# yzGuu830/efficient-speech-codec

Measured on AMD Instinct MI355X. Metric: audio-seconds/sec encode+decode, ESC-Base 9kbps 3s@16kHz, higher is better.
Workload: dtype f32 (fp32 storage and accumulation everywhere; the K = C contractions of the MLPs, of the attention's Q / K / V projections, of PatchMerge / PatchSplit and of the de-embedding run on the fp16 matrix cores with every fp32 operand split into two fp16 terms under power-of-two scales (range-safe by cons

## Files before the change

### efficient-speech-codec_amd/build.py

```python
import os
import subprocess
import sys
from concurrent.futures import ThreadPoolExecutor

HERE = os.path.dirname(os.path.abspath(__file__))
CSRC = os.path.join(HERE, "csrc")
OUT_DIR = os.path.join(HERE, "esc", "lib")
TAG = os.environ.get("ESCX_BUILD_TAG", "")
OBJ_DIR = os.path.join(HERE, "build" + ("_" + TAG if TAG else ""))
LIB = os.path.join(OUT_DIR, "libescx" + ("_" + TAG if TAG else "") + ".so")
SOURCES = ["escx_api.cpp", "escx_params.cpp", "escx_profile.cpp", "collective.cpp", "train.hip", "disc.hip", "dac.hip", "dac_loss.hip", "gemm_swin.hip", "gemm_misc.hip", "kernels_misc.hip", "len_kernels.hip", "fused_swin.hip"]
HEADERS = ["launch_prof.h", "split_terms.h", "fused_pvq.h", "fused_prvq.h", "train_prvq.h", "fused_mlp_x3.h", "train_kernels.h", "train_mlp_fused.h", "disc_kernels.h", "disc_msd_kernels.h", "dac_kernels.h", "dac_x3.h", "dac_grad_kernels.h", "dac_param_grad_kernels.h", "dac_loss_kernels.h", "gemm_bf16.h", "conv32_halo.h", "gemm_engine.h", "kernels.h", "len_kernels.h", "launchers.h", "escx_internal.h", "fused_mlp.h", "fused_attn.h", "fused_rowgemm.h", "fused_deembed.h", os.path.join("..", "..", "include", "escx.h")]
HIPCC = os.environ.get("HIPCC", "/opt/rocm/bin/hipcc")
FLAGS = ["--offload-arch=gfx950", "-O3", "-std=c++17", "-fPIC", "-Wno-unused-result"] + os.environ.get("ESCX_EXTRA_CXXFLAGS", "").split()


def _newest(paths):
    return max(os.path.getmtime(p) for p in paths)


def build(force: bool = False, verbose: bool = True) -> str:
    srcs = [os.path.join(CSRC, s) for s in SOURCES]
    deps = srcs + [os.path.normpath(os.path.join(CSRC, h)) for h in HEADERS]
    if not force and os.path.exists(LIB) and os.path.getmtime(LIB) >= _newest(deps):
        return LIB
    os.makedirs(OUT_DIR, exist_ok=True)
    os.makedirs(OBJ_DIR, exist_ok=True)

    def compile_one(src):
        obj = os.path.join(OBJ_DIR, os.path.basename(src) + ".o")
        cmd = [HIPCC] + FLAGS + (["-x", "hip"] if src.endswith(".cpp") else []) + ["-c", src, "-o", obj]
        r = subprocess.run(cmd, capture_output=True, text=True)
        if r.returncode != 0:
            raise RuntimeError(f"hipcc failed for {src}:\n{r.stdout}\n{r.stderr}")
        return obj

    with ThreadPoolExecutor(max_workers=len(srcs)) as ex:
        objs = list(ex.map(compile_one, srcs))
    cmd = [HIPCC, "--offload-arch=gfx950", "-shared", "-fPIC", "-o", LIB] + objs + ["-ldl"]
    r = subprocess.run(cmd, capture_output=True, text=True)
    if r.returncode != 0:
        raise RuntimeError(f"link failed:\n{r.stdout}\n{r.stderr}")
    if verbose:
        print(f"built {LIB} ({os.path.getsize(LIB) / 1e6:.1f} MB)")
    return LIB


if __name__ == "__main__":
    build(force="--force" in sys.argv)
```

### efficient-speech-codec_amd/csrc/escx_api.cpp

```cpp
#include <hip/hip_runtime.h>

#include <algorithm>
#include <cmath>
#include <cstdlib>
#include <cstring>
#include <map>
#include <mutex>
#include <tuple>
#include <utility>
#include <vector>

#include "escx_internal.h"
#include "launchers.h"

using namespace escx;

static void part_layout(escx_handle_s* h, int B, int T, int* k, int* per, int* pass) {
    *k = std::min(n_parts(h, B), h->n_sets);
    *pass = std::max(1, std::min(pass_clips(h, B, T), h->sets[0].shp.B));
    *per = *k <= 1 ? B : (B + *k - 1) / *k;
}

template <class F>
static int run_halves(escx_handle_s* h, int B, int T, hipStream_t st, F part) {
// ... 963 lines not shown
    const int n = h->n, G = c.group_size;
    const long long bstride = (long long)S * G * s.Tq, sstride = (long long)G * s.Tq;
    const int T2 = c.patch_t * s.W;
    long long* cd = (long long*)codes;
    if ((rc = run_stft(h, wave, B, Lx, s.T, h->spec, st))) return rc;
    if (raw_feat) PROF("unpad_len", 0, 2.0 * B * s.T * c.in_dim * h->F * 4, unpad_rows_len(h->spec, raw_feat, lc.d_L, 0, c.patch_t, c.hop_length, B, s.T, c.in_dim, h->F, h->Fp, st));
    if ((rc = run_encoder(h, s, st))) return rc;
    const size_t lslot = (size_t)G * B * s.Tq;
    float* loss = cm_loss ? h->loss_terms : nullptr;
    int n_slots = 1;
    int H = s.encH[n - 1], Hn;
    float* dec = h->decA; float* other = h->decB;
    if ((rc = run_pvq_quantize(h, h->quants[0], h->enc_hs[n - 1], nullptr, B, s.W, cd, bstride, loss, dec, st))) return rc;
    for (int i = 0; i + 1 < n; ++i) {
        if (i < S - 1) {
            if ((rc = run_pvq_quantize(h, h->quants[i + 1], h->enc_hs[n - 1 - i], dec, B, s.W, cd + (i + 1) * sstride, bstride, loss ? loss + (size_t)(i + 1) * lslot : nullptr, dec, st))) return rc;
            n_slots = i + 2;
        }
        if ((rc = run_layer(h, h->layers[n + i], dec, other, B, H, s.W, &Hn, st))) return rc;
        std::swap(dec, other); H = Hn;
    }
    if ((rc = run_layer(h, h->layers[2 * n - 1], dec, other, B, H, s.W, &Hn, st))) return rc;
    if ((rc = run_deembed(h, other, B, s.W, h->rspec, st))) return rc;
    if ((rc = run_istft(h, h->rspec, B, T2, wave_out, st))) return rc;
    if (recon_feat) PROF("unpad_len", 0, 2.0 * B * T2 * c.in_dim * h->F * 4, unpad_rows_len(h->rspec, recon_feat, lc.d_W, 1, c.patch_t, c.hop_length, B, T2, c.in_dim, h->F, h->Fp, st));
    if (cm_loss) PROF("loss_reduce_len", 0, (double)n_slots * lslot * 4, loss_reduce_len(loss, lc.d_W, c.overlap, n_slots, G, B, s.Tq, cm_loss, st));
    PROF("codes_mask_len", 0, 8.0 * B * bstride, codes_mask_len(cd, cd, lc.d_W, c.overlap, B, S * G, s.Tq, -1, st));
    return launch_ok("forward_lengths");
}

static int run_prvq(escx_handle_s* h, const float* enc, const long long* codes_in, int B, int W, long long* codes, long long bstride, const int* clip_S,
                    int S, float* loss, long long lslot, float* out, hipStream_t st) {
    const escx_config& c = h->cfg;
    const Quant& q = h->quants[0];
    const int Tq = W / c.overlap, M = B * Tq;
    const double vec = (double)c.overlap * q.Hq * q.C, G = c.group_size;
    int rc = -1;
    PROF(codes_in ? "prvq_decode" : (out ? "prvq_fused" : "prvq_fused_codes"),
         codes_in ? 2.0 * M * vec * q.d : 2.0 * M * vec * q.d * (out ? 2 : 1) + 2.0 * M * S * G * c.codebook_size * q.d,
         (double)M * vec * ((codes_in ? 0 : 1) + (out ? 1 : 0)) * 4,
         rc = prvq_fused(enc, codes_in, B, q.Hq, W, q.Cp, c.overlap, q.wdf, q.Nz, q.Kq, pvq_down_splits(M, q.Kq, q.Cp), pvq_down_bk(q.Cp), q.cbn, q.c2, q.cbraw,
                         c.group_size, c.codebook_size, q.d, q.dt, q.wup, codes, bstride, clip_S, S, S, loss, lslot, 1.0f / ((float)Tq * q.d * c.group_size),
                         c.l2norm, out, st));
    if (rc) ESCX_FAIL(ESCX_ERR_UNSUPPORTED, "rvq quantiser: geometry not covered (codebook_dim %d, %d groups)", q.d, c.group_size);
    return launch_ok("prvq");
}

static int run_plain_decoder(escx_handle_s* h, int B, int Hb, int W, float* rspec, hipStream_t st) {
    const int n = h->n;
    int rc, H = Hb, Hn;
    float* dec = h->decA; float* other = h->decB;
    for (int i = 0; i + 1 < n; ++i) {
        if ((rc = run_layer(h, h->layers[n + i], dec, other, B, H, W, &Hn, st))) return rc;
        std::swap(dec, other); H = Hn;
    }
    if ((rc = run_layer(h, h->layers[2 * n - 1], dec, other, B, H, W, &Hn, st))) return rc;
    return run_deembed(h, other, B, W, rspec, st);
}

static int rvq_counts(escx_handle_s* h, int B, const int32_t* streams, int S, int* Smax) {
    if (!streams) {
        if (S < 1 || S > h->num_rvqs) ESCX_FAIL(ESCX_ERR_INVALID_ARG, "num_streams=%d outside [1, %d] (num_rvqs)", S, h->num_rvqs);
        *Smax = S;
        return 0;
    }
    if (B < 1) ESCX_FAIL(ESCX_ERR_INVALID_ARG, "batch=%d: the per-clip stream counts need at least one clip", B);
    int m = 0;
    for (int b = 0; b < B; ++b) {
        if (streams[b] < 1 || streams[b] > h->num_rvqs) ESCX_FAIL(ESCX_ERR_INVALID_ARG, "streams[%d]=%d outside [1, %d] (num_rvqs)", b, streams[b], h->num_rvqs);
        m = std::max(m, (int)streams[b]);
    }
    *Smax = m;
    return 0;
}

static int rvq_upload(escx_handle_s* h, int B, const int32_t* streams, const int** dev, hipStream_t st) {
    *dev = nullptr;
    if (!streams) return 0;
    int32_t* d = nullptr;
    MixBufs mb; mb.add(&d, (size_t)B);
    int rc = mix_alloc(h, mb); if (rc) return rc;
    ESCX_HIP(hipMemcpyAsync(d, streams, (size_t)B * sizeof(int32_t), hipMemcpyHostToDevice, st));
    *dev = d;
    return 0;
}

static int rvq_encode(escx_handle_s* h, const float* wave, int B, int L, const int32_t* streams, int S, int64_t* codes, int* fh, int* fw, void* stream) {
    int rc = check_ready(h); if (rc) return rc;
    if (!wave || !codes) ESCX_FAIL(ESCX_ERR_INVALID_ARG, "null pointer");
    int Smax = 0; if ((rc = rvq_counts(h, B, streams, S, &Smax))) return rc;
    if (L <= h->n_fft / 2) ESCX_FAIL(ESCX_ERR_INVALID_ARG, "n_samples=%d too short for reflect padding of %d", L, h->n_fft / 2);
    Shapes s; if ((rc = ensure_ws(h, B, frames_of(h, L), &s))) return rc;
    hipStream_t st = (hipStream_t)stream;
    const int* Sdev; if ((rc = rvq_upload(h, B, streams, &Sdev, st))) return rc;
    if ((rc = ensure_pvq_tables(h, st))) return rc;
    const long long cstride = (long long)Smax * h->cfg.group_size * s.Tq;
    rc = run_halves(h, B, s.T, st, [&](int b0, int nb, hipStream_t sti) -> int {
        Shapes sp = s; sp.B = nb; int r;
        if ((r = run_stft(h, wave + (size_t)b0 * L, nb, L, sp.T, h->spec, sti))) return r;
        if ((r = run_encoder(h, sp, sti))) return r;
        return run_prvq(h, h->enc_hs[h->n - 1], nullptr, nb, sp.W, (long long*)codes + b0 * cstride, cstride, Sdev ? Sdev + b0 : nullptr, Smax, nullptr, 0, nullptr, sti);
    });
    if (rc) return rc;
    if (fh) *fh = s.encH[h->n - 1];
    if (fw) *fw = s.W;
    return ESCX_OK;
}

static int rvq_decode(escx_handle_s* h, const int64_t* codes, int B, int S, const int32_t* streams, int fh, int fw, float* wave_out, float* recon_feat, void* stream) {
    int rc = check_infer_ready(h); if (rc) return rc;
    if (!codes || !wave_out) ESCX_FAIL(ESCX_ERR_INVALID_ARG, "null pointer");
    const escx_config& c = h->cfg;
    if (S < 1 || S > h->num_rvqs) ESCX_FAIL(ESCX_ERR_INVALID_ARG, "codes.size(1)=%d outside [1, %d] (num_rvqs)", S, h->num_rvqs);
    int Smax = 0; if ((rc = rvq_counts(h, B, streams, S, &Smax))) return rc;
    if (Smax > S) ESCX_FAIL(ESCX_ERR_INVALID_ARG, "codes.size(1)=%d: must be at least max(streams)=%d", S, Smax);
    if (fw < 1 || fw % c.overlap) ESCX_FAIL(ESCX_ERR_ASSERT, "Time dimension must be multiple of overlap");
    Shapes s; if ((rc = ensure_ws(h, B, frames_for_width(h, fw), &s))) return rc;
    if (s.W != fw || s.encH[h->n - 1] != fh) ESCX_FAIL(ESCX_ERR_INVALID_ARG, "feat_shape (%d,%d) does not match the model (%d,%d)", fh, fw, s.encH[h->n - 1], s.W);
    hipStream_t st = (hipStream_t)stream;
    const int* Sdev; if ((rc = rvq_upload(h, B, streams, &Sdev, st))) return rc;
    if ((rc = ensure_pvq_tables(h, st))) return rc;
    const int T2 = c.patch_t * fw, out_len = c.hop_length * (T2 - 1);
    const long long cstride = (long long)S * c.group_size * (fw / c.overlap);
    return run_halves(h, B, s.T, st, [&](int b0, int nb, hipStream_t sti) -> int {
        int r;
        if ((r = run_prvq(h, nullptr, (const long long*)codes + b0 * cstride, nb, fw, nullptr, cstride, Sdev ? Sdev + b0 : nullptr, S, nullptr, 0, h->decA, sti))) return r;
        if ((r = run_plain_decoder(h, nb, fh, fw, h->rspec, sti))) return r;
        if ((r = run_istft(h, h->rspec, nb, T2, wave_out + (size_t)b0 * out_len, sti))) return r;
        if (recon_feat) spec_unpad(h, h->rspec, recon_feat + (size_t)b0 * T2 * c.in_dim * h->F, (long long)nb * T2, sti);
        return launch_ok("rvq_decode");
    });
}

static int rvq_forward(escx_handle_s* h, const float* wave, const float* feat, int B, int LT, const int32_t* streams, int S, int64_t* codes, float* wave_out,
                       float* raw_feat, float* recon_feat, float* cm_loss, void* stream) {
    int rc = check_infer_ready(h); if (rc) return rc;
    if ((!wave == !feat) || !codes || !wave_out) ESCX_FAIL(ESCX_ERR_INVALID_ARG, "null pointer (exactly one of wave / feat, codes and wave_out are required)");
    const escx_config& c = h->cfg;
    int Smax = 0; if ((rc = rvq_counts(h, B, streams, S, &Smax))) return rc;
    const int L = wave ? LT : 0;
    int T = wave ? 0 : LT;
    if (wave && L <= h->n_fft / 2) ESCX_FAIL(ESCX_ERR_INVALID_ARG, "n_samples=%d too short for reflect padding of %d", L, h->n_fft / 2);
    if (!wave && T < c.patch_t) ESCX_FAIL(ESCX_ERR_INVALID_ARG, "n_frames=%d shorter than one patch", T);
    if (wave) T = frames_of(h, L);
    Shapes s; if ((rc = ensure_ws(h, B, T, &s))) return rc;
    if (s.W % c.overlap) ESCX_FAIL(ESCX_ERR_ASSERT, "Time dimension must be multiple of overlap");
    hipStream_t st = (hipStream_t)stream;
    const int* Sdev; if ((rc = rvq_upload(h, B, streams, &Sdev, st))) return rc;
    if ((rc = ensure_pvq_tables(h, st))) return rc;
    const int G = c.group_size, T2 = c.patch_t * s.W, out_len = c.hop_length * (T2 - 1);
    const long long cstride = (long long)Smax * G * s.Tq;
    return run_halves(h, B, s.T, st, [&](int b0, int nb, hipStream_t sti) -> int {
        Shapes sp = s; sp.B = nb; int r;
        if (wave) { if ((r = run_stft(h, wave + (size_t)b0 * L, nb, L, sp.T, h->spec, sti))) return r; }
        else spec_pad(h, feat + (size_t)b0 * sp.T * c.in_dim * h->F, h->spec, (long long)nb * sp.T, sti);
        if (raw_feat) spec_unpad(h, h->spec, raw_feat + (size_t)b0 * sp.T * c.in_dim * h->F, (long long)nb * sp.T, sti);
        if ((r = run_encoder(h, sp, sti))) return r;
        const long long lslot = (long long)G * nb * sp.Tq;
        float* loss = cm_loss ? h->loss_terms : nullptr;
        if ((r = run_prvq(h, h->enc_hs[h->n - 1], nullptr, nb, sp.W, (long long*)codes + b0 * cstride, cstride, Sdev ? Sdev + b0 : nullptr, Smax, loss, lslot, h->decA, sti))) return r;
        if ((r = run_plain_decoder(h, nb, sp.encH[h->n - 1], sp.W, h->rspec, sti))) return r;
        if ((r = run_istft(h, h->rspec, nb, T2, wave_out + (size_t)b0 * out_len, sti))) return r;
        if (recon_feat) spec_unpad(h, h->rspec, recon_feat + (size_t)b0 * T2 * c.in_dim * h->F, (long long)nb * T2, sti);
        if (cm_loss) PROF("loss_reduce", 0, (double)lslot * Smax * 4, loss_reduce(loss, Smax, G, nb * sp.Tq, sp.Tq, cm_loss + b0, sti));
        return launch_ok("rvq_forward");
    });
}

extern "C" int escx_spec_transform(escx_handle h, const float* wave, int B, int L, float* spec, void* stream) {
    int rc = check_ready(h); if (rc) return rc;
    if (!wave || !spec || B < 1) ESCX_FAIL(ESCX_ERR_INVALID_ARG, "bad argument");
    if (L <= h->n_fft / 2) ESCX_FAIL(ESCX_ERR_INVALID_ARG, "n_samples=%d too short for reflect padding of %d", L, h->n_fft / 2);
    const int T = frames_of(h, L);
    TmpBuf t; if (t.alloc((size_t)B * T * h->cfg.in_dim * h->Fp)) ESCX_FAIL(ESCX_ERR_HIP, "hipMalloc failed");
    hipStream_t st = (hipStream_t)stream;
    if ((rc = run_stft(h, wave, B, L, T, t.p, st))) return rc;
    spec_unpad(h, t.p, spec, (long long)B * T, st);
    return launch_ok("spec_transform");
}

extern "C" int escx_audio_reconstruct(escx_handle h, const float* spec, int B, int T, float* wave, void* stream) {
    int rc = check_ready(h); if (rc) return rc;
    if (!spec || !wave || B < 1 || T < 2) ESCX_FAIL(ESCX_ERR_INVALID_ARG, "bad argument (need at least 2 frames)");
    TmpBuf ts, tf;
    if (ts.alloc((size_t)B * T * h->cfg.in_dim * h->Fp) || tf.alloc((size_t)B * T * h->winP)) ESCX_FAIL(ESCX_ERR_HIP, "hipMalloc failed");
    hipStream_t st = (hipStream_t)stream;
    const escx_config& c = h->cfg;
    spec_pad(h, spec, ts.p, (long long)B * T, st);
    gemm_store(ts.p, c.in_dim * h->Fp, B * T, h->idft_w, h->winP, c.in_dim * h->Fp, tf.p, h->winP, nullptr, st);
    istft_ola(tf.p, h->win2, wave, B, T, h->winP, c.win_length, c.hop_length, h->left, h->n_fft / 2, c.hop_length * (T - 1), st);
    return launch_ok("audio_reconstruct");
}

extern "C" int escx_patch_embed(escx_handle h, const float* spec, int B, int T, float* tokens, void* stream) {
    int rc = check_ready(h); if (rc) return rc;
    const escx_config& c = h->cfg;
    const int W = T / c.patch_t, H0 = c.in_freq / c.patch_f;
    if (!spec || !tokens || B < 1 || W < 1) ESCX_FAIL(ESCX_ERR_INVALID_ARG, "bad argument");
    TmpBuf ts, tt;
    if (ts.alloc((size_t)B * T * c.in_dim * h->Fp) || tt.alloc((size_t)B * H0 * W * h->C0p)) ESCX_FAIL(ESCX_ERR_HIP, "hipMalloc failed");
    hipStream_t st = (hipStream_t)stream;
    spec_pad(h, spec, ts.p, (long long)B * T, st);
    if ((rc = run_patch_embed(h, ts.p, B, T, W, tt.p, st))) return rc;
    unpad_rows(tt.p, tokens, (long long)B * H0 * W, h->C0, h->C0p, st);
    return launch_ok("patch_embed");
}

static int stage_ws_for_w(escx_handle_s* h, int B, int W, Shapes* s) {
    int rc = ensure_ws(h, h->parts * B, frames_for_width(h, W), s, B);
    if (!rc) s->B = B;
    return rc;
}

extern "C" int escx_transformer_layer(escx_handle h, int layer_id, const float* x, int B, int H, int W, float* y, int* H_out, void* stream) {
    int rc = check_ready(h); if (rc) return rc;
    if (layer_id < 0 || layer_id >= 2 * h->n) ESCX_FAIL(ESCX_ERR_INVALID_ARG, "layer_id out of range");
    const Layer& L = h->layers[layer_id];
    Shapes s; if ((rc = stage_ws_for_w(h, B, W, &s))) return rc;
    if ((size_t)H > (size_t)2 * s.H0) ESCX_FAIL(ESCX_ERR_INVALID_ARG, "H too large for this model");
    hipStream_t st = (hipStream_t)stream;
    if ((rc = ensure_pvq_tables(h, st))) return rc;
    int Hn;
    const size_t need = (size_t)B * H * W * L.Cp, cap = std::max<size_t>((size_t)B * s.H0 * s.W * h->C0p, 1);
    size_t big = 0; for (int i = 0; i < h->n; ++i) big = std::max(big, (size_t)B * s.encH[i] * s.W * rup(h->cfg.h_dims[i], 16));
    if (need > std::max(cap, big)) ESCX_FAIL(ESCX_ERR_INVALID_ARG, "(H=%d, W=%d) is larger than any map of this layer", H, W);
    pad_rows(x, h->stageA, (long long)B * H * W, L.C, L.Cp, st);
    if ((rc = run_layer(h, L, h->stageA, h->stageB, B, H, W, &Hn, st))) return rc;
    unpad_rows(h->stageB, y, (long long)B * Hn * W, L.scale ? L.Cout : L.C, L.scale ? L.CoutP : L.Cp, st);
    if (H_out) *H_out = Hn;
    return launch_ok("transformer_layer");
}

extern "C" int escx_pvq_encode(escx_handle h, int sid, const float* enc, const float* dec, int B, int W, int64_t* codes, int64_t bstride,
                               void* stream) {
    int rc = check_ready(h); if (rc) return rc;
    if (h->kind != 0) ESCX_FAIL(ESCX_ERR_UNSUPPORTED, "escx_pvq_encode: the cross-scale quantisers do not exist on an rvq handle (escx_rvq_encode / escx_rvq_decode)");
    if (sid < 0 || sid >= h->cfg.max_streams) ESCX_FAIL(ESCX_ERR_INVALID_ARG, "stream_id out of range");
    if (W % h->cfg.overlap) ESCX_FAIL(ESCX_ERR_ASSERT, "Time dimension must be multiple of overlap");
    const Quant& q = h->quants[sid];
    Shapes s; if ((rc = stage_ws_for_w(h, B, W, &s))) return rc;
    hipStream_t st = (hipStream_t)stream;
    const long long rows = (long long)B * q.Hq * W;
    if ((rc = ensure_pvq_tables(h, st))) return rc;
    pad_rows(enc, h->stageA, rows, q.C, q.Cp, st);
    if (dec) pad_rows(dec, h->stageB, rows, q.C, q.Cp, st);
    return run_pvq_quantize(h, q, h->stageA, dec ? h->stageB : nullptr, B, W, (long long*)codes, bstride, nullptr, nullptr, st);
}

extern "C" int escx_pvq_decode(escx_handle h, int sid, const int64_t* codes, int64_t bstride, const float* dec, int B, int W, float* out,
                               void* stream) {
    int rc = check_ready(h); if (rc) return rc;
    if (h->kind != 0) ESCX_FAIL(ESCX_ERR_UNSUPPORTED, "escx_pvq_decode: the cross-scale quantisers do not exist on an rvq handle (escx_rvq_encode / escx_rvq_decode)");
    if (sid < 0 || sid >= h->cfg.max_streams) ESCX_FAIL(ESCX_ERR_INVALID_ARG, "stream_id out of range");
    if (W % h->cfg.overlap) ESCX_FAIL(ESCX_ERR_ASSERT, "Time dimension must be multiple of overlap");
    const Quant& q = h->quants[sid];
    Shapes s; if ((rc = stage_ws_for_w(h, B, W, &s))) return rc;
    hipStream_t st = (hipStream_t)stream;
    const long long rows = (long long)B * q.Hq * W;
    if ((rc = ensure_pvq_tables(h, st))) return rc;
    if (dec) pad_rows(dec, h->stageB, rows, q.C, q.Cp, st);
    if ((rc = run_pvq_decode(h, q, (const long long*)codes, bstride, dec ? h->stageB : nullptr, B, W, h->stageA, st))) return rc;
    unpad_rows(h->stageA, out, rows, q.C, q.Cp, st);
    return launch_ok("pvq_decode");
}

extern "C" int escx_rvq_encode(escx_handle h, const float* tokens, int B, int W, int S, int64_t* codes, float* zq_out, void* stream) {
    int rc = check_ready(h); if (rc) return rc;
    if (h->kind != 1) ESCX_FAIL(ESCX_ERR_UNSUPPORTED, "escx_rvq_encode needs an rvq handle (escx_create_rvq)");
    if (!tokens || !codes) ESCX_FAIL(ESCX_ERR_INVALID_ARG, "null pointer");
    if (B < 1 || W < 1) ESCX_FAIL(ESCX_ERR_INVALID_ARG, "batch and W must be positive");
    if (S < 1 || S > h->num_rvqs) ESCX_FAIL(ESCX_ERR_INVALID_ARG, "num_streams=%d outside [1, %d] (num_rvqs)", S, h->num_rvqs);
    if (W % h->cfg.overlap) ESCX_FAIL(ESCX_ERR_ASSERT, "Time dimension must be multiple of overlap");
    const Quant& q = h->quants[0];
    Shapes s; if ((rc = stage_ws_for_w(h, B, W, &s))) return rc;
    hipStream_t st = (hipStream_t)stream;
    const long long rows = (long long)B * q.Hq * W;
    pad_rows(tokens, h->stageA, rows, q.C, q.Cp, st);
    if ((rc = run_prvq(h, h->stageA, nullptr, B, W, (long long*)codes, (long long)S * h->cfg.group_size * (W / h->cfg.overlap), nullptr, S, nullptr, 0,
                       zq_out ? h->stageB : nullptr, st))) return rc;
    if (zq_out) unpad_rows(h->stageB, zq_out, rows, q.C, q.Cp, st);
    return launch_ok("rvq_encode");
}

extern "C" int escx_rvq_decode(escx_handle h, const int64_t* codes, int B, int S, int W, float* tokens_out, void* stream) {
    int rc = check_ready(h); if (rc) return rc;
    if (h->kind != 1) ESCX_FAIL(ESCX_ERR_UNSUPPORTED, "escx_rvq_decode needs an rvq handle (escx_create_rvq)");
    if (!codes || !tokens_out) ESCX_FAIL(ESCX_ERR_INVALID_ARG, "null pointer");
    if (B < 1 || W < 1) ESCX_FAIL(ESCX_ERR_INVALID_ARG, "batch and W must be positive");
    if (S < 1 || S > h->num_rvqs) ESCX_FAIL(ESCX_ERR_INVALID_ARG, "codes.size(1)=%d outside [1, %d] (num_rvqs)", S, h->num_rvqs);
    if (W % h->cfg.overlap) ESCX_FAIL(ESCX_ERR_ASSERT, "Time dimension must be multiple of overlap");
    const Quant& q = h->quants[0];
    Shapes s; if ((rc = stage_ws_for_w(h, B, W, &s))) return rc;
    hipStream_t st = (hipStream_t)stream;
    if ((rc = run_prvq(h, nullptr, (const long long*)codes, B, W, nullptr, (long long)S * h->cfg.group_size * (W / h->cfg.overlap), nullptr, S, nullptr, 0,
                       h->stageA, st))) return rc;
    unpad_rows(h->stageA, tokens_out, (long long)B * q.Hq * W, q.C, q.Cp, st);
    return launch_ok("rvq_decode");
}

extern "C" int escx_patch_deembed(escx_handle h, const float* tokens, int B, int W, float* spec, void* stream) {
    int rc = check_infer_ready(h); if (rc) return rc;
    Shapes s; if ((rc = stage_ws_for_w(h, B, W, &s))) return rc;
    hipStream_t st = (hipStream_t)stream;
    pad_rows(tokens, h->stageA, (long long)B * s.H0 * W, h->C0, h->C0p, st);
    if ((rc = run_deembed(h, h->stageA, B, W, h->rspec, st))) return rc;
    spec_unpad(h, h->rspec, spec, (long long)B * h->cfg.patch_t * W, st);
    return launch_ok("patch_deembed");
}

extern "C" int escx_debug_mlp_trace(unsigned long long* dev_buf) { mlp_set_trace(dev_buf); return 0; }
extern "C" int escx_test_fastdiv(int n, int d) { return test_fastdiv(n, d); }
extern "C" int escx_test_math(const float* x, float* y, int64_t n, int which, void* stream) {
    test_math(x, y, n, which, (hipStream_t)stream);
    return launch_ok("test_math");
}
extern "C" int escx_test_copy_rows(const float* src, float* dst, int64_t rows, int row_floats, void* stream) {
    if (!src || !dst || rows < 1 || row_floats < 4 || row_floats % 4) ESCX_FAIL(ESCX_ERR_INVALID_ARG, "bad argument");
    test_copy_rows(src, dst, rows, row_floats, (hipStream_t)stream);
    return launch_ok("test_copy_rows");
}
extern "C" int escx_codes_pack10(const int64_t* codes, uint8_t* out, int64_t n, void* stream) {
    if (!codes || !out || n < 0) ESCX_FAIL(ESCX_ERR_INVALID_ARG, "bad argument");
    codes_pack10((const long long*)codes, out, n, (hipStream_t)stream);
    return launch_ok("codes_pack10");
}
extern "C" int escx_codes_unpack10(const uint8_t* in, int64_t* codes, int64_t n, void* stream) {
    if (!codes || !in || n < 0) ESCX_FAIL(ESCX_ERR_INVALID_ARG, "bad argument");
    codes_unpack10(in, (long long*)codes, n, (hipStream_t)stream);
    return launch_ok("codes_unpack10");
}
static int ragged_offsets(int B, int Smax, int64_t gt, const int32_t* streams, hipStream_t st, const long long** off_dev, long long* n) {
    if (!streams || B < 1 || Smax < 1 || gt < 1) ESCX_FAIL(ESCX_ERR_INVALID_ARG, "bad argument");
    std::vector<long long> off((size_t)B + 1, 0);
    for (int b = 0; b < B; ++b) {
        if (streams[b] < 1 || streams[b] > Smax) ESCX_FAIL(ESCX_ERR_INVALID_ARG, "streams[%d]=%d outside [1, %d]", b, streams[b], Smax);
        off[b + 1] = off[b] + (long long)streams[b] * gt;
    }
    long long* d = reinterpret_cast<long long*>(stream_scratch(st, 2, 2 * off.size()));
    if (!d) ESCX_FAIL(ESCX_ERR_HIP, "scratch allocation failed");
    ESCX_HIP(hipMemcpyAsync(d, off.data(), off.size() * sizeof(long long), hipMemcpyHostToDevice, st));
    *off_dev = d; *n = off[B];
    return 0;
}
extern "C" int escx_codes_pack10_streams(const int64_t* codes, int B, int Smax, int64_t gt, const int32_t* streams, uint8_t* out, void* stream) {
    if (!codes || !out) ESCX_FAIL(ESCX_ERR_INVALID_ARG, "null pointer");
    hipStream_t st = (hipStream_t)stream;
    const long long* off; long long n; int rc;
    if ((rc = ragged_offsets(B, Smax, gt, streams, st, &off, &n))) return rc;
    codes_pack10_streams((const long long*)codes, out, off, B, (long long)Smax * gt, n, st);
    return launch_ok("codes_pack10_streams");
}
extern "C" int escx_codes_unpack10_streams(const uint8_t* in, int B, int Smax, int64_t gt, const int32_t* streams, int64_t* codes, void* stream) {
    if (!codes || !in) ESCX_FAIL(ESCX_ERR_INVALID_ARG, "null pointer");
    hipStream_t st = (hipStream_t)stream;
    const long long* off; long long n; int rc;
    if ((rc = ragged_offsets(B, Smax, gt, streams, st, &off, &n))) return rc;
    codes_unpack10_streams(in, (long long*)codes, off, B, (long long)Smax * gt, st);
    return launch_ok("codes_unpack10_streams");
}
extern "C" int escx_codes_narrow(const int64_t* codes, int16_t* out, int64_t n, void* stream) {
    codes_narrow((const long long*)codes, (short*)out, n, (hipStream_t)stream);
    return launch_ok("codes_narrow");
}
extern "C" int escx_codes_widen(const int16_t* in, int64_t* codes, int64_t n, void* stream) {
    codes_widen((const short*)in, (long long*)codes, n, (hipStream_t)stream);
    return launch_ok("codes_widen");
}
```

### efficient-speech-codec_amd/csrc/fused_deembed.h

```cpp
#pragma once
#include <hip/hip_runtime.h>
#include <type_traits>
#include "gemm_engine.h"
#include "split_terms.h"

namespace escx {

struct DeembedArgs {
    const float* x;
    const f32x4* wf;
    const float* bias;
    float* out;
    int B, H, W, pf, pt, in_dim, Fp, n_out;
};

template <int CP>
__global__ __launch_bounds__(512) void deembed7_kernel(DeembedArgs a) {
    ESCX_SET_PRIO_SMALL();
    constexpr int KK = CP / 16, TH = 8, TW = 32, HH = TH + 6, HW = TW + 6, PS = CP + 4;
    constexpr int NW = 8, NP = 7 * KK, NPW = (NP + NW - 1) / NW;
    __shared__ float xs[HH * HW * PS];
    __shared__ f32x4 wr[2][NP * 64];
    const int tid = threadIdx.x, lane = tid & 63, l15 = lane & 15, lg = lane >> 4;
    const int wave = __builtin_amdgcn_readfirstlane(tid >> 6);
    const int ntw = (a.W + TW - 1) / TW, nth = (a.H + TH - 1) / TH;
    int bid = blockIdx.x;
    const int tw = bid % ntw; bid /= ntw;
    const int th = bid % nth; const int b = bid / nth;
    const int h0 = th * TH, w0 = tw * TW;

    auto issue_row = [&](int dh, int buf) {
        const f32x4* src = a.wf + (size_t)dh * NP * 64 + lane;
#pragma unroll
        for (int i = 0; i < NPW; ++i) {
            int c = wave + i * NW;
            if (NP % NW != 0) c = min(c, NP - 1);
            __builtin_amdgcn_global_load_lds((const void*)(src + c * 64), (__attribute__((address_space(3))) void*)(&wr[buf][c * 64]), 16, 0, 0);
        }
    };
    issue_row(0, 0);

    const float* xb = a.x + (size_t)b * a.H * a.W * CP;
    auto halo_vec = [&](int v) -> f32x4 {
        const int pix = v / (KK * 4), q = v - pix * (KK * 4);
        const int ph = pix / HW, pw = pix - ph * HW;
        const int gh = h0 - 3 + ph, gw = w0 - 3 + pw;
        return (gh >= 0 && gh < a.H && gw >= 0 && gw < a.W) ? ld4(xb + ((size_t)gh * a.W + gw) * CP + 4 * q) : zero4();
    };
    auto halo_put = [&](int v, f32x4 val) {
        const int pix = v / (KK * 4), q = v - pix * (KK * 4);
        *reinterpret_cast<f32x4*>(&xs[pix * PS + 4 * q]) = val;
    };
    constexpr int ROWV = HW * KK * 4;
    static_assert(ROWV <= 512, "one vector per thread per extra halo row");
    for (int v = tid; v < TH * ROWV; v += 512) halo_put(v, halo_vec(v));

    const bool seg1 = w0 + 16 < a.W;
    f32x4 acc[2] = {zero4(), zero4()};
    const float* xrow = &xs[(wave * HW + l15) * PS + 4 * lg];
    auto tap_row = [&](auto two_segments, int dh) {
        constexpr bool TWO = decltype(two_segments)::value;
        constexpr int NS = 7 * KK;
        const f32x4* wb = &wr[dh & 1][lane];
        const float* xr = xrow + dh * HW * PS;
        f32x4 w[2], x0[2], x1[2];
        auto fetch = [&](int st, int slot) {
            const int dw = st / KK, kk = st - dw * KK;
            w[slot] = wb[st * 64];
            x0[slot] = *reinterpret_cast<const f32x4*>(xr + dw * PS + 16 * kk);
            if (TWO) x1[slot] = *reinterpret_cast<const f32x4*>(xr + (dw + 16) * PS + 16 * kk);
            __builtin_amdgcn_sched_group_barrier(0x100, TWO ? 3 : 2, 0);
        };
        fetch(0, 0);
#pragma unroll
        for (int st = 0; st < NS; ++st) {
            if (st + 1 < NS) fetch(st + 1, (st + 1) & 1);
#pragma unroll
            for (int r = 0; r < 4; ++r) {
                acc[0] = __builtin_amdgcn_mfma_f32_16x16x4f32(w[st & 1][r], x0[st & 1][r], acc[0], 0, 0, 0);
                if (TWO) acc[1] = __builtin_amdgcn_mfma_f32_16x16x4f32(w[st & 1][r], x1[st & 1][r], acc[1], 0, 0, 0);
            }
            __builtin_amdgcn_sched_group_barrier(0x008, TWO ? 8 : 4, 0);
        }
    };
    for (int dh = 0; dh < 7; ++dh) {
        asm volatile("s_waitcnt vmcnt(0)" ::: "memory");
        __syncthreads();
        issue_row(min(dh + 1, 6), (dh + 1) & 1);
        const bool extra = dh < 6 && tid < ROWV;
        f32x4 nv = zero4();
        if (extra) nv = halo_vec((TH + dh) * ROWV + tid);
        if (seg1) tap_row(std::true_type{}, dh); else tap_row(std::false_type{}, dh);
        if (extra) halo_put((TH + dh) * ROWV + tid, nv);
    }

    const int h = h0 + wave;
    if (h >= a.H) return;
    const int Q = a.pf * a.pt;
    const f32x4 bv = ld4(a.bias + 4 * lg);
#pragma unroll
    for (int t = 0; t < 2; ++t) {
        const int w = w0 + 16 * t + l15;
        if (w >= a.W) continue;
#pragma unroll
        for (int r = 0; r < 4; ++r) {
            const int nn = 4 * lg + r;
            if (nn >= a.n_out) continue;
            const int co = nn / Q, q = nn - co * Q, s1 = q / a.pt, s2 = q - s1 * a.pt;
            a.out[((size_t)(b * (a.pt * a.W) + a.pt * w + s2) * a.in_dim + co) * a.Fp + a.pf * h + s1] = acc[t][r] + bv[r];
        }
    }
}

constexpr int de2_steps(int CP) { return (49 * CP + 31) / 32; }
inline size_t deembed7_x2_bytes(int CP) { return (size_t)de2_steps(CP) * 2 * 1024 + 32; }

__global__ __launch_bounds__(256) void deembed7_x2_pack_kernel(const f32x4* __restrict__ wf, bf16x8* __restrict__ out, int CP, int nsteps) {
    const int idx = blockIdx.x * 256 + threadIdx.x;
    if (idx >= nsteps * 64) return;
    const int step = idx >> 6, lane = idx & 63, n = lane & 15, g = lane >> 4, KK = CP / 16;
    bf16x8* tail = out + (size_t)nsteps * 2 * 64;
    const float sc = x2_scale(*reinterpret_cast<const unsigned*>(tail));
    float v[8];
#pragma unroll
    for (int e = 0; e < 8; ++e) {
        const int k = 32 * step + 8 * g + e, tap = k / CP, c = k - tap * CP;
        v[e] = tap < 49 ? wf[(size_t)(tap * KK + c / 16) * 64 + 16 * ((c % 16) / 4) + n][c % 4] : 0.f;
    }
    bf16x8 t[2];
    split_terms<2>(v, t, sc);
    out[(size_t)(step * 2 + 0) * 64 + lane] = t[0]; out[(size_t)(step * 2 + 1) * 64 + lane] = t[1];
    if (idx == 0) { float* o = reinterpret_cast<float*>(tail + 1); o[0] = 1.0f / sc; o[1] = sc; o[2] = 0.f; o[3] = 0.f; }
}

template <int CP>
__global__ __launch_bounds__(512) void deembed7_x2_kernel(DeembedArgs a, const bf16x8* __restrict__ wf2) {
    static_assert(CP == 48, "one wrap of the channel index per 32-deep step");
    ESCX_SET_PRIO_SMALL();
    constexpr int TH = 8, TW = 32, HH = TH + 6, HW = TW + 6, PS = CP + 8;
    constexpr int NSTEP = de2_steps(CP), CH = 8, NCH = (NSTEP + CH - 1) / CH, NW = 8, Q8 = CP / 8;
    extern __shared__ __attribute__((aligned(16))) unsigned char de2_lds[];
    _Float16* xh0 = reinterpret_cast<_Float16*>(de2_lds);
    _Float16* xh1 = xh0 + HH * HW * PS;
    bf16x8* wr = reinterpret_cast<bf16x8*>(xh1 + HH * HW * PS);
    const int tid = threadIdx.x, lane = tid & 63, l15 = lane & 15, lg = lane >> 4;
    const int wave = __builtin_amdgcn_readfirstlane(tid >> 6);
    const int ntw = (a.W + TW - 1) / TW, nth = (a.H + TH - 1) / TH;
    int bid = blockIdx.x;
    const int tw = bid % ntw; bid /= ntw;
    const int th = bid % nth; const int b = bid / nth;
    const int h0 = th * TH, w0 = tw * TW;

    auto issue_chunk = [&](int ch, int buf) {
        const int pieces = min(CH, NSTEP - ch * CH) * 2;
        const bf16x8* src = wf2 + (size_t)ch * CH * 2 * 64 + lane;
        for (int c = wave; c < pieces; c += NW)
            __builtin_amdgcn_global_load_lds((const void*)(src + c * 64), (__attribute__((address_space(3))) void*)(&wr[(buf * CH * 2 + c) * 64]), 16, 0, 0);
    };
    issue_chunk(0, 0);
    const f32x4 scv = *reinterpret_cast<const f32x4*>(wf2 + (size_t)NSTEP * 2 * 64 + 1);

    const float* xb = a.x + (size_t)b * a.H * a.W * CP;
    constexpr int NV = (HH * HW * Q8 + 511) / 512;
    float xr[NV][8];
    float amax = 0.f;
#pragma unroll
    for (int i = 0; i < NV; ++i) {
        const int v = tid + 512 * i;
        const int pix = v / Q8, q = v - pix * Q8;
        const int ph = pix / HW, pw = pix - ph * HW;
        const int gh = h0 - 3 + ph, gw = w0 - 3 + pw;
        if (v < HH * HW * Q8 && gh >= 0 && gh < a.H && gw >= 0 && gw < a.W) {
            const float* p = xb + ((size_t)gh * a.W + gw) * CP + 8 * q;
            const f32x4 u0 = ld4(p), u1 = ld4(p + 4);
#pragma unroll
            for (int e = 0; e < 4; ++e) { xr[i][e] = u0[e]; xr[i][4 + e] = u1[e]; amax = fmaxf(amax, fmaxf(fabsf(u0[e]), fabsf(u1[e]))); }
        } else {
#pragma unroll
            for (int e = 0; e < 8; ++e) xr[i][e] = 0.f;
        }
    }
    __shared__ float de2_red[NW];
    for (int o = 32; o >= 1; o >>= 1) amax = fmaxf(amax, __shfl_xor(amax, o));
    if (lane == 0) de2_red[wave] = amax;
    __syncthreads();
#pragma unroll
    for (int i = 0; i < NW; ++i) amax = fmaxf(amax, de2_red[i]);
    const float act_sc = act_pow2_scale(amax), act_inv = 1.0f / act_sc;
#pragma unroll
    for (int i = 0; i < NV; ++i) {
        const int v = tid + 512 * i;
        if (v < HH * HW * Q8) {
            const int pix = v / Q8, q = v - pix * Q8;
            bf16x8 t[2];
            split_terms<2>(xr[i], t, act_sc);
            *reinterpret_cast<bf16x8*>(xh0 + pix * PS + 8 * q) = t[0];
            *reinterpret_cast<bf16x8*>(xh1 + pix * PS + 8 * q) = t[1];
        }
    }

    const bool seg1 = w0 + 16 < a.W;
    f32x4 acc0 = zero4(), acc1 = zero4();
    int c = 8 * lg, dw = 0, dh = 0;
    for (int ch = 0; ch < NCH; ++ch) {
        asm volatile("s_waitcnt vmcnt(0)" ::: "memory");
        __syncthreads();
        if (ch + 1 < NCH) issue_chunk(ch + 1, (ch + 1) & 1);
        const bf16x8* wb = &wr[((ch & 1) * CH * 2) * 64 + lane];
#pragma unroll
        for (int s = 0; s < CH; ++s) {
            if (ch * CH + s >= NSTEP) break;
            const int dhc = dh > 6 ? 6 : dh;
            const int xoff = ((wave + dhc) * HW + dw + l15) * PS + c;
            const bf16x8 wt0 = wb[(s * 2) * 64], wt1 = wb[(s * 2 + 1) * 64];
            const bf16x8 x00 = *reinterpret_cast<const bf16x8*>(xh0 + xoff), x01 = *reinterpret_cast<const bf16x8*>(xh1 + xoff);
            acc0 = mma_x<2>(wt0, x01, acc0); acc0 = mma_x<2>(wt1, x00, acc0); acc0 = mma_x<2>(wt0, x00, acc0);
            if (seg1) {
                const bf16x8 x10 = *reinterpret_cast<const bf16x8*>(xh0 + xoff + 16 * PS), x11 = *reinterpret_cast<const bf16x8*>(xh1 + xoff + 16 * PS);
                acc1 = mma_x<2>(wt0, x11, acc1); acc1 = mma_x<2>(wt1, x10, acc1); acc1 = mma_x<2>(wt0, x10, acc1);
            }
            c += 32;
            if (c >= CP) { c -= CP; if (++dw == 7) { dw = 0; ++dh; } }
        }
    }

    const int h = h0 + wave;
    if (h >= a.H) return;
    const int Q = a.pf * a.pt;
    const f32x4 bv = ld4(a.bias + 4 * lg);
    const f32x4 accs[2] = {acc0 * (scv[0] * act_inv), acc1 * (scv[0] * act_inv)};
#pragma unroll
    for (int t = 0; t < 2; ++t) {
        const int w = w0 + 16 * t + l15;
        if (w >= a.W) continue;
#pragma unroll
        for (int r = 0; r < 4; ++r) {
            const int nn = 4 * lg + r;
            if (nn >= a.n_out) continue;
            const int co = nn / Q, q = nn - co * Q, s1 = q / a.pt, s2 = q - s1 * a.pt;
            a.out[((size_t)(b * (a.pt * a.W) + a.pt * w + s2) * a.in_dim + co) * a.Fp + a.pf * h + s1] = accs[t][r] + bv[r];
        }
    }
}

}
```

### efficient-speech-codec_amd/csrc/fused_swin.hip

```cpp
#include "fused_attn.h"
#include "fused_mlp.h"
#include "fused_mlp_x3.h"
#include <atomic>
#include "fused_rowgemm.h"
#include "fused_deembed.h"
#include "launchers.h"

namespace escx {

template <int CP, int TM>
static void launch_mlp(const MlpArgs& a, hipStream_t s) {
    const int waves = (a.M + 16 * TM - 1) / (16 * TM);
    ESCX_LAUNCH((mlp_fused_kernel<CP, TM>), dim3((waves + 3) / 4), dim3(256), 0, s, a);
}

template <int CP, int TM, int NW>
static void launch_mlp_lds(const MlpArgs& a, hipStream_t s) {
    const int rows = 16 * TM * NW;
    const int hs = a.HS > 1 ? a.HS : 1;
    ESCX_LAUNCH((mlp_fused_lds_kernel<CP, TM, NW>), dim3(((a.M + rows - 1) / rows) * hs), dim3(64 * NW), 0, s, a);
}

template <int CP>
static int launch_mlp_lds_variant(int variant, const MlpArgs& a, hipStream_t s) {
    switch (variant) {
        case 1: launch_mlp_lds<CP, 1, 4>(a, s); return 0;
        case 3: launch_mlp_lds<CP, 1, 8>(a, s); return 0;
        default: return -1;
    }
}

static unsigned long long* g_mlp_trace = nullptr;
void mlp_set_trace(unsigned long long* p) { g_mlp_trace = p; }
unsigned long long* debug_trace_buffer() { return g_mlp_trace; }

void rows_combine(float* dst, const float* src, const float* partial, const float* bias, long long M, int Cp, int n, hipStream_t s) {
    const long long n4 = M * Cp / 4;
    ESCX_LAUNCH(rows_combine_kernel, dim3((unsigned)((n4 + 255) / 256)), dim3(256), 0, s, dst, src, partial, bias, M, Cp, n);
}

template <int CP, int NW>
static void launch_mlp_split(const MlpArgs& a, hipStream_t s) {
    const int rows = 16 * NW;
    ESCX_LAUNCH((mlp_fused_lds_kernel<CP, 1, NW, true>), dim3((a.M + rows - 1) / rows), dim3(64 * NW), 0, s, a);
}

int mlp_fused(float* x, int M, int C, int Cp, const float* gamma, const float* beta, const float* w1f, const float* b1,
              const float* w2f, const float* b2, const float* wcf, int hiddenP, int variant, int* hs_io, float* partial, hipStream_t s, float* out,
              const MlpSplit* split) {
    if (split) {
        const int hs0 = hs_io ? *hs_io : 1;
        if (hs0 > 1 || out || (variant != 1 && variant != 3) || (split->NT & 1) || !(Cp == 80 || Cp == 96 || Cp == 144)) return ESCX_COMB_UNSUPPORTED;
        MlpArgs a{x, gamma, beta, reinterpret_cast<const f32x4*>(w1f), b1, reinterpret_cast<const f32x4*>(w2f), b2,
                  reinterpret_cast<const f32x4*>(wcf), M, C, hiddenP / 16, 1e-5f, 1, nullptr, nullptr,
                  reinterpret_cast<const f32x4*>(split->wf), split->gamma, split->beta, split->out, split->NT, split->H, split->W, split->C2p};
        const bool nw8 = variant == 3;
        switch (Cp) {
            case 80: if (nw8) launch_mlp_split<80, 8>(a, s); else launch_mlp_split<80, 4>(a, s); return 0;
            case 96: if (nw8) launch_mlp_split<96, 8>(a, s); else launch_mlp_split<96, 4>(a, s); return 0;
            case 144: if (nw8) launch_mlp_split<144, 8>(a, s); else launch_mlp_split<144, 4>(a, s); return 0;
        }
        return ESCX_COMB_UNSUPPORTED;
    }
    int hs = hs_io ? *hs_io : 1;
    const bool lds_width = Cp == 48 || Cp == 80 || Cp == 96 || Cp == 144 || Cp == 192 || Cp == 384;
    if (hs > 1 && (variant <= 0 || variant > 3 || !lds_width || !partial || (hiddenP / 16) % hs)) hs = 1;
    if (hs_io) *hs_io = hs;
    MlpArgs a{x, gamma, beta, reinterpret_cast<const f32x4*>(w1f), b1, reinterpret_cast<const f32x4*>(w2f), b2,
              reinterpret_cast<const f32x4*>(wcf), M, C, hiddenP / 16, 1e-5f, hs, partial, out,
              nullptr, nullptr, nullptr, nullptr, 0, 0, 0, 0};
    if (out && hs > 1) return -1;
    if (variant > 0) {
        switch (Cp) {
            case 48: return launch_mlp_lds_variant<48>(variant, a, s);
            case 80: return launch_mlp_lds_variant<80>(variant, a, s);
            case 96: return launch_mlp_lds_variant<96>(variant, a, s);
            case 144: return launch_mlp_lds_variant<144>(variant, a, s);
            case 192: return launch_mlp_lds_variant<192>(variant, a, s);
            case 384: return launch_mlp_lds_variant<384>(variant, a, s);
            default: break;
        }
    }
    switch (Cp) {
        case 16: launch_mlp<16, 4>(a, s); return 0;
        case 32: launch_mlp<32, 4>(a, s); return 0;
        case 48: launch_mlp<48, 4>(a, s); return 0;
        case 64: launch_mlp<64, 4>(a, s); return 0;
        case 80: launch_mlp<80, 4>(a, s); return 0;
        case 96: launch_mlp<96, 2>(a, s); return 0;
        case 112: launch_mlp<112, 2>(a, s); return 0;
        case 128: launch_mlp<128, 2>(a, s); return 0;
        case 144: launch_mlp<144, 2>(a, s); return 0;
        case 160: launch_mlp<160, 2>(a, s); return 0;
        case 192: launch_mlp<192, 2>(a, s); return 0;
        case 256: launch_mlp<256, 1>(a, s); return 0;
        case 288: launch_mlp<288, 1>(a, s); return 0;
        case 384: launch_mlp<384, 1>(a, s); return 0;
        default: return -1;
    }
}

static size_t mlp_x3_frag_bytes(int Cp, int hiddenP, int nt) { return (size_t)(hiddenP / 32) * mlp_x3_frags(Cp, nt) * 1024; }
size_t mlp_x3_bytes(int Cp, int hiddenP, int nt) { return mlp_x3_frag_bytes(Cp, hiddenP, nt) + 48 + (nt == 2 ? (size_t)(hiddenP + 2 * Cp) * sizeof(float) : 0); }

int mlp_x3_pack(const float* w1, const float* w2, void* image, int Cp, int hiddenP, hipStream_t s, int nt, const float* gamma, const float* beta, const float* b1, int C) {
    if (Cp % 16 || hiddenP % 32 || (nt != 2 && nt != 3)) return -1;
    if (nt == 2 && (!gamma || !beta || !b1)) return -1;
    char* tail = reinterpret_cast<char*>(image) + mlp_x3_frag_bytes(Cp, hiddenP, nt);
    const int KS = (Cp + 31) / 32, KK = Cp / 16;
    const long long total = (long long)(hiddenP / 32) * (2 * KS + KK) * 64;
    if (nt == 2) {
        unsigned* mx = reinterpret_cast<unsigned*>(tail);
        if (hipMemsetAsync(mx, 0, 16, s) != hipSuccess) return -1;
        const long long n = (long long)hiddenP * Cp;
        ESCX_LAUNCH(absmax_bits_kernel, dim3((unsigned)std::min<long long>(256, (n + 255) / 256)), dim3(256), 0, s, w1, n, mx);
        ESCX_LAUNCH(absmax_bits_kernel, dim3((unsigned)std::min<long long>(256, (n + 255) / 256)), dim3(256), 0, s, w2, n, mx + 1);
        ESCX_LAUNCH(rownorm2_max_bits_kernel, dim3((unsigned)((hiddenP + 3) / 4)), dim3(256), 0, s, w1, hiddenP, Cp, Cp, mx + 2);
    }
    ESCX_LAUNCH(mlp_x3_pack_kernel, dim3((unsigned)((total + 255) / 256)), dim3(256), 0, s, w1, w2, reinterpret_cast<bf16x8*>(image), Cp, hiddenP, KS, KK, nt, gamma, beta, b1, C);
    if (nt == 2) ESCX_LAUNCH(mlp_x3_prescale_kernel, dim3((unsigned)((hiddenP + 2 * Cp + 255) / 256)), dim3(256), 0, s, reinterpret_cast<bf16x8*>(tail), gamma, beta, b1, Cp, hiddenP);
    return 0;
}

template <int CP, int NW, int NT = 3>
static void launch_mlp_x3(const MlpArgs& a, hipStream_t s) {
    auto kern = mlp_x3_kernel<CP, NW, false, NT>;
    constexpr int lds = 2 * mlp_x3_stage_frags(CP, NT) * 1024;
    if constexpr (lds > 48 * 1024) {
        static std::atomic<unsigned> done{0};
        int dev = 0; (void)hipGetDevice(&dev);
        const unsigned bit = 1u << (dev & 31);
        if (!(done.load(std::memory_order_relaxed) & bit)) { (void)hipFuncSetAttribute((const void*)kern, hipFuncAttributeMaxDynamicSharedMemorySize, lds); done.fetch_or(bit, std::memory_order_relaxed); }
    }
    const int hs = a.HS > 1 ? a.HS : 1;
    ESCX_LAUNCH(kern, dim3(((a.M + 16 * NW - 1) / (16 * NW)) * hs), dim3(64 * NW), lds, s, a);
}


size_t mlp_x3_split_bytes(int Cp, int Np) { return (size_t)(Np / 16) * mlp_x3_split_tfy(Cp, 3) * 1024 + 32; }
static char* mlp_x3_split_trailer(const void* image, int Cp, int Np) { return reinterpret_cast<char*>(const_cast<void*>(image)) + mlp_x3_split_bytes(Cp, Np) - 32; }
int mlp_x3_split_pack(const float* wf, void* image, int Cp, int Np, hipStream_t s, int nt, const float* gamma, const float* beta, int C) {
    if (nt != 2 && nt != 3) return -1;
    if (nt == 2 && (!gamma || !beta)) return -1;
    const int KK = Cp / 16, NT = Np / 16;
    const long long total = (long long)NT * ((KK + 1) / 2) * 64;
    char* tail = mlp_x3_split_trailer(image, Cp, Np);
    if (nt == 2) {
        if (hipMemsetAsync(tail, 0, 16, s) != hipSuccess) return -1;
        const long long n = (long long)NT * KK * 64 * 4;
        ESCX_LAUNCH(absmax_bits_kernel, dim3((unsigned)std::min<long long>(256, (n + 255) / 256)), dim3(256), 0, s, wf, n, reinterpret_cast<unsigned*>(tail));
    }
    ESCX_LAUNCH(mlp_x3_split_pack_kernel, dim3((unsigned)((total + 255) / 256)), dim3(256), 0, s, reinterpret_cast<const f32x4*>(wf), reinterpret_cast<bf16x8*>(image), NT, KK,
                nt, mlp_x3_split_tfy(Cp, nt), reinterpret_cast<bf16x8*>(tail), gamma, beta, Cp, C);
    return 0;
}

template <int CP, int NW, int NT = 3>
static void launch_mlp_x3_split(const MlpArgs& a, hipStream_t s) {
    auto kern = mlp_x3_kernel<CP, NW, true, NT>;
    constexpr int lds = 2 * mlp_x3_stage_frags(CP, NT) * 1024;
    if constexpr (lds > 48 * 1024) {
        static std::atomic<unsigned> done{0};
        int dev = 0; (void)hipGetDevice(&dev);
        const unsigned bit = 1u << (dev & 31);
        if (!(done.load(std::memory_order_relaxed) & bit)) { (void)hipFuncSetAttribute((const void*)kern, hipFuncAttributeMaxDynamicSharedMemorySize, lds); done.fetch_or(bit, std::memory_order_relaxed); }
    }
    ESCX_LAUNCH(kern, dim3((a.M + 16 * NW - 1) / (16 * NW)), dim3(64 * NW), lds, s, a);
}

int mlp_x3(float* x, int M, int C, int Cp, const float* gamma, const float* beta, const float* b1, const float* b2, const void* image, int hiddenP, int nw, int* hs_io, float* partial,
           hipStream_t s, const MlpSplit* split, int nt, float* out) {
    if (!image || hiddenP % 32 || (nt != 2 && nt != 3)) return -1;
    if (out && (split || (hs_io && *hs_io > 1))) return -1;
    if (split) {
        if ((hs_io && *hs_io > 1) || !split->wf || !(Cp == 80 || Cp == 96 || Cp == 144)) return ESCX_COMB_UNSUPPORTED;
        MlpArgs a{};
        a.x = x; a.gamma = gamma; a.beta = beta; a.b1 = b1; a.b2 = b2; a.M = M; a.C = C; a.HT = hiddenP / 16; a.eps = 1e-5f; a.HS = 1; a.x3_w = image;
        a.sp_wf = reinterpret_cast<const f32x4*>(split->wf); a.sp_gamma = split->gamma; a.sp_beta = split->beta; a.sp_out = split->out;
        a.sp_NT = split->NT; a.sp_H = split->H; a.sp_W = split->W; a.sp_C2p = split->C2p;
        if (nt == 2) a.sp_scale = reinterpret_cast<const float*>(mlp_x3_split_trailer(split->wf, Cp, 16 * split->NT) + 16);
        switch (Cp) {
#define ESCX_X3S_CASE(CPV) case CPV: if (nt == 2) { if (nw == 8) launch_mlp_x3_split<CPV, 8, 2>(a, s); else launch_mlp_x3_split<CPV, 4, 2>(a, s); } \
                           else { if (nw == 8) launch_mlp_x3_split<CPV, 8>(a, s); else launch_mlp_x3_split<CPV, 4>(a, s); } return 0;
            ESCX_X3S_CASE(80) ESCX_X3S_CASE(96) ESCX_X3S_CASE(144)
#undef ESCX_X3S_CASE
        }
        return ESCX_COMB_UNSUPPORTED;
    }
    int hs = hs_io ? *hs_io : 1;
    if (hs > 1 && (!partial || (hiddenP / 32) % hs)) hs = 1;
    if (hs_io) *hs_io = hs;
    MlpArgs a{};
    a.x = x; a.gamma = gamma; a.beta = beta; a.b1 = b1; a.b2 = b2; a.M = M; a.C = C; a.HT = hiddenP / 16; a.eps = 1e-5f; a.HS = hs; a.partial = partial; a.x3_w = image; a.out = out;
#define ESCX_X3_CASE(CPV) case CPV: if (nt == 2) { if (nw == 8) launch_mlp_x3<CPV, 8, 2>(a, s); else launch_mlp_x3<CPV, 4, 2>(a, s); } \
                          else { if (nw == 8) launch_mlp_x3<CPV, 8>(a, s); else launch_mlp_x3<CPV, 4>(a, s); } return 0;
    switch (Cp) {
        ESCX_X3_CASE(48) ESCX_X3_CASE(80) ESCX_X3_CASE(96) ESCX_X3_CASE(144) ESCX_X3_CASE(192) ESCX_X3_CASE(384)
        default: return -1;
    }
#undef ESCX_X3_CASE
}


template <int KP, int SEGS>
static int launch_rowgemm(const RowGemmArgs& a, hipStream_t s) {
    if (a.x3_wf) {
        if constexpr (KP == 96 || KP == 160 || KP == 192 || KP == 288 || KP == 384 || KP == 144 || KP == 80) {
            constexpr int KSx = (KP + 31) / 32, TFx = 3 * KSx, UTx = 36 / TFx >= 4 ? 4 : (36 / TFx >= 2 ? 2 : 1);
            constexpr int TMx = KP <= 96 ? 2 : 1, NWx = 4;
            auto kern = rowgemm_x3_kernel<KP, SEGS, TMx, NWx, UTx>;
            auto kern2 = rowgemm_x3_kernel<KP, SEGS, TMx, NWx, UTx, 2>;
            constexpr int lds = 2 * UTx * TFx * 1024, lds2 = 2 * UTx * 2 * KSx * 1024;
            if constexpr (lds > 48 * 1024) {
                static std::atomic<unsigned> done{0};
                int dev = 0; (void)hipGetDevice(&dev);
                const unsigned bit = 1u << (dev & 31);
                if (!(done.load(std::memory_order_relaxed) & bit)) {
                    (void)hipFuncSetAttribute((const void*)kern, hipFuncAttributeMaxDynamicSharedMemorySize, lds);
                    (void)hipFuncSetAttribute((const void*)kern2, hipFuncAttributeMaxDynamicSharedMemorySize, lds2);
                    done.fetch_or(bit, std::memory_order_relaxed);
                }
            }
            if (a.x3_scale) ESCX_LAUNCH(kern2, dim3((a.M + 16 * TMx * NWx - 1) / (16 * TMx * NWx), 1), dim3(64 * NWx), lds2, s, a);
            else ESCX_LAUNCH(kern, dim3((a.M + 16 * TMx * NWx - 1) / (16 * TMx * NWx), 1), dim3(64 * NWx), lds, s, a);
            return 0;
        }
    }
    constexpr int KK = KP / 16;
    constexpr int UT = KK <= 6 ? 4 : (KK <= 12 ? 2 : 1);
    constexpr int TM = KP <= 192 ? 2 : 1;
    constexpr int NW = 4;
    const int rows = 16 * TM * NW;
    RowGemmArgs b = a;
    b.nt_chunk = (a.NT + UT - 1) / UT * UT;
    const int chunks = (a.NT + b.nt_chunk - 1) / b.nt_chunk;
    ESCX_LAUNCH((rowgemm_fused_kernel<KP, SEGS, TM, NW, UT>), dim3((a.M + rows - 1) / rows, chunks), dim3(64 * NW), 0, s, b);
    return 0;
}

size_t rowgemm_x3_bytes(int KP, int Np) { return (size_t)(Np / 16) * 3 * ((KP + 31) / 32) * 1024 + 32; }
static char* rowgemm_x3_trailer(const void* image, int KP, int Np) { return reinterpret_cast<char*>(const_cast<void*>(image)) + rowgemm_x3_bytes(KP, Np) - 32; }
int rowgemm_x3_pack(const float* wf, void* image, int KP, int Np, hipStream_t s, int nt, const float* gamma, const float* beta, int C) {
    const int KK = KP / 16, KS = (KP + 31) / 32, NT = Np / 16;
    const long long total = (long long)NT * (KS > KK ? KS : KK) * 64;
    if (nt == 2) {
        unsigned* mx = reinterpret_cast<unsigned*>(rowgemm_x3_trailer(image, KP, Np));
        (void)hipMemsetAsync(mx, 0, 16, s);
        const long long n = (long long)NT * KK * 64 * 4;
        ESCX_LAUNCH(absmax_bits_kernel, dim3((unsigned)std::min<long long>(256, (n + 255) / 256)), dim3(256), 0, s, wf, n, mx);
    }
    ESCX_LAUNCH(attn_x3_pack_kernel, dim3((unsigned)((total + 255) / 256)), dim3(256), 0, s, reinterpret_cast<const f32x4*>(wf), reinterpret_cast<bf16x8*>(image),
                       reinterpret_cast<bf16x8*>(rowgemm_x3_trailer(image, KP, Np)), NT, 1, KK, KS, (nt == 2 ? 2 : 3) * KS, 0u, nt == 2 ? 2 : 3, gamma, beta, KP, C, (const float*)nullptr, 0, 0, 0);
    return 0;
}

int rowgemm_fused(int segs, const float* x, float* out, const float* gamma, const float* beta, const float* wf, const int* map, int M,
                  int rows_per_clip, int src_rows_per_clip, int C, int Cp, int Np, int split, int H, int W, int C2p, hipStream_t s,
                  const void* x3_wf, int x3_nt) {
    const int KP = segs * Cp;
    RowGemmArgs a{x, out, gamma, beta, reinterpret_cast<const f32x4*>(wf), map, M, rows_per_clip, src_rows_per_clip, C, Cp, Np / 16,
                  split, H, W, C2p, 1e-5f, Np / 16, x3_wf,
                  (x3_wf && x3_nt == 2) ? reinterpret_cast<const float*>(rowgemm_x3_trailer(x3_wf, KP, Np) + 16) : nullptr};
    if (segs == 1) {
        switch (KP) {
            case 16: return launch_rowgemm<16, 1>(a, s);
            case 48: return launch_rowgemm<48, 1>(a, s);
            case 80: return launch_rowgemm<80, 1>(a, s);
            case 96: return launch_rowgemm<96, 1>(a, s);
            case 144: return launch_rowgemm<144, 1>(a, s);
            case 192: return launch_rowgemm<192, 1>(a, s);
            case 384: return launch_rowgemm<384, 1>(a, s);
            default: return -1;
        }
    }
    switch (KP) {
        case 32: return launch_rowgemm<32, 2>(a, s);
        case 96: return launch_rowgemm<96, 2>(a, s);
        case 160: return launch_rowgemm<160, 2>(a, s);
        case 192: return launch_rowgemm<192, 2>(a, s);
        case 288: return launch_rowgemm<288, 2>(a, s);
        case 384: return launch_rowgemm<384, 2>(a, s);
        default: return -1;
    }
}

size_t deembed7_x2_image_bytes(int Cp) { return Cp == 48 ? deembed7_x2_bytes(Cp) : 0; }
int deembed7_x2_pack(const float* wfrag, void* image, int Cp, hipStream_t s) {
    if (Cp != 48) return -1;
    const int nsteps = de2_steps(Cp);
    unsigned* mx = reinterpret_cast<unsigned*>(reinterpret_cast<char*>(image) + deembed7_x2_bytes(Cp) - 32);
    if (hipMemsetAsync(mx, 0, 32, s) != hipSuccess) return -1;
    const long long n = (long long)49 * (Cp / 16) * 64 * 4;
    ESCX_LAUNCH(absmax_bits_kernel, dim3((unsigned)std::min<long long>(256, (n + 255) / 256)), dim3(256), 0, s, wfrag, n, mx);
    ESCX_LAUNCH(deembed7_x2_pack_kernel, dim3((nsteps * 64 + 255) / 256), dim3(256), 0, s, reinterpret_cast<const f32x4*>(wfrag), reinterpret_cast<bf16x8*>(image), Cp, nsteps);
    return 0;
}

int deembed7_fused(const float* tok, int B, int H, int W, int Cp, const float* wfrag, const float* bias, float* out, int pf, int pt,
                   int in_dim, int Fp, hipStream_t s, const void* x2_image) {
    DeembedArgs a{tok, reinterpret_cast<const f32x4*>(wfrag), bias, out, B, H, W, pf, pt, in_dim, Fp, in_dim * pf * pt};
    if (a.n_out > 16) return -1;
    const int grid = B * ((H + 7) / 8) * ((W + 31) / 32);
    if (x2_image && Cp == 48) {
        auto kern = deembed7_x2_kernel<48>;
        constexpr int lds = 2 * 14 * 38 * (48 + 8) * 2 + 2 * 8 * 2 * 1024;
        static std::atomic<unsigned> done{0};
        int dev = 0; (void)hipGetDevice(&dev);
        const unsigned bit = 1u << (dev & 31);
        if (!(done.load(std::memory_order_relaxed) & bit)) { (void)hipFuncSetAttribute((const void*)kern, hipFuncAttributeMaxDynamicSharedMemorySize, lds); done.fetch_or(bit, std::memory_order_relaxed); }
        ESCX_LAUNCH(kern, dim3(grid), dim3(512), lds, s, a, reinterpret_cast<const bf16x8*>(x2_image));
        return 0;
    }
    switch (Cp) {
        case 16: ESCX_LAUNCH(deembed7_kernel<16>, dim3(grid), dim3(512), 0, s, a); return 0;
        case 32: ESCX_LAUNCH(deembed7_kernel<32>, dim3(grid), dim3(512), 0, s, a); return 0;
        case 48: ESCX_LAUNCH(deembed7_kernel<48>, dim3(grid), dim3(512), 0, s, a); return 0;
        default: return -1;
    }
}

static constexpr bool attn_x3_fused(int Cp, int mode) {
    return (Cp == 48 && mode == 0) || (Cp == 80 && (mode == 0 || mode == 2)) || (Cp == 96 && mode != 2) || (Cp == 144 && mode != 2) || (Cp == 192 && mode == 1);
}
static int attn_x3_pairing(int Cp, int mode, int n_groups) { return (!attn_x3_fused(Cp, mode) || Cp < 80) ? 0 : (mode == 2 ? 2 : (n_groups % 2 == 0 ? 1 : 0)); }

template <int CP, int MODE, int NW, bool LEN = false>
static int launch_attn(const AttnArgs& a, hipStream_t s, bool pair) {
    constexpr int UT = CP <= 96 ? 4 : (CP <= 192 ? 2 : 1);
    constexpr int TMW = attn_windows_per_wave(CP);
    const int per_block = TMW * NW;
    const int gs = a.GS > 1 ? a.GS : 1;
    if (a.tape_qkv) {
        if constexpr (LEN) return ESCX_COMB_UNSUPPORTED;
        if constexpr (CP == 16 || CP == 48 || CP == 80 || CP == 96) {
            if (gs == 1) {
                ESCX_LAUNCH((attn_fused_kernel<CP, MODE, UT, TMW, NW, true>), dim3((a.n_windows + per_block - 1) / per_block), dim3(64 * NW), 0, s, a);
                return 0;
            }
        }
        return ESCX_COMB_UNSUPPORTED;
    }
    if constexpr (attn_x3_fused(CP, MODE)) {
        if (a.x3_wf) {
            auto kern = attn_fused_kernel<CP, MODE, UT, TMW, NW, false, true, 3, false, LEN>;
            auto kern2 = attn_fused_kernel<CP, MODE, UT, TMW, NW, false, true, 2, false, LEN>;
            constexpr int lds = 2 * UT * attn_x3_tf(CP) * 1024, lds2 = 2 * UT * attn_x3_tf(CP, 2) * 1024;
            if constexpr (lds > 48 * 1024) {
                static std::atomic<unsigned> done{0};
                int dev = 0; (void)hipGetDevice(&dev);
                const unsigned bit = 1u << (dev & 31);
                if (!(done.load(std::memory_order_relaxed) & bit)) {
                    (void)hipFuncSetAttribute((const void*)kern, hipFuncAttributeMaxDynamicSharedMemorySize, lds);
                    (void)hipFuncSetAttribute((const void*)kern2, hipFuncAttributeMaxDynamicSharedMemorySize, lds2);
                    done.fetch_or(bit, std::memory_order_relaxed);
                }
            }
            if constexpr (CP >= 80) {
                if (a.x3_scale && pair) {
                    auto kern2p = attn_fused_kernel<CP, MODE, UT, TMW, NW, false, true, 2, true, LEN>;
                    if constexpr (lds2 > 48 * 1024) {
                        static std::atomic<unsigned> donep{0};
                        int dev = 0; (void)hipGetDevice(&dev);
                        const unsigned bit = 1u << (dev & 31);
                        if (!(donep.load(std::memory_order_relaxed) & bit)) { (void)hipFuncSetAttribute((const void*)kern2p, hipFuncAttributeMaxDynamicSharedMemorySize, lds2); donep.fetch_or(bit, std::memory_order_relaxed); }
                    }
                    ESCX_LAUNCH(kern2p, dim3(((a.n_windows + per_block - 1) / per_block) * gs), dim3(64 * NW), lds2, s, a);
                    return 0;
                }
            }
            if (pair) return -1;
            if (a.x3_scale) ESCX_LAUNCH(kern2, dim3(((a.n_windows + per_block - 1) / per_block) * gs), dim3(64 * NW), lds2, s, a);
            else ESCX_LAUNCH(kern, dim3(((a.n_windows + per_block - 1) / per_block) * gs), dim3(64 * NW), lds, s, a);
            return 0;
        }
    }
    ESCX_LAUNCH((attn_fused_kernel<CP, MODE, UT, TMW, NW, false, false, 3, false, LEN>), dim3(((a.n_windows + per_block - 1) / per_block) * gs), dim3(64 * NW), 0, s, a);
    return 0;
}

template <int CP, bool LEN = false>
static int launch_attn_cp(int mode, int nw, const AttnArgs& a, hipStream_t s, bool pair) {
    if (nw == 8) {
        switch (mode) {
            case 0: return launch_attn<CP, 0, 8, LEN>(a, s, pair);
            case 1: return launch_attn<CP, 1, 8, LEN>(a, s, pair);
            case 2: return launch_attn<CP, 2, 8, LEN>(a, s, pair);
        }
    } else {
        switch (mode) {
            case 0: return launch_attn<CP, 0, 4, LEN>(a, s, pair);
            case 1: return launch_attn<CP, 1, 4, LEN>(a, s, pair);
            case 2: return launch_attn<CP, 2, 4, LEN>(a, s, pair);
        }
    }
    return -1;
}

template <int CP, int NW>
static int launch_attn_packed(const AttnArgs& a, hipStream_t s) {
    constexpr int UT = CP <= 96 ? 4 : (CP <= 192 ? 2 : 1);
    const int pairs = (a.n_windows + 1) / 2;
    const int gs = a.GS > 1 ? a.GS : 1;
    if constexpr (CP == 384 && NW == 4) {
        if (a.x3_wf) {
            auto kern = attn_packed_kernel<CP, UT, NW, true>;
            auto kern2 = attn_packed_kernel<CP, UT, NW, true, 2>;
            constexpr int lds = 2 * UT * attn_x3_tf(CP) * 1024, lds2 = 2 * UT * attn_x3_tf(CP, 2) * 1024;
            static std::atomic<unsigned> done{0};
            int dev = 0; (void)hipGetDevice(&dev);
            const unsigned bit = 1u << (dev & 31);
            if (!(done.load(std::memory_order_relaxed) & bit)) {
                (void)hipFuncSetAttribute((const void*)kern, hipFuncAttributeMaxDynamicSharedMemorySize, lds);
                (void)hipFuncSetAttribute((const void*)kern2, hipFuncAttributeMaxDynamicSharedMemorySize, lds2);
                done.fetch_or(bit, std::memory_order_relaxed);
            }
            if (a.x3_scale) ESCX_LAUNCH(kern2, dim3(((pairs + NW - 1) / NW) * gs), dim3(64 * NW), lds2, s, a);
            else ESCX_LAUNCH(kern, dim3(((pairs + NW - 1) / NW) * gs), dim3(64 * NW), lds, s, a);
            return 0;
        }
    }
    ESCX_LAUNCH((attn_packed_kernel<CP, UT, NW>), dim3(((pairs + NW - 1) / NW) * gs), dim3(64 * NW), 0, s, a);
    return 0;
}

size_t attn_x3_bytes(int Cp, int mode, int n_groups) { return (size_t)n_groups * (mode == 2 ? 8 : 4) * attn_x3_tf(Cp) * 1024 + 48; }
static char* attn_x3_trailer(const void* image, int Cp, int mode, int n_groups) { return reinterpret_cast<char*>(const_cast<void*>(image)) + attn_x3_bytes(Cp, mode, n_groups) - 48; }

int attn_x3_pack(const float* waf, void* image, int Cp, int mode, int n_groups, hipStream_t s, int nt, const float* gamma, const float* beta, int C, const float* bqkv) {
    const int KK = Cp / 16, KS = attn_x3_ks(Cp), TF = attn_x3_tf(Cp, nt == 2 ? 2 : 3), TPG = mode == 2 ? 8 : 4;
    const unsigned proj_mask = mode == 2 ? ((1u << 5) | (1u << 7)) : (1u << 3);
    const int pair = nt == 2 ? attn_x3_pairing(Cp, mode, n_groups) : 0;
    const int n_tiles = n_groups * TPG;
    (void)hipMemsetAsync(image, 0, attn_x3_bytes(Cp, mode, n_groups), s);
    const long long total = (long long)n_tiles * (KS > KK ? KS : KK) * 64;
    if (nt == 2) {
        unsigned* mx = reinterpret_cast<unsigned*>(attn_x3_trailer(image, Cp, mode, n_groups));
        const long long n = (long long)n_tiles * KK * 64 * 4;
        const unsigned all = (1u << TPG) - 1, vmask = mode == 2 ? ((1u << 4) | (1u << 6)) : (1u << 2);
        const dim3 grid((unsigned)std::min<long long>(256, (n + 255) / 256));
        ESCX_LAUNCH(absmax_tiles_bits_kernel, grid, dim3(256), 0, s, waf, n, KK * 256, TPG, all & ~proj_mask, mx);
        ESCX_LAUNCH(absmax_tiles_bits_kernel, grid, dim3(256), 0, s, waf, n, KK * 256, TPG, vmask, mx + 1);
        ESCX_LAUNCH(absmax_tiles_bits_kernel, grid, dim3(256), 0, s, waf, n, KK * 256, TPG, proj_mask, mx + 2);
    }
    ESCX_LAUNCH(attn_x3_pack_kernel, dim3((unsigned)((total + 255) / 256)), dim3(256), 0, s, reinterpret_cast<const f32x4*>(waf), reinterpret_cast<bf16x8*>(image),
                       reinterpret_cast<bf16x8*>(attn_x3_trailer(image, Cp, mode, n_groups)), n_tiles, TPG, KK, KS, TF, proj_mask, nt == 2 ? 2 : 3, gamma, beta, Cp, C, bqkv, n_groups * (mode == 2 ? 6 : 3) * 16, pair,
                       x2_tail_paired(Cp, nt) ? 1 : 0);
    return 0;
}

int attn_fused(const float* src, float* dst, int Cp, int C, int mode, int n_groups, const float* gamma, const float* beta,
               const float* wf, const float* bqkv, const float* bias_tab, const float* bproj, const int* map, int slots, int tokens,
               int n_windows, int nWh, int nWw, int shifted, float scale, int nw, int* gs_io, float* partial, int rows, hipStream_t s,
               const AttnTape* tape, const void* x3_wf, int x3_nt, bool len_tables) {
    int gs = gs_io ? *gs_io : 1;
    if (gs > 1 && (!partial || n_groups % gs)) gs = 1;
    const int pairing = (!tape && x3_wf && x3_nt == 2) ? attn_x3_pairing(Cp, mode, n_groups) : 0;
    if (pairing == 1 && (n_groups / gs) % 2) gs = 1;
    if (gs_io) *gs_io = gs;
    AttnArgs a{src, dst, gamma, beta, reinterpret_cast<const f32x4*>(wf), bqkv, bias_tab, bproj, map, slots, tokens, n_windows,
               nWh, nWw, shifted, C, n_groups, scale, 1e-5f, gs, partial, rows, g_mlp_trace,
               tape ? tape->xn : nullptr, tape ? tape->qkv : nullptr, tape ? tape->o : nullptr, tape ? tape->ldq : 0, tape ? tape->ldo : 0,
               tape ? tape->hdp : 0, tape ? tape->nH : 0, tape ? nullptr : x3_wf,
               (!tape && x3_wf && x3_nt == 2) ? reinterpret_cast<const float*>(attn_x3_trailer(x3_wf, Cp, mode, n_groups) + 16) : nullptr};
    if (tape && nw < 0) return ESCX_COMB_UNSUPPORTED;
    if (len_tables) {
        if (tape || nw < 0) return ESCX_COMB_UNSUPPORTED;
        switch (Cp) {
            case 16: return launch_attn_cp<16, true>(mode, nw, a, s, pairing != 0);
            case 32: return launch_attn_cp<32, true>(mode, nw, a, s, pairing != 0);
            case 48: return launch_attn_cp<48, true>(mode, nw, a, s, pairing != 0);
            case 64: return launch_attn_cp<64, true>(mode, nw, a, s, pairing != 0);
            case 80: return launch_attn_cp<80, true>(mode, nw, a, s, pairing != 0);
            case 96: return launch_attn_cp<96, true>(mode, nw, a, s, pairing != 0);
            case 128: return launch_attn_cp<128, true>(mode, nw, a, s, pairing != 0);
            case 144: return launch_attn_cp<144, true>(mode, nw, a, s, pairing != 0);
            case 192: return launch_attn_cp<192, true>(mode, nw, a, s, pairing != 0);
            case 256: return launch_attn_cp<256, true>(mode, nw, a, s, pairing != 0);
            case 384: return launch_attn_cp<384, true>(mode, nw, a, s, pairing != 0);
            default: return -1;
        }
    }
    if (nw < 0) {
        nw = -nw;
        if (mode == 0) {
#define ESCX_PACK(CPV) case CPV: return nw == 8 ? launch_attn_packed<CPV, 8>(a, s) : launch_attn_packed<CPV, 4>(a, s);
            switch (Cp) { ESCX_PACK(64) ESCX_PACK(96) ESCX_PACK(128) ESCX_PACK(192) ESCX_PACK(256) ESCX_PACK(384) default: break; }
#undef ESCX_PACK
        }
    }
    switch (Cp) {
        case 16: return launch_attn_cp<16>(mode, nw, a, s, pairing != 0);
        case 32: return launch_attn_cp<32>(mode, nw, a, s, pairing != 0);
        case 48: return launch_attn_cp<48>(mode, nw, a, s, pairing != 0);
        case 64: return launch_attn_cp<64>(mode, nw, a, s, pairing != 0);
        case 80: return launch_attn_cp<80>(mode, nw, a, s, pairing != 0);
        case 96: return launch_attn_cp<96>(mode, nw, a, s, pairing != 0);
        case 128: return launch_attn_cp<128>(mode, nw, a, s, pairing != 0);
        case 144: return launch_attn_cp<144>(mode, nw, a, s, pairing != 0);
        case 192: return launch_attn_cp<192>(mode, nw, a, s, pairing != 0);
        case 256: return launch_attn_cp<256>(mode, nw, a, s, pairing != 0);
        case 384: return launch_attn_cp<384>(mode, nw, a, s, pairing != 0);
        default: return -1;
    }
}

}
```

### efficient-speech-codec_amd/csrc/kernels.h

```cpp
#pragma once
#include <hip/hip_runtime.h>
#include "gemm_engine.h"

namespace escx {

template <int SEGS, int MODE>
__global__ __launch_bounds__(256) void ln_rows_kernel(const float* __restrict__ src, float* __restrict__ dst,
                                                      const float* __restrict__ gamma, const float* __restrict__ beta,
                                                      const int* __restrict__ map, int rows_per_clip, int src_rows_per_clip,
                                                      int total_rows, int C, int Cp, float eps) {
    const int sub = threadIdx.x & 15;
    const int grp = (blockIdx.x * 256 + threadIdx.x) >> 4;
    const int ngrp = (gridDim.x * 256) >> 4;
    const int V = Cp / 4;
    for (int row = grp; row < total_rows; row += ngrp) {
        const int b = row / rows_per_clip, rr = row - b * rows_per_clip;
        const float* sp[SEGS];
        bool zero_out = false;
#pragma unroll
        for (int s = 0; s < SEGS; ++s) {
            int srow = (MODE == 0) ? rr : map[rr * SEGS + s];
            if (srow < 0) { sp[s] = nullptr; if (MODE == 1) zero_out = true; }
            else sp[s] = src + ((size_t)b * src_rows_per_clip + srow) * Cp;
        }
        float* dp = dst + (size_t)row * (SEGS * Cp);
        if (zero_out) {
            for (int v = sub; v < V; v += 16) st4(dp + 4 * v, zero4());
            continue;
        }
        float sum = 0.f;
#pragma unroll
        for (int s = 0; s < SEGS; ++s)
            if (sp[s])
                for (int v = sub; v < V; v += 16) {
                    f32x4 x = ld4(sp[s] + 4 * v);
#pragma unroll
                    for (int e = 0; e < 4; ++e) if (4 * v + e < C) sum += x[e];
                }
#pragma unroll
        for (int o = 8; o >= 1; o >>= 1) sum += __shfl_xor(sum, o, 16);
        const float mean = sum / (float)(SEGS * C);
        float var = 0.f;
#pragma unroll
        for (int s = 0; s < SEGS; ++s)
            for (int v = sub; v < V; v += 16) {
                f32x4 x = sp[s] ? ld4(sp[s] + 4 * v) : zero4();
#pragma unroll
                for (int e = 0; e < 4; ++e) if (4 * v + e < C) { const float d = x[e] - mean; var += d * d; }
            }
#pragma unroll
        for (int o = 8; o >= 1; o >>= 1) var += __shfl_xor(var, o, 16);
        const float rstd = 1.0f / sqrtf(var / (float)(SEGS * C) + eps);
#pragma unroll
        for (int s = 0; s < SEGS; ++s)
            for (int v = sub; v < V; v += 16) {
                f32x4 x = sp[s] ? ld4(sp[s] + 4 * v) : zero4();
                const f32x4 g = ld4(gamma + s * Cp + 4 * v), bb = ld4(beta + s * Cp + 4 * v);
                f32x4 y;
#pragma unroll
                for (int e = 0; e < 4; ++e) y[e] = (4 * v + e < C) ? (x[e] - mean) * rstd * g[e] + bb[e] : 0.f;
                st4(dp + s * Cp + 4 * v, y);
            }
    }
}

template <int STEPS>
__global__ __launch_bounds__(256) void window_attention_kernel(const float* __restrict__ qkv, const float* __restrict__ bias,
                                                               float* __restrict__ out, int total_pairs, int nH, int ldq, int ldo,
                                                               int nWh, int nWw, int shifted) {
    constexpr int HDP = 4 * STEPS;
    constexpr int DT = (HDP + 15) / 16;
    const int lane = threadIdx.x & 63;
    const int i = lane & 15, g = lane >> 4;
    const int wave_global = (blockIdx.x * 256 + threadIdx.x) >> 6;
    const int nwaves = (gridDim.x * 256) >> 6;
    const int kOff = nH * HDP, vOff = 2 * nH * HDP;
    for (int pair = wave_global; pair < total_pairs; pair += nwaves) {
        const int win = pair / nH, h = pair - win * nH;
        const float* base = qkv + (size_t)win * 16 * ldq + h * HDP;
        const float* rowp = base + (size_t)i * ldq + STEPS * g;
        float kf[STEPS], qf[STEPS];
#pragma unroll
        for (int r = 0; r < STEPS; ++r) { qf[r] = rowp[r]; kf[r] = rowp[kOff + r]; }
        f32x4 s = zero4();
#pragma unroll
        for (int r = 0; r < STEPS; ++r) s = __builtin_amdgcn_mfma_f32_16x16x4f32(kf[r], qf[r], s, 0, 0, 0);
        s += ld4(bias + ((size_t)h * 16 + i) * 16 + 4 * g);
        if (shifted) {
            const int wloc = win % (nWh * nWw);
            const int wh = wloc / nWw, ww = wloc - wh * nWw;
            const bool lastH = (wh == nWh - 1), lastW = (ww == nWw - 1);
            const int qh = i >> 2, qw = i & 3;
            const int labq = 3 * (lastH ? (qh < 2 ? 1 : 2) : 0) + (lastW ? (qw < 2 ? 1 : 2) : 0);
            const int labkh = 3 * (lastH ? (g < 2 ? 1 : 2) : 0);
#pragma unroll
            for (int r = 0; r < 4; ++r) {
                const int labk = labkh + (lastW ? (r < 2 ? 1 : 2) : 0);
                s[r] += (labk != labq) ? -100.0f : 0.0f;
            }
        }
        float mx = fmaxf(fmaxf(s[0], s[1]), fmaxf(s[2], s[3]));
        mx = fmaxf(mx, __shfl_xor(mx, 16));
        mx = fmaxf(mx, __shfl_xor(mx, 32));
        f32x4 p;
#pragma unroll
        for (int r = 0; r < 4; ++r) p[r] = expf(s[r] - mx);
        float den = (p[0] + p[1]) + (p[2] + p[3]);
        den += __shfl_xor(den, 16);
        den += __shfl_xor(den, 32);
        const float inv = 1.0f / den;
#pragma unroll
        for (int r = 0; r < 4; ++r) p[r] *= inv;
        float* orow = out + ((size_t)win * 16 + i) * ldo + h * HDP;
#pragma unroll
        for (int t = 0; t < DT; ++t) {
            const int d = t * 16 + i;
            f32x4 o = zero4();
#pragma unroll
            for (int r = 0; r < 4; ++r) {
                const float vv = (d < HDP) ? base[(size_t)(4 * g + r) * ldq + vOff + d] : 0.f;
                o = __builtin_amdgcn_mfma_f32_16x16x4f32(vv, p[r], o, 0, 0, 0);
            }
            if (t * 16 + 4 * g < HDP) st4(orow + t * 16 + 4 * g, o);
        }
        if (h == 0 && nH * HDP < ldo) {
            for (int c = nH * HDP + g; c < ldo; c += 4) out[((size_t)win * 16 + i) * ldo + c] = 0.f;
        }
    }
}

__global__ __launch_bounds__(64) void window_attention_any_kernel(const float* __restrict__ qkv, const float* __restrict__ bias, float* __restrict__ out, int nH, int hd,
                                                                  int hdp, int ldq, int ldo, int ws, int nWh, int nWw, int shift) {
    const int win = blockIdx.x, h = blockIdx.y, N = ws * ws;
    const int wloc = win % (nWh * nWw), wh = wloc / nWw, ww = wloc - wh * nWw;
    const int Hp = nWh * ws, Wp = nWw * ws;
    const float* base = qkv + (size_t)win * N * ldq + h * hdp;
    const int kOff = nH * hdp, vOff = 2 * nH * hdp;
    const float* bh = bias + (size_t)h * N * N;
    auto region = [&](int p, int P) { return p < P - ws ? 0 : (p < P - shift ? 1 : 2); };
    for (int i = threadIdx.x; i < N; i += 64) {
        const float* q = base + (size_t)i * ldq;
        const int labq = shift > 0 ? 3 * region(wh * ws + i / ws, Hp) + region(ww * ws + i % ws, Wp) : 0;
        auto score = [&](int j) {
            const float* k = base + (size_t)j * ldq + kOff;
            float s = 0.f;
            for (int d = 0; d < hd; ++d) s = __builtin_fmaf(q[d], k[d], s);
            s += bh[(size_t)i * N + j];
            if (shift > 0) { const int labk = 3 * region(wh * ws + j / ws, Hp) + region(ww * ws + j % ws, Wp); s += (labk != labq) ? -100.0f : 0.0f; }
            return s;
        };
        float mx = -__builtin_inff();
        for (int j = 0; j < N; ++j) mx = fmaxf(mx, score(j));
        float den = 0.f;
        for (int j = 0; j < N; ++j) den += expf(score(j) - mx);
        const float inv = 1.0f / den;
        float* orow = out + ((size_t)win * N + i) * ldo + h * hdp;
        for (int d0 = 0; d0 < hdp; d0 += 4) {
            float o0 = 0.f, o1 = 0.f, o2 = 0.f, o3 = 0.f;
            for (int j = 0; j < N; ++j) {
                const float p = expf(score(j) - mx) * inv;
                const float* v = base + (size_t)j * ldq + vOff + d0;
                o0 = __builtin_fmaf(p, v[0], o0); o1 = __builtin_fmaf(p, v[1], o1); o2 = __builtin_fmaf(p, v[2], o2); o3 = __builtin_fmaf(p, v[3], o3);
            }
            orow[d0] = o0; orow[d0 + 1] = o1; orow[d0 + 2] = o2; orow[d0 + 3] = o3;
        }
        if (h == 0) for (int c = nH * hdp; c < ldo; ++c) out[((size_t)win * N + i) * ldo + c] = 0.f;
    }
}

struct SearchArgs {
    const float* zpart; int splits; int M; int ldz;
    const float* cbn; const float* c2; const float* cbraw;
    int Ksz, d, Tq;
    long long* codes; long long bstride;
    float* loss; float loss_scale;
    int l2norm;
};

__device__ __forceinline__ bool arg_better(float d1, int i1, float d2, int i2) {
    const bool n1 = d1 != d1, n2 = d2 != d2;
    if (n1 || n2) return n1 && (!n2 || i1 < i2);
    return d1 < d2 || (d1 == d2 && i1 < i2);
}
__device__ __forceinline__ bool arg_better_sel(float d1, int i1, float d2, int i2) {
    const bool n1 = d1 != d1, n2 = d2 != d2;
    return (n1 | n2) ? (n1 & (!n2 | (i1 < i2))) : ((d1 < d2) | ((d1 == d2) & (i1 < i2)));
}

template <int STEPS>
__global__ __launch_bounds__(256) void pvq_search_kernel(SearchArgs a) {
    ESCX_SET_PRIO_SMALL();
    constexpr int DT = 4 * STEPS;
    __shared__ float zs[16][DT + 1];
    __shared__ float zn2[16][DT];
    __shared__ float asum[16];
    __shared__ float bestd[4][16];
    __shared__ int besti[4][16];
    const int g = blockIdx.y;
    const int m0 = blockIdx.x * 16;
    const int tid = threadIdx.x;
    for (int e = tid; e < 16 * DT; e += 256) {
        const int r = e / DT, j = e - r * DT;
        const int m = m0 + r;
        float part[16];
        const bool live = m < a.M && j < a.d;
        const float* zp = a.zpart + (size_t)(live ? m : 0) * a.ldz + g * DT + (live ? j : 0);
#pragma unroll
        for (int s = 0; s < 16; ++s) part[s] = (live && s < a.splits) ? zp[(size_t)s * a.M * a.ldz] : 0.f;
        float z = 0.f;
#pragma unroll
        for (int s = 0; s < 16; ++s) z += part[s];
        for (int s = 16; s < a.splits; ++s) z += live ? zp[(size_t)s * a.M * a.ldz] : 0.f;
        zs[r][j] = z;
    }
    __syncthreads();
    if (tid < 16) {
        float ss = 0.f;
        for (int j = 0; j < a.d; ++j) ss += zs[tid][j] * zs[tid][j];
        const float den = a.l2norm ? fmaxf(sqrtf(ss), 1e-12f) : 1.0f;
        float s2 = 0.f;
        for (int j = 0; j < DT; ++j) {
            const float zn = (j < a.d) ? zs[tid][j] / den : 0.f;
            s2 += zn * zn;
            zn2[tid][j] = 2.0f * zn;
        }
        asum[tid] = s2;
    }
    __syncthreads();
    const int lane = tid & 63, wave = tid >> 6;
    const int vi = lane & 15, lg = lane >> 4;
    float zf[STEPS];
#pragma unroll
    for (int r = 0; r < STEPS; ++r) zf[r] = zn2[vi][STEPS * lg + r];
    const float av = asum[vi];
    const float* cb = a.cbn + (size_t)g * a.Ksz * DT;
    const float* c2 = a.c2 + (size_t)g * a.Ksz;
    float bd = __builtin_inff();
    int bi = 0x7fffffff;
    bool have = false;
    const int per_wave = (a.Ksz + 3) / 4;
    const int cbeg = wave * per_wave, cend = min(a.Ksz, cbeg + per_wave);
    auto load_tile = [&](int c0, float* cf, float* c2v) {
        const float* p = cb + (size_t)min(c0 + vi, a.Ksz - 1) * DT + STEPS * lg;
#pragma unroll
        for (int r = 0; r < STEPS; ++r) cf[r] = p[r];
#pragma unroll
        for (int r = 0; r < 4; ++r) c2v[r] = c2[min(c0 + 4 * lg + r, a.Ksz - 1)];
    };
    float cf[STEPS], c2v[4], cfn[STEPS], c2n[4];
    if (cbeg < cend) load_tile(cbeg, cf, c2v);
    for (int c0 = cbeg; c0 < cend; c0 += 16) {
        load_tile(min(c0 + 16, cend - 1), cfn, c2n);
        f32x4 dot = zero4();
#pragma unroll
        for (int r = 0; r < STEPS; ++r) dot = __builtin_amdgcn_mfma_f32_16x16x4f32(cf[r], zf[r], dot, 0, 0, 0);
#pragma unroll
        for (int r = 0; r < 4; ++r) {
            const int code = c0 + 4 * lg + r;
            if (code < cend) {
                const float dist = (av - dot[r]) + c2v[r];
                if (!have || arg_better(dist, code, bd, bi)) { bd = dist; bi = code; have = true; }
            }
        }
#pragma unroll
        for (int r = 0; r < STEPS; ++r) cf[r] = cfn[r];
#pragma unroll
        for (int r = 0; r < 4; ++r) c2v[r] = c2n[r];
    }
    if (!have) { bd = __builtin_inff(); bi = 0x7fffffff; }
#pragma unroll
    for (int o = 16; o <= 32; o <<= 1) {
        const float od = __shfl_xor(bd, o);
        const int oi = __shfl_xor(bi, o);
        if (arg_better(od, oi, bd, bi)) { bd = od; bi = oi; }
    }
    if (lg == 0) { bestd[wave][vi] = bd; besti[wave][vi] = bi; }
    __syncthreads();
    if (tid < 16) {
        float d0 = bestd[0][tid]; int i0 = besti[0][tid];
        for (int w = 1; w < 4; ++w) if (arg_better(bestd[w][tid], besti[w][tid], d0, i0)) { d0 = bestd[w][tid]; i0 = besti[w][tid]; }
        const int m = m0 + tid;
        if (m < a.M) {
            const int b = m / a.Tq, t = m - b * a.Tq;
            a.codes[(size_t)b * a.bstride + (size_t)g * a.Tq + t] = (long long)i0;
            if (a.loss) {
                const float* q = a.cbraw + ((size_t)g * a.Ksz + i0) * DT;
                float e = 0.f;
                for (int j = 0; j < a.d; ++j) { const float df = q[j] - zs[tid][j]; e += df * df; }
                a.loss[(size_t)g * a.M + m] = e * a.loss_scale;
            }
        }
    }
}

struct PvqUpArgs {
    const long long* codes; long long bstride; const float* cb; const float* W; const float* dec; float* out;
    int G, Ksz, dt, Tq, M, Hq, Wd, Cp, ov, Kup, NT, nt_per_wg;
};

template <int KC>
__global__ __launch_bounds__(256) void pvq_up_kernel(PvqUpArgs a) {
    ESCX_SET_PRIO_SMALL();
    constexpr int UNR = 4;
    const int lane = threadIdx.x & 63, l15 = lane & 15, lg = lane >> 4;
    const int wave = __builtin_amdgcn_readfirstlane(threadIdx.x >> 6);
    const int m = blockIdx.x * 16 + l15;
    const bool live = m < a.M;
    const int b = live ? m / a.Tq : 0, t = live ? m - b * a.Tq : 0;
    const size_t base = ((size_t)b * a.Hq * a.Wd + (size_t)a.ov * t) * a.Cp + 4 * lg;
    f32x4 zf[KC];
#pragma unroll
    for (int c = 0; c < KC; ++c) {
        const int k = 16 * c + 4 * lg, g = k / a.dt;
        zf[c] = zero4();
        if (live && g < a.G) {
            long long code = a.codes[(size_t)b * a.bstride + (size_t)g * a.Tq + t];
            code = code < 0 ? 0 : (code >= a.Ksz ? a.Ksz - 1 : code);
            zf[c] = ld4(a.cb + ((size_t)g * a.Ksz + (size_t)code) * a.dt + (k - g * a.dt));
        }
    }
    const int nt_lo = blockIdx.y * a.nt_per_wg, nt_hi = min(a.NT, nt_lo + a.nt_per_wg);
    const float* wrow = a.W + (size_t)l15 * a.Kup + 4 * lg;
    for (int nt0 = nt_lo + wave * UNR; nt0 < nt_hi; nt0 += 4 * UNR) {
        f32x4 wf[UNR][KC], dv[UNR];
        size_t idx[UNR];
#pragma unroll
        for (int u = 0; u < UNR; ++u) {
            const int nt = min(nt0 + u, nt_hi - 1);
#pragma unroll
            for (int c = 0; c < KC; ++c) wf[u][c] = ld4(wrow + (size_t)(16 * nt) * a.Kup + 16 * c);
            const int n0 = 16 * nt, oh = n0 / a.Cp, c0 = n0 - oh * a.Cp, o = oh / a.Hq, h = oh - o * a.Hq;
            idx[u] = base + (size_t)(h * a.Wd + o) * a.Cp + c0;
            dv[u] = (live && a.dec) ? ld4(a.dec + idx[u]) : zero4();
        }
#pragma unroll
        for (int u = 0; u < UNR; ++u) {
            f32x4 acc = zero4();
#pragma unroll
            for (int c = 0; c < KC; ++c)
#pragma unroll
                for (int r = 0; r < 4; ++r) acc = __builtin_amdgcn_mfma_f32_16x16x4f32(wf[u][c][r], zf[c][r], acc, 0, 0, 0);
            if (live && nt0 + u < nt_hi) {
                if (a.dec) acc += dv[u];
                st4(a.out + idx[u], acc);
            }
        }
    }
}

__global__ __launch_bounds__(64) void loss_reduce_kernel(const float* __restrict__ terms, int n_slots, int G, int M, int Tq, float* __restrict__ out) {
    const int b = blockIdx.x, lane = threadIdx.x;
    const int per = n_slots * G * Tq;
    float acc = 0.f;
    for (int i = lane; i < per; i += 64) {
        const int sg = i / Tq, t = i - sg * Tq;
        acc += terms[(size_t)sg * M + (size_t)b * Tq + t];
    }
#pragma unroll
    for (int o = 1; o < 64; o <<= 1) acc += __shfl_xor(acc, o);
    if (lane == 0) out[b] = acc;
}

__global__ void istft_ola_kernel(const float* __restrict__ frames, const float* __restrict__ win2, float* __restrict__ wave,
                                 int B, int T, int ldf, int win, int hop, int left, int half, int out_len) {
    const int idx = blockIdx.x * blockDim.x + threadIdx.x;
    if (idx >= B * out_len) return;
    const int b = idx / out_len, s = idx - b * out_len;
    const int p = s + half - left;
    int t_hi = p / hop; if (t_hi > T - 1) t_hi = T - 1;
    float acc = 0.f, env = 0.f;
    for (int t = t_hi; t >= 0; --t) {
        const int j = p - t * hop;
        if (j >= win) break;
        acc += frames[((size_t)b * T + t) * ldf + j];
        env += win2[j];
    }
    wave[idx] = acc / env;
}

template <int NO>
__global__ __launch_bounds__(256) void deembed_border_kernel(const float* __restrict__ x, const float* __restrict__ wv,
                                                             const float* __restrict__ bv, float* __restrict__ out, int B, int H, int W,
                                                             int C, int Cp, int pf, int pt, int in_dim, int Fp) {
    const int per_clip = 2 * W + 2 * (H > 2 ? H - 2 : 0);
    const int wave = (blockIdx.x * 256 + threadIdx.x) >> 6, lane = threadIdx.x & 63;
    if (wave >= B * per_clip) return;
    const int b = wave / per_clip; int i = wave - b * per_clip;
    int h, w;
    if (i < W) { h = 0; w = i; }
    else if (i < 2 * W) { h = H - 1; w = i - W; }
    else { i -= 2 * W; h = 1 + (i >> 1); w = (i & 1) ? W - 1 : 0; }
    if (H == 1 && i >= W && i < 2 * W) return;
    if (W == 1 && i >= 2 * W && (i & 1)) return;
    const int eh = (h == 0 ? 1 : 0) | (h == H - 1 ? 2 : 0), ew = (w == 0 ? 1 : 0) | (w == W - 1 ? 2 : 0);
    const int K = 49 * C;
    const float* wvar = wv + (size_t)(4 * eh + ew) * NO * K;
    float acc[NO];
#pragma unroll
    for (int o = 0; o < NO; ++o) acc[o] = 0.f;
    for (int k = lane; k < K; k += 64) {
        const int tap = k / C, ci = k - tap * C;
        const int hh = h + tap / 7 - 3, ww = w + tap % 7 - 3;
        if (hh < 0 || hh >= H || ww < 0 || ww >= W) continue;
        const float xv = x[((size_t)(b * H + hh) * W + ww) * Cp + ci];
#pragma unroll
        for (int o = 0; o < NO; ++o) acc[o] = fmaf(wvar[(size_t)o * K + k], xv, acc[o]);
    }
#pragma unroll
    for (int o = 0; o < NO; ++o) {
#pragma unroll
        for (int sft = 32; sft >= 1; sft >>= 1) acc[o] += __shfl_xor(acc[o], sft);
    }
    if (lane == 0) {
        const int Q = pf * pt;
        for (int o = 0; o < NO; ++o) {
            const int co = o / Q, q = o - co * Q, s1 = q / pt, s2 = q - s1 * pt;
            out[((size_t)(b * (pt * W) + pt * w + s2) * in_dim + co) * Fp + pf * h + s1] = acc[o] + bv[(4 * eh + ew) * NO + o];
        }
    }
}

__global__ void pad_rows_kernel(const float* __restrict__ src, float* __restrict__ dst, long long rows, int C, int Cp) {
    const long long idx = (long long)blockIdx.x * blockDim.x + threadIdx.x;
    if (idx >= rows * Cp) return;
    const long long r = idx / Cp; const int c = (int)(idx - r * Cp);
    dst[idx] = c < C ? src[r * C + c] : 0.f;
}
__global__ void unpad_rows_kernel(const float* __restrict__ src, float* __restrict__ dst, long long rows, int C, int Cp) {
    const long long idx = (long long)blockIdx.x * blockDim.x + threadIdx.x;
    if (idx >= rows * C) return;
    const long long r = idx / C; const int c = (int)(idx - r * C);
    dst[idx] = src[r * Cp + c];
}
__global__ void codes_pack10_kernel(const long long* __restrict__ in, unsigned char* __restrict__ out, long long n) {
    const long long q = (long long)blockIdx.x * blockDim.x + threadIdx.x;
    if (q * 4 >= n) return;
    unsigned long long v = 0;
#pragma unroll
    for (int j = 0; j < 4; ++j) { const long long i = q * 4 + j; v |= (unsigned long long)((i < n ? in[i] : 0) & 1023) << (10 * j); }
#pragma unroll
    for (int j = 0; j < 5; ++j) out[q * 5 + j] = (unsigned char)(v >> (8 * j));
}
__global__ void codes_unpack10_kernel(const unsigned char* __restrict__ in, long long* __restrict__ out, long long n) {
    const long long q = (long long)blockIdx.x * blockDim.x + threadIdx.x;
    if (q * 4 >= n) return;
    unsigned long long v = 0;
#pragma unroll
    for (int j = 0; j < 5; ++j) v |= (unsigned long long)in[q * 5 + j] << (8 * j);
#pragma unroll
    for (int j = 0; j < 4; ++j) { const long long i = q * 4 + j; if (i < n) out[i] = (long long)((v >> (10 * j)) & 1023); }
}
__global__ __launch_bounds__(256) void test_copy_rows_kernel(const float* __restrict__ src, float* __restrict__ dst, long long rows, int Cp) {
    const int sub = threadIdx.x & 15;
    const long long grp = ((long long)blockIdx.x * 256 + threadIdx.x) >> 4, ngrp = ((long long)gridDim.x * 256) >> 4;
    for (long long r = grp; r < rows; r += ngrp)
        for (int v = sub; v < Cp / 4; v += 16) st4(dst + r * Cp + 4 * v, ld4(src + r * Cp + 4 * v));
}
__global__ void test_math_kernel(const float* __restrict__ x, float* __restrict__ y, long long n, int which) {
    const long long i = (long long)blockIdx.x * blockDim.x + threadIdx.x;
    if (i >= n) return;
    y[i] = which == 0 ? gelu_bf(x[i]) : (which == 1 ? erf_bf(x[i]) : (which == 2 ? exp_fast(x[i]) : gelu_erf(x[i])));
}
__global__ __launch_bounds__(256) void rows_permute_kernel(const float* __restrict__ src, float* __restrict__ dst, const int* __restrict__ map, int rows,
                                                           long long row_len, int vec) {
    const long long step = (long long)gridDim.x * 256;
    for (int r = blockIdx.y; r < rows; r += gridDim.y) {
        const float* s = src + (size_t)map[r] * row_len;
        float* d = dst + (size_t)r * row_len;
        if (vec) {
            for (long long i = (long long)blockIdx.x * 256 + threadIdx.x; i < row_len / 4; i += step)
                reinterpret_cast<float4*>(d)[i] = reinterpret_cast<const float4*>(s)[i];
        } else {
            for (long long i = (long long)blockIdx.x * 256 + threadIdx.x; i < row_len; i += step) d[i] = s[i];
        }
    }
}
__global__ void codes_permute_kernel(const long long* __restrict__ src, long long src_stride, long long* __restrict__ dst, const int* __restrict__ map,
                                     const int* __restrict__ S, int rows, int Smax, int GT) {
    const long long per = (long long)Smax * GT;
    const long long idx = (long long)blockIdx.x * blockDim.x + threadIdx.x;
    if (idx >= rows * per) return;
    const int r = (int)(idx / per);
    const long long k = idx - r * per;
    dst[idx] = k < (long long)S[r] * GT ? src[(size_t)map[r] * src_stride + k] : -1;
}
struct SlotRows { int m[8]; };
__global__ __launch_bounds__(64) void loss_reduce_streams_kernel(const float* __restrict__ terms, long long lslot, const int* __restrict__ S, int cap,
                                                                 SlotRows rows, int G, int Tq, float* __restrict__ out) {
    const int b = blockIdx.x, lane = threadIdx.x;
    const int per = min(S[b], cap) * G * Tq;
    float acc = 0.f;
    for (int i = lane; i < per; i += 64) {
        const int sg = i / Tq, t = i - sg * Tq;
        const int j = sg / G, g = sg - j * G;
        acc += terms[(size_t)j * lslot + (size_t)g * rows.m[j] + (size_t)b * Tq + t];
    }
#pragma unroll
    for (int o = 1; o < 64; o <<= 1) acc += __shfl_xor(acc, o);
    if (lane == 0) out[b] = acc;
}
__device__ inline int clip_of(const long long* __restrict__ off, int B, long long i) {
    int lo = 0, hi = B - 1;
    while (lo < hi) { const int mid = (lo + hi + 1) >> 1; if (off[mid] <= i) lo = mid; else hi = mid - 1; }
    return lo;
}
__global__ void codes_pack10_streams_kernel(const long long* __restrict__ in, unsigned char* __restrict__ out, const long long* __restrict__ off, int B,
                                            long long clip_stride) {
    const long long n = off[B];
    const long long q = (long long)blockIdx.x * blockDim.x + threadIdx.x;
    if (q * 4 >= n) return;
    unsigned long long v = 0;
#pragma unroll
    for (int j = 0; j < 4; ++j) {
        const long long i = q * 4 + j;
        if (i >= n) break;
        const int b = clip_of(off, B, i);
        v |= (unsigned long long)(in[(size_t)b * clip_stride + (i - off[b])] & 1023) << (10 * j);
    }
#pragma unroll
    for (int j = 0; j < 5; ++j) out[q * 5 + j] = (unsigned char)(v >> (8 * j));
}
__global__ void codes_unpack10_streams_kernel(const unsigned char* __restrict__ in, long long* __restrict__ out, const long long* __restrict__ off, int B,
                                              long long clip_stride) {
    const long long e = (long long)blockIdx.x * blockDim.x + threadIdx.x;
    if (e >= (long long)B * clip_stride) return;
    const int b = (int)(e / clip_stride);
    const long long k = e - b * clip_stride;
    if (k >= off[b + 1] - off[b]) { out[e] = -1; return; }
    const long long bit = 10 * (off[b] + k);
    const unsigned v = (unsigned)in[bit >> 3] | ((unsigned)in[(bit >> 3) + 1] << 8);
    out[e] = (long long)((v >> (bit & 7)) & 1023);
}
__global__ void codes_narrow_kernel(const long long* __restrict__ in, short* __restrict__ out, long long n) {
    const long long i = (long long)blockIdx.x * blockDim.x + threadIdx.x;
    if (i < n) out[i] = (short)in[i];
}
__global__ void codes_widen_kernel(const short* __restrict__ in, long long* __restrict__ out, long long n) {
    const long long i = (long long)blockIdx.x * blockDim.x + threadIdx.x;
    if (i < n) out[i] = (long long)in[i];
}

}
```

### efficient-speech-codec_amd/csrc/launchers.h

```cpp
#pragma once
#include <hip/hip_runtime.h>

namespace escx {

void gemm_qkv(const float* A, int lda, int M, const float* W, int Np, int Kp, float* out, const float* bias,
              int nq, float scale, hipStream_t s);
void gemm_proj_scatter(const float* A, int lda, int M, const float* W, int Np, int Kp, float* out, const float* shortcut,
                       const float* bias, const int* map, int slots, int tokens, hipStream_t s);
void gemm_gelu(const float* A, int lda, int M, const float* W, int Np, int Kp, float* out, const float* bias, hipStream_t s);
void gemm_residual(const float* A, int lda, int M, const float* W, int Np, int Kp, float* out, const float* bias,
                   const float* res, hipStream_t s);
void gemm_store(const float* A, int lda, int M, const float* W, int Np, int Kp, float* out, int ldo, const float* bias, hipStream_t s);
void gemm_split(const float* A, int lda, int M, const float* W, int Np, int Kp, float* out, int H, int Wd, int C2p, hipStream_t s);

#ifndef ESCX_MLP_OCC4
#define ESCX_MLP_OCC4 96
#endif
#ifndef ESCX_ATTN_TMW2_MAX
#define ESCX_ATTN_TMW2_MAX 48
#endif
constexpr int attn_windows_per_wave(int Cp) { return Cp <= ESCX_ATTN_TMW2_MAX ? 2 : 1; }

constexpr int ESCX_COMB_UNSUPPORTED = -3;
struct MlpSplit { const float* wf; const float* gamma; const float* beta; float* out; int NT, H, W, C2p; };
int mlp_fused(float* x, int M, int C, int Cp, const float* gamma, const float* beta, const float* w1f, const float* b1,
              const float* w2f, const float* b2, const float* wcf, int hiddenP, int variant, int* hs_io, float* partial, hipStream_t s,
              float* out = nullptr,
              const MlpSplit* split = nullptr);
unsigned long long* debug_trace_buffer();
size_t mlp_x3_bytes(int Cp, int hiddenP, int nt = 3);
int mlp_x3_pack(const float* w1, const float* w2, void* image, int Cp, int hiddenP, hipStream_t s, int nt = 3, const float* gamma = nullptr, const float* beta = nullptr,
                const float* b1 = nullptr, int C = 0);
struct MlpSplit;
int mlp_x3(float* x, int M, int C, int Cp, const float* gamma, const float* beta, const float* b1, const float* b2, const void* image, int hiddenP, int nw, int* hs_io, float* partial,
           hipStream_t s, const MlpSplit* split = nullptr, int nt = 3, float* out = nullptr);
size_t mlp_x3_split_bytes(int Cp, int Np);
int mlp_x3_split_pack(const float* wf, void* image, int Cp, int Np, hipStream_t s, int nt = 3, const float* gamma = nullptr, const float* beta = nullptr, int C = 0);
void rows_combine(float* dst, const float* src, const float* partial, const float* bias, long long M, int Cp, int n, hipStream_t s);

int rowgemm_fused(int segs, const float* x, float* out, const float* gamma, const float* beta, const float* wf, const int* map, int M,
                  int rows_per_clip, int src_rows_per_clip, int C, int Cp, int Np, int split, int H, int W, int C2p, hipStream_t s,
                  const void* x3_wf = nullptr, int x3_nt = 3);
size_t rowgemm_x3_bytes(int KP, int Np);
int rowgemm_x3_pack(const float* wf, void* image, int KP, int Np, hipStream_t s, int nt = 3, const float* gamma = nullptr, const float* beta = nullptr, int C = 0);
void loss_reduce(const float* terms, int n_slots, int G, int M, int Tq, float* out, hipStream_t s);
void mlp_set_trace(unsigned long long* p);
int test_fastdiv(int n, int d);
int deembed7_fused(const float* tok, int B, int H, int W, int Cp, const float* wfrag, const float* bias, float* out, int pf, int pt,
                   int in_dim, int Fp, hipStream_t s, const void* x2_image = nullptr);
size_t deembed7_x2_image_bytes(int Cp);
int deembed7_x2_pack(const float* wfrag, void* image, int Cp, hipStream_t s);
int attn_fused(const float* src, float* dst, int Cp, int C, int mode, int n_groups, const float* gamma, const float* beta,
               const float* wf, const float* bqkv, const float* bias_tab, const float* bproj, const int* map, int slots, int tokens,
               int n_windows, int nWh, int nWw, int shifted, float scale, int nw, int* gs_io, float* partial, int rows, hipStream_t s,
               const struct AttnTape* tape = nullptr,
               const void* x3_wf = nullptr, int x3_nt = 3,
               bool len_tables = false);
size_t attn_x3_bytes(int Cp, int mode, int n_groups);
int attn_x3_pack(const float* waf, void* image, int Cp, int mode, int n_groups, hipStream_t s, int nt = 3, const float* gamma = nullptr, const float* beta = nullptr, int C = 0, const float* bqkv = nullptr);
struct AttnTape { float* xn; float* qkv; float* o; int ldq, ldo, hdp, nH; };

void gemm_frames(const float* wave, int B, int L, int T, int hop, int off, const float* W, int Np, int Kp, float* out, hipStream_t s);
void gemm_patch(const float* spec, int B, int T, int in_dim, int Fp, int H, int Wd, int pf, int pt, const float* W, int Np, int Kp,
                float* out, const float* bias, hipStream_t s);
void gemm_conv_deembed1(const float* x, int B, int H, int Wd, int Cp, const float* W, int Np, float* out, const float* bias,
                        int pf, int pt, hipStream_t s);
void gemm_conv_spec(const float* x, int B, int T, int F, int Cp, const float* W, float* out, const float* bias, int Fp, int in_dim,
                    hipStream_t s);
void gemm_deembed_composed(const float* x, int B, int H, int Wd, int Cp, const float* W, float* out, const float* bias, int pf, int pt,
                           int in_dim, int Fp, hipStream_t s);
int deembed_border(const float* x, const float* wv, const float* bv, float* out, int B, int H, int W, int C, int Cp, int pf, int pt,
                   int in_dim, int Fp, hipStream_t s);
void gemm_pvq_down(const float* enc, const float* dec, int B, int Hq, int Wd, int Cp, int ov, const float* W, int Np, int Kp,
                   float* zpart, int splits, hipStream_t s);
int pvq_down_splits(int M, int Kp, int Cp);
void gemm_pvq_up(const long long* codes, long long bstride, const float* cbraw, int G, int Ksz, int dt, int B, int Hq, int Wd, int Cp,
                 int ov, const float* W, int Np, int Kp, const float* dec, float* out, hipStream_t s);

void ln_rows(int mode, const float* src, float* dst, const float* gamma, const float* beta, const int* map, int rows_per_clip,
             int src_rows_per_clip, int total_rows, int C, int Cp, hipStream_t s);
int window_attention(const float* qkv, const float* bias, float* out, int total_windows, int nH, int hdp, int ldq, int ldo, int nWh,
                     int nWw, int shifted, hipStream_t s);
int window_attention_any(const float* qkv, const float* bias, float* out, int total_windows, int ws, int nH, int hd, int hdp, int ldq, int ldo, int nWh, int nWw,
                         int shift, hipStream_t s);
int pvq_fused(const float* enc, const float* dec, int B, int Hq, int Wd, int Cp, int ov, const float* wdf, int Np, int Kq, int splits, int bk,
              const float* cbn, const float* c2, const float* cbraw, int G, int Ksz, int d, int dt, const float* wup, const float* tab, const float* gq,
              float* out, long long* codes, long long bstride, float* loss, float loss_scale, int l2norm, hipStream_t s);
bool prvq_geometry_ok(int Np, int dt, int G, int Kq, int Cp, int splits, int bk);
int prvq_fused(const float* enc, const long long* codes_in, int B, int Hq, int Wd, int Cp, int ov, const float* wdf, int Np, int Kq, int splits, int bk,
               const float* cbn, const float* c2, const float* cbraw, int G, int Ksz, int d, int dt, const float* wup,
               long long* codes, long long bstride, const int* clip_S, int S, int Smax, float* loss, long long lslot, float loss_scale, int l2norm,
               float* out, hipStream_t s);
int prvq_train_fwd(const float* enc, int B, int Hq, int Wd, int Cp, int ov, const float* wdf, int Np, int Kq, int splits, int bk, const float* cbn, const float* c2,
                   const float* cbraw, int G, int Ksz, int d, int dt, const float* wup, long long* codes, long long bstride, int S, int R, int freeze, float* ze,
                   float* zq, float* terms, long long lslot, float loss_scale, int l2norm, float* out, hipStream_t s);
void pvq_tab_add(const long long* codes, long long bstride, const float* tab, const float* gq, int G, int Ksz, int B, int Hq, int Wd, int Cp, int ov,
                 const float* dec, float* out, hipStream_t s);
int pvq_down_bk(int Cp);
int pvq_up(const long long* codes, long long bstride, const float* cbraw, int G, int Ksz, int dt, int B, int Hq, int Wd, int Cp, int ov,
           const float* W, int Np, int Kp, const float* dec, float* out, hipStream_t s);
int pvq_search(const float* zpart, int splits, int M, int ldz, const float* cbn, const float* c2, const float* cbraw, int G, int Ksz,
               int d, int dt, int Tq, long long* codes, long long bstride, float* loss, float loss_scale, int l2norm, hipStream_t s);
void istft_ola(const float* frames, const float* win2, float* wave, int B, int T, int ldf, int win, int hop, int left, int half,
               int out_len, hipStream_t s);
void pad_rows(const float* src, float* dst, long long rows, int C, int Cp, hipStream_t s);
void unpad_rows(const float* src, float* dst, long long rows, int C, int Cp, hipStream_t s);
void codes_pack10(const long long* in, unsigned char* out, long long n, hipStream_t s);
void codes_unpack10(const unsigned char* in, long long* out, long long n, hipStream_t s);
void test_math(const float* x, float* y, long long n, int which, hipStream_t s);
void test_copy_rows(const float* src, float* dst, long long rows, int Cp, hipStream_t s);
void rows_permute(const float* src, float* dst, const int* map, int rows, long long row_len, hipStream_t s);
void codes_permute(const long long* src, long long src_stride, long long* dst, const int* map, const int* S, int rows, int Smax, int GT, hipStream_t s);
void loss_reduce_streams(const float* terms, long long lslot, const int* S, int cap, const int* slot_clips, int G, int Tq, int B, float* out, hipStream_t s);
void codes_pack10_streams(const long long* in, unsigned char* out, const long long* off, int B, long long clip_stride, long long n, hipStream_t s);
void codes_unpack10_streams(const unsigned char* in, long long* out, const long long* off, int B, long long clip_stride, hipStream_t s);
void gemm_frames_len(const float* wave, const int* len, int B, int L, int T, int hop, int off, const float* W, int Np, int Kp, float* out, hipStream_t s);
int window_attention_len(const float* qkv, const float* bias, float* out, int total_windows, int nH, int hdp, int ldq, int ldo, const int* flags, int shifted,
                         hipStream_t s);
void zero_dead_cols(float* x, const int* wlen, int B, int H, int W, int Cp, hipStream_t s);
int deembed_border_len(const float* x, const float* wv, const float* bv, float* out, const int* wlen, int B, int H, int W, int C, int Cp, int pf, int pt,
                       int in_dim, int Fp, hipStream_t s);
void istft_ola_len(const float* frames, const float* win2, float* wave, const int* wlen, int pt, int B, int T, int ldf, int win, int hop, int left, int half,
                   int out_len, hipStream_t s);
void loss_reduce_len(const float* terms, const int* wlen, int ov, int n_slots, int G, int B, int Tq, float* out, hipStream_t s);
void codes_mask_len(const long long* src, long long* dst, const int* wlen, int ov, int B, int rows, int Tq, long long fill, hipStream_t s);
void unpad_rows_len(const float* src, float* dst, const int* len, int per_w, int pt, int hop, int B, int T, int segs, int C, int Cp, hipStream_t s);
void codes_narrow(const long long* in, short* out, long long n, hipStream_t s);
void codes_widen(const short* in, long long* out, long long n, hipStream_t s);

}
```

### efficient-speech-codec_amd/csrc/len_kernels.h

```cpp
#pragma once
#include <hip/hip_runtime.h>
#include "gemm_engine.h"

namespace escx {

struct FrameALen {
    static constexpr bool SKIPS_DEAD_TILES = true;
    const float* wave; const int* len; int L, T, hop, off, M; FastDiv dT;
    struct Ctx { const float* w; int start; int n; };
    __device__ __forceinline__ Ctx make_ctx(int m) const {
        Ctx c; c.w = nullptr; c.start = 0; c.n = 0;
        if (m < M) {
            const int b = dT.div(m), f = m - b * T, n = len[b];
            if (f < 1 + n / hop) { c.w = wave + (size_t)b * L; c.start = f * hop + off; c.n = n; }
        }
        return c;
    }
    __device__ __forceinline__ int row_live(const Ctx& c) const { return c.w != nullptr; }
    __device__ __forceinline__ float at(const Ctx& c, int p) const {
        if (p < 0) p = -p;
        if (p >= c.n) p = 2 * (c.n - 1) - p;
        return c.w[p];
    }
    __device__ __forceinline__ f32x4 load4(const Ctx& c, int k0, int kin) const {
        if (!c.w) return zero4();
        const int p = c.start + k0 + kin;
        f32x4 v; v[0] = at(c, p); v[1] = at(c, p + 1); v[2] = at(c, p + 2); v[3] = at(c, p + 3);
        return v;
    }
};

template <int STEPS>
__global__ __launch_bounds__(256) void window_attention_len_kernel(const float* __restrict__ qkv, const float* __restrict__ bias, float* __restrict__ out,
                                                                   int total_pairs, int nH, int ldq, int ldo, const int* __restrict__ flags, int shifted) {
    constexpr int HDP = 4 * STEPS;
    constexpr int DT = (HDP + 15) / 16;
    const int lane = threadIdx.x & 63;
    const int i = lane & 15, g = lane >> 4;
    const int wave_global = (blockIdx.x * 256 + threadIdx.x) >> 6;
    const int nwaves = (gridDim.x * 256) >> 6;
    const int kOff = nH * HDP, vOff = 2 * nH * HDP;
    for (int pair = wave_global; pair < total_pairs; pair += nwaves) {
        const int win = pair / nH, h = pair - win * nH;
        const float* base = qkv + (size_t)win * 16 * ldq + h * HDP;
        const float* rowp = base + (size_t)i * ldq + STEPS * g;
        float kf[STEPS], qf[STEPS];
#pragma unroll
        for (int r = 0; r < STEPS; ++r) { qf[r] = rowp[r]; kf[r] = rowp[kOff + r]; }
        f32x4 s = zero4();
#pragma unroll
        for (int r = 0; r < STEPS; ++r) s = __builtin_amdgcn_mfma_f32_16x16x4f32(kf[r], qf[r], s, 0, 0, 0);
        s += ld4(bias + ((size_t)h * 16 + i) * 16 + 4 * g);
        if (shifted) {
            const int fl = flags[win];
            const bool lastH = (fl & 1) != 0, lastW = (fl & 2) != 0;
            const int qh = i >> 2, qw = i & 3;
            const int labq = 3 * (lastH ? (qh < 2 ? 1 : 2) : 0) + (lastW ? (qw < 2 ? 1 : 2) : 0);
            const int labkh = 3 * (lastH ? (g < 2 ? 1 : 2) : 0);
#pragma unroll
            for (int r = 0; r < 4; ++r) {
                const int labk = labkh + (lastW ? (r < 2 ? 1 : 2) : 0);
                s[r] += (labk != labq) ? -100.0f : 0.0f;
            }
        }
        float mx = fmaxf(fmaxf(s[0], s[1]), fmaxf(s[2], s[3]));
        mx = fmaxf(mx, __shfl_xor(mx, 16));
        mx = fmaxf(mx, __shfl_xor(mx, 32));
        f32x4 p;
#pragma unroll
        for (int r = 0; r < 4; ++r) p[r] = expf(s[r] - mx);
        float den = (p[0] + p[1]) + (p[2] + p[3]);
        den += __shfl_xor(den, 16);
        den += __shfl_xor(den, 32);
        const float inv = 1.0f / den;
#pragma unroll
        for (int r = 0; r < 4; ++r) p[r] *= inv;
        float* orow = out + ((size_t)win * 16 + i) * ldo + h * HDP;
#pragma unroll
        for (int t = 0; t < DT; ++t) {
            const int d = t * 16 + i;
            f32x4 o = zero4();
#pragma unroll
            for (int r = 0; r < 4; ++r) {
                const float vv = (d < HDP) ? base[(size_t)(4 * g + r) * ldq + vOff + d] : 0.f;
                o = __builtin_amdgcn_mfma_f32_16x16x4f32(vv, p[r], o, 0, 0, 0);
            }
            if (t * 16 + 4 * g < HDP) st4(orow + t * 16 + 4 * g, o);
        }
        if (h == 0 && nH * HDP < ldo) {
            for (int c = nH * HDP + g; c < ldo; c += 4) out[((size_t)win * 16 + i) * ldo + c] = 0.f;
        }
    }
}

__global__ void zero_dead_cols_kernel(float* __restrict__ x, const int* __restrict__ wlen, int B, int H, int W, int Cp) {
    const long long idx = (long long)blockIdx.x * blockDim.x + threadIdx.x;
    const int V = Cp / 4;
    if (idx >= (long long)B * H * W * V) return;
    const long long tok = idx / V;
    const int w = (int)(tok % W), b = (int)(tok / ((long long)H * W));
    if (w >= wlen[b]) st4(x + idx * 4, zero4());
}

template <int NO>
__global__ __launch_bounds__(256) void deembed_border_len_kernel(const float* __restrict__ x, const float* __restrict__ wv, const float* __restrict__ bv,
                                                                 float* __restrict__ out, const int* __restrict__ wlen, int B, int H, int W, int C, int Cp,
                                                                 int pf, int pt, int in_dim, int Fp) {
    const int per_clip = 2 * W + 2 * (H > 2 ? H - 2 : 0);
    const int wave = (blockIdx.x * 256 + threadIdx.x) >> 6, lane = threadIdx.x & 63;
    if (wave >= B * per_clip) return;
    const int b = wave / per_clip; int i = wave - b * per_clip;
    const int Wb = wlen[b];
    int h, w;
    if (i < W) { h = 0; w = i; }
    else if (i < 2 * W) { h = H - 1; w = i - W; }
    else { i -= 2 * W; h = 1 + (i >> 1); w = (i & 1) ? Wb - 1 : 0; }
    if (w >= Wb) return;
    if (H == 1 && i >= W && i < 2 * W) return;
    if (Wb == 1 && i >= 2 * W && (i & 1)) return;
    const int eh = (h == 0 ? 1 : 0) | (h == H - 1 ? 2 : 0), ew = (w == 0 ? 1 : 0) | (w == Wb - 1 ? 2 : 0);
    const int K = 49 * C;
    const float* wvar = wv + (size_t)(4 * eh + ew) * NO * K;
    float acc[NO];
#pragma unroll
    for (int o = 0; o < NO; ++o) acc[o] = 0.f;
    for (int k = lane; k < K; k += 64) {
        const int tap = k / C, ci = k - tap * C;
        const int hh = h + tap / 7 - 3, ww = w + tap % 7 - 3;
        if (hh < 0 || hh >= H || ww < 0 || ww >= Wb) continue;
        const float xv = x[((size_t)(b * H + hh) * W + ww) * Cp + ci];
#pragma unroll
        for (int o = 0; o < NO; ++o) acc[o] = fmaf(wvar[(size_t)o * K + k], xv, acc[o]);
    }
#pragma unroll
    for (int o = 0; o < NO; ++o) {
#pragma unroll
        for (int sft = 32; sft >= 1; sft >>= 1) acc[o] += __shfl_xor(acc[o], sft);
    }
    if (lane == 0) {
        const int Q = pf * pt;
        for (int o = 0; o < NO; ++o) {
            const int co = o / Q, q = o - co * Q, s1 = q / pt, s2 = q - s1 * pt;
            out[((size_t)(b * (pt * W) + pt * w + s2) * in_dim + co) * Fp + pf * h + s1] = acc[o] + bv[(4 * eh + ew) * NO + o];
        }
    }
}

__global__ void istft_ola_len_kernel(const float* __restrict__ frames, const float* __restrict__ win2, float* __restrict__ wave, const int* __restrict__ wlen,
                                     int pt, int B, int T, int ldf, int win, int hop, int left, int half, int out_len) {
    const int idx = blockIdx.x * blockDim.x + threadIdx.x;
    if (idx >= B * out_len) return;
    const int b = idx / out_len, s = idx - b * out_len;
    const int Tb = pt * wlen[b];
    if (s >= hop * (Tb - 1)) { wave[idx] = 0.f; return; }
    const int p = s + half - left;
    int t_hi = p / hop; if (t_hi > Tb - 1) t_hi = Tb - 1;
    float acc = 0.f, env = 0.f;
    for (int t = t_hi; t >= 0; --t) {
        const int j = p - t * hop;
        if (j >= win) break;
        acc += frames[((size_t)b * T + t) * ldf + j];
        env += win2[j];
    }
    wave[idx] = acc / env;
}

__global__ __launch_bounds__(64) void loss_reduce_len_kernel(const float* __restrict__ terms, const int* __restrict__ wlen, int ov, int n_slots, int G, int M,
                                                             int Tq, float* __restrict__ out) {
    const int b = blockIdx.x, lane = threadIdx.x;
    const int Tb = wlen[b] / ov;
    const int per = n_slots * G * Tb;
    float acc = 0.f;
    for (int i = lane; i < per; i += 64) {
        const int sg = i / Tb, t = i - sg * Tb;
        acc += terms[(size_t)sg * M + (size_t)b * Tq + t];
    }
#pragma unroll
    for (int o = 1; o < 64; o <<= 1) acc += __shfl_xor(acc, o);
    if (lane == 0) out[b] = acc / (float)Tb;
}

__global__ void codes_mask_len_kernel(const long long* __restrict__ src, long long* __restrict__ dst, const int* __restrict__ wlen, int ov, int B, int rows,
                                      int Tq, long long fill) {
    const long long idx = (long long)blockIdx.x * blockDim.x + threadIdx.x;
    if (idx >= (long long)B * rows * Tq) return;
    const int t = (int)(idx % Tq), b = (int)(idx / ((long long)rows * Tq));
    const bool live = t < wlen[b] / ov;
    if (live) { if (src != dst) dst[idx] = src[idx]; }
    else dst[idx] = fill;
}

__global__ void unpad_rows_len_kernel(const float* __restrict__ src, float* __restrict__ dst, const int* __restrict__ len, int per_w, int pt, int hop, int B,
                                      int T, int segs, int C, int Cp) {
    const long long idx = (long long)blockIdx.x * blockDim.x + threadIdx.x;
    if (idx >= (long long)B * T * segs * C) return;
    const long long r = idx / C; const int c = (int)(idx - r * C);
    const long long fr = r / segs; const int t = (int)(fr % T), b = (int)(fr / T);
    const int n = per_w ? pt * len[b] : 1 + len[b] / hop;
    dst[idx] = t < n ? src[r * Cp + c] : 0.f;
}

}
```

### efficient-speech-codec_amd/esc/_native.py

```python
import ctypes
import os
from ctypes import POINTER, Structure, byref, c_char_p, c_double, c_float, c_int, c_int16, c_int32, c_int64, c_void_p

_LIB_TAG = os.environ.get("ESCX_LIB_TAG", "")
_LIB_PATH = os.path.join(os.path.dirname(os.path.abspath(__file__)), "lib", "libescx" + ("_" + _LIB_TAG if _LIB_TAG else "") + ".so")
MAX_SCALES = 8


class EscxConfig(Structure):
    _fields_ = [
        ("in_dim", c_int32), ("in_freq", c_int32), ("n_scales", c_int32), ("h_dims", c_int32 * MAX_SCALES),
        ("max_streams", c_int32), ("win_length", c_int32), ("hop_length", c_int32), ("patch_f", c_int32),
        ("patch_t", c_int32), ("swin_heads", c_int32 * MAX_SCALES), ("swin_depth", c_int32), ("window_size", c_int32),
        ("mlp_ratio", c_float), ("overlap", c_int32), ("group_size", c_int32), ("codebook_size", c_int32),
        ("codebook_dims", c_int32 * MAX_SCALES), ("l2norm", c_int32),
    ]


class EscxRvqConfig(Structure):
    _fields_ = [("base", EscxConfig), ("num_rvqs", c_int32), ("codebook_dim", c_int32)]


class EscxDiscConfig(Structure):
    _fields_ = [("sample_rate", c_int32), ("n_rates", c_int32), ("n_periods", c_int32), ("periods", c_int32 * 8), ("n_ffts", c_int32),
                ("fft_sizes", c_int32 * 8), ("n_bands", c_int32), ("bands", (c_float * 2) * 8), ("rates", c_int32 * 8)]


class EscxSpecLossConfig(Structure):
    _fields_ = [("n_scales", c_int32), ("window", c_int32 * 16), ("n_mels", c_int32 * 16), ("filterbank", c_void_p * 16), ("clamp_eps", c_float), ("pow", c_float),
                ("mag_weight", c_float), ("log_weight", c_float)]


class EscxDacConfig(Structure):
    _fields_ = [("encoder_dim", c_int32), ("n_encoder_rates", c_int32), ("encoder_rates", c_int32 * 8), ("latent_dim", c_int32),
                ("decoder_dim", c_int32), ("n_decoder_rates", c_int32), ("decoder_rates", c_int32 * 8), ("n_codebooks", c_int32),
                ("codebook_size", c_int32), ("codebook_dim", c_int32), ("sample_rate", c_int32)]


SIGNATURES = {
    "escx_last_error": (c_char_p, []),
    "escx_version": (c_char_p, []),
    "escx_create": (c_int, [POINTER(EscxConfig), c_int, POINTER(c_void_p)]),
    "escx_create_rvq": (c_int, [POINTER(EscxRvqConfig), c_int, POINTER(c_void_p)]),
    "escx_quantizer_kind": (c_int, [c_void_p]),
    "escx_destroy": (None, [c_void_p]),
    "escx_set_param": (c_int, [c_void_p, c_char_p, c_void_p, POINTER(c_int64), c_int]),
    "escx_finalize_params": (c_int, [c_void_p]),
    "escx_num_required_keys": (c_int, [c_void_p]),
    "escx_required_key": (c_char_p, [c_void_p, c_int]),
    "escx_reserve": (c_int, [c_void_p, c_int, c_int]),
    "escx_workspace_bytes": (c_int64, [c_void_p]),
    "escx_set_precision": (c_int, [c_void_p, c_int]),
    "escx_get_precision": (c_int, [c_void_p]),
    "escx_encode": (c_int, [c_void_p, c_void_p, c_int, c_int, c_int, c_void_p, POINTER(c_int), POINTER(c_int), c_void_p]),
    "escx_decode": (c_int, [c_void_p, c_void_p, c_int, c_int, c_int, c_int, c_void_p, c_void_p, c_void_p]),
    "escx_forward": (c_int, [c_void_p, c_void_p, c_int, c_int, c_int, c_void_p, c_void_p, c_void_p, c_void_p, c_void_p, c_void_p]),
    "escx_forward_feat": (c_int, [c_void_p, c_void_p, c_int, c_int, c_int, c_void_p, c_void_p, c_void_p, c_void_p, c_void_p]),
    "escx_encode_streams": (c_int, [c_void_p, c_void_p, c_int, c_int, POINTER(c_int32), c_void_p, POINTER(c_int), POINTER(c_int), c_void_p]),
    "escx_decode_streams": (c_int, [c_void_p, c_void_p, c_int, c_int, POINTER(c_int32), c_int, c_int, c_void_p, c_void_p, c_void_p]),
    "escx_forward_streams": (c_int, [c_void_p, c_void_p, c_void_p, c_int, c_int, POINTER(c_int32), c_void_p, c_void_p, c_void_p, c_void_p, c_void_p, c_void_p]),
    "escx_encode_lengths": (c_int, [c_void_p, c_void_p, c_int, c_int, POINTER(c_int32), c_int, c_void_p, POINTER(c_int), POINTER(c_int), c_void_p]),
    "escx_decode_lengths": (c_int, [c_void_p, c_void_p, c_int, c_int, POINTER(c_int32), c_int, c_int, c_void_p, c_void_p, c_void_p]),
    "escx_forward_lengths": (c_int, [c_void_p, c_void_p, c_int, c_int, POINTER(c_int32), c_int, c_void_p, c_void_p, c_void_p, c_void_p, c_void_p, c_void_p]),
    "escx_num_frames": (c_int, [c_void_p, c_int]),
    "escx_output_samples": (c_int, [c_void_p, c_int]),
    "escx_spec_transform": (c_int, [c_void_p, c_void_p, c_int, c_int, c_void_p, c_void_p]),
    "escx_audio_reconstruct": (c_int, [c_void_p, c_void_p, c_int, c_int, c_void_p, c_void_p]),
    "escx_patch_embed": (c_int, [c_void_p, c_void_p, c_int, c_int, c_void_p, c_void_p]),
    "escx_transformer_layer": (c_int, [c_void_p, c_int, c_void_p, c_int, c_int, c_int, c_void_p, POINTER(c_int), c_void_p]),
    "escx_pvq_encode": (c_int, [c_void_p, c_int, c_void_p, c_void_p, c_int, c_int, c_void_p, c_int64, c_void_p]),
    "escx_pvq_decode": (c_int, [c_void_p, c_int, c_void_p, c_int64, c_void_p, c_int, c_int, c_void_p, c_void_p]),
    "escx_rvq_encode": (c_int, [c_void_p, c_void_p, c_int, c_int, c_int, c_void_p, c_void_p, c_void_p]),
    "escx_rvq_decode": (c_int, [c_void_p, c_void_p, c_int, c_int, c_int, c_void_p, c_void_p]),
    "escx_patch_deembed": (c_int, [c_void_p, c_void_p, c_int, c_int, c_void_p, c_void_p]),
    "escx_profile_enable": (c_int, [c_void_p, c_int]),
    "escx_profile_report": (c_char_p, [c_void_p]),
    "escx_debug_mlp_trace": (c_int, [c_void_p]),
    "escx_test_math": (c_int, [c_void_p, c_void_p, c_int64, c_int, c_void_p]),
    "escx_test_fastdiv": (c_int, [c_int, c_int]),
    "escx_test_copy_rows": (c_int, [c_void_p, c_void_p, c_int64, c_int, c_void_p]),
    "escx_codes_pack10": (c_int, [c_void_p, c_void_p, c_int64, c_void_p]),
    "escx_codes_unpack10": (c_int, [c_void_p, c_void_p, c_int64, c_void_p]),
    "escx_codes_pack10_streams": (c_int, [c_void_p, c_int, c_int, c_int64, POINTER(c_int32), c_void_p, c_void_p]),
    "escx_codes_unpack10_streams": (c_int, [c_void_p, c_int, c_int, c_int64, POINTER(c_int32), c_void_p, c_void_p]),
    "escx_codes_narrow": (c_int, [c_void_p, c_void_p, c_int64, c_void_p]),
    "escx_codes_widen": (c_int, [c_void_p, c_void_p, c_int64, c_void_p]),
    "escx_flat_param_count": (c_int, [c_void_p]),
    "escx_flat_param_key": (c_char_p, [c_void_p, c_int]),
    "escx_flat_param_offset": (c_int64, [c_void_p, c_int]),
    "escx_flat_param_numel": (c_int64, [c_void_p, c_int]),
    "escx_flat_param_total": (c_int64, [c_void_p]),
    "escx_load_flat_params": (c_int, [c_void_p, c_void_p, c_int, c_void_p]),
    "escx_train_forward": (c_int, [c_void_p, c_void_p, c_void_p, c_int, c_int, c_int, c_int, c_void_p, c_void_p, c_void_p, c_void_p, c_void_p, c_void_p, c_void_p]),
    "escx_train_forward_feat": (c_int, [c_void_p, c_void_p, c_void_p, c_int, c_int, c_int, c_int, c_void_p, c_void_p, c_void_p, c_void_p, c_void_p, c_void_p]),
    "escx_train_backward": (c_int, [c_void_p, c_void_p, c_void_p, c_void_p, c_void_p, c_void_p, c_void_p]),
    "escx_train_backward_ex": (c_int, [c_void_p, c_void_p, c_void_p, c_void_p, c_void_p, c_void_p, c_void_p, c_void_p, c_void_p]),
    "escx_rvq_train_forward": (c_int, [c_void_p, c_void_p, c_void_p, c_void_p, c_int, c_int, c_int, c_int, c_void_p, c_void_p, c_void_p, c_void_p, c_void_p, c_void_p, c_void_p]),
    "escx_rvq_train_backward": (c_int, [c_void_p, c_void_p, c_void_p, c_void_p, c_void_p, c_void_p, c_void_p, c_void_p, c_void_p]),
    "escx_train_tape_bytes": (c_int64, [c_void_p]),
    "escx_train_tape_generation": (c_int64, [c_void_p]),
    "escx_stft_loss": (c_int, [c_void_p, c_void_p, c_int, c_int64, c_void_p, c_void_p, c_void_p]),
    "escx_mel_loss": (c_int, [c_void_p, c_void_p, c_int, c_int, c_int, c_void_p, c_void_p, c_void_p]),
    "escx_stft_loss_ex": (c_int, [c_void_p, c_void_p, c_int, c_int64, c_void_p, c_void_p, c_void_p, c_void_p]),
    "escx_mel_loss_ex": (c_int, [c_void_p, c_void_p, c_int, c_int, c_int, c_void_p, c_void_p, c_void_p, c_void_p]),
    "escx_scale_rows": (c_int, [c_void_p, c_void_p, c_void_p, c_int, c_int64, c_void_p]),
    "escx_grad_norm_clip": (c_int, [c_void_p, c_int64, c_float, c_void_p, c_void_p]),
    "escx_adamw_step": (c_int, [c_void_p, c_void_p, c_void_p, c_void_p, c_int64, c_int, c_double, c_double, c_double, c_double, c_double, c_void_p, c_void_p]),
    "escx_disc_create": (c_int, [POINTER(EscxDiscConfig), c_int, POINTER(c_void_p)]),
    "escx_disc_destroy": (None, [c_void_p]),
    "escx_disc_param_count": (c_int, [c_void_p]),
    "escx_disc_param_key": (c_char_p, [c_void_p, c_int]),
    "escx_disc_param_offset": (c_int64, [c_void_p, c_int]),
    "escx_disc_param_numel": (c_int64, [c_void_p, c_int]),
    "escx_disc_param_total": (c_int64, [c_void_p]),
    "escx_disc_num_fmaps": (c_int, [c_void_p, c_int]),
    "escx_disc_fmap_shape": (c_int, [c_void_p, c_int, c_int] + [POINTER(c_int)] * 7),
    "escx_disc_forward": (c_int, [c_void_p, c_void_p, c_int64, c_void_p, c_int, c_int, POINTER(c_void_p), c_void_p]),
    "escx_disc_backward": (c_int, [c_void_p, c_void_p, c_int64, c_void_p, c_int, c_int, POINTER(c_void_p), POINTER(c_void_p), c_void_p, c_void_p, c_void_p]),
    "escx_gan_term": (c_int, [c_void_p, c_void_p, c_void_p, c_int, c_int, c_int, c_int, c_int, c_int, c_int, c_float, c_void_p, c_int, c_void_p]),
    "escx_gan_term_grad": (c_int, [c_void_p, c_void_p, c_void_p, c_void_p, c_int, c_int, c_int, c_int, c_int, c_int, c_int, c_float, c_void_p]),
    "escx_disc_set_precision": (c_int, [c_void_p, c_int]),
    "escx_disc_get_precision": (c_int, [c_void_p]),
    "escx_disc_profile_enable": (c_int, [c_int]),
    "escx_disc_profile_report": (c_char_p, []),
    "escx_dac_create": (c_int, [POINTER(EscxDacConfig), c_int, POINTER(c_void_p)]),
    "escx_dac_destroy": (None, [c_void_p]),
    "escx_dac_param_count": (c_int, [c_void_p]),
    "escx_dac_param_key": (c_char_p, [c_void_p, c_int]),
    "escx_dac_param_offset": (c_int64, [c_void_p, c_int]),
    "escx_dac_param_numel": (c_int64, [c_void_p, c_int]),
    "escx_dac_param_total": (c_int64, [c_void_p]),
    "escx_dac_num_frames": (c_int, [c_void_p, c_int]),
    "escx_dac_output_samples": (c_int, [c_void_p, c_int]),
    "escx_dac_encode": (c_int, [c_void_p, c_void_p, c_int64, c_void_p, c_int, c_int, c_int, c_void_p, c_void_p, c_void_p, c_void_p, c_void_p]),
    "escx_dac_encode_ex": (c_int, [c_void_p, c_void_p, c_int64, c_void_p, c_int, c_int, c_int, POINTER(c_int32), POINTER(c_int32), c_int, c_void_p, c_void_p, c_void_p,
                                   c_void_p, c_void_p, c_void_p]),
    "escx_dac_from_codes": (c_int, [c_void_p, c_void_p, c_int64, c_void_p, c_int, c_int, c_int, c_void_p, c_void_p, c_void_p]),
    "escx_dac_from_codes_ex": (c_int, [c_void_p, c_void_p, c_int64, c_void_p, c_int, c_int, c_int, POINTER(c_int32), c_void_p, c_void_p, c_void_p]),
    "escx_dac_decode": (c_int, [c_void_p, c_void_p, c_int64, c_void_p, c_int, c_int, c_void_p, c_void_p]),
    "escx_dac_encode_lengths": (c_int, [c_void_p, c_void_p, c_int64, c_void_p, c_int, c_int, POINTER(c_int32), c_int, c_int, POINTER(c_int32), c_void_p, c_void_p,
                                        c_void_p, c_void_p, c_void_p]),
    "escx_dac_from_codes_lengths": (c_int, [c_void_p, c_void_p, c_int64, c_void_p, c_int, c_int, c_int, POINTER(c_int32), POINTER(c_int32), c_void_p, c_void_p,
                                            c_void_p]),
    "escx_dac_decode_lengths": (c_int, [c_void_p, c_void_p, c_int64, c_void_p, c_int, c_int, POINTER(c_int32), POINTER(c_int32), c_void_p, c_void_p]),
    "escx_dac_set_snake_maps": (c_int, [c_void_p, c_int]),
    "escx_dac_get_snake_maps": (c_int, [c_void_p]),
    "escx_dac_set_precision": (c_int, [c_void_p, c_int]),
    "escx_dac_get_precision": (c_int, [c_void_p]),
    "escx_dac_set_grad_precision": (c_int, [c_void_p, c_int]),
    "escx_dac_get_grad_precision": (c_int, [c_void_p]),
    "escx_dac_set_param_grad_precision": (c_int, [c_void_p, c_int]),
    "escx_dac_get_param_grad_precision": (c_int, [c_void_p]),
    "escx_dac_set_padding": (c_int, [c_void_p, c_int]),
    "escx_dac_get_padding": (c_int, [c_void_p]),
    "escx_dac_delay": (c_int, [c_void_p]),
    "escx_dac_output_length": (c_int, [c_void_p, c_int]),
    "escx_dac_encode_chunks": (c_int, [c_void_p, c_void_p, c_int64, c_void_p, c_int, c_int64, c_int, c_int, c_int, c_int64, c_int, c_void_p, c_void_p, c_void_p, c_void_p,
                               c_void_p]),
    "escx_dac_test_math": (c_int, [c_void_p, c_void_p, c_void_p, c_int64, c_int, c_void_p]),
    "escx_dac_decode_tape_floats": (c_int64, [c_void_p, c_int, c_int]),
    "escx_dac_decode_tape": (c_int, [c_void_p, c_void_p, c_int64, c_void_p, c_int, c_int, c_void_p, c_void_p, c_int64, c_void_p]),
    "escx_dac_decode_backward": (c_int, [c_void_p, c_void_p, c_int64, c_void_p, c_int64, c_void_p, c_int, c_int, c_void_p, c_void_p]),
    "escx_dac_decode_backward_params": (c_int, [c_void_p, c_void_p, c_int64, c_void_p, c_int64, c_void_p, c_void_p, c_int, c_int, c_void_p, c_void_p, c_void_p]),
    "escx_dac_param_grad_workspace_floats": (c_int64, [c_void_p]),
    "escx_dac_param_grad_slices": (c_int, [c_void_p, c_int, c_int, c_int]),
    "escx_dac_test_grad_math": (c_int, [c_void_p, c_void_p, c_void_p, c_int64, c_int, c_void_p]),
    "escx_dac_encode_tape_floats": (c_int64, [c_void_p, c_int, c_int, c_int]),
    "escx_dac_encode_tape": (c_int, [c_void_p, c_void_p, c_int64, c_void_p, c_int, c_int, c_int, POINTER(c_int32), c_void_p, c_void_p, c_void_p, c_void_p, c_void_p,
                                     c_int64, c_void_p]),
    "escx_dac_encode_backward": (c_int, [c_void_p, c_void_p, c_int64, c_void_p, c_int64, c_void_p, c_void_p, c_void_p, c_int, c_int, c_void_p, c_void_p]),
    "escx_dac_encode_backward_params": (c_int, [c_void_p, c_void_p, c_int64, c_void_p, c_int64, c_void_p, c_void_p, c_void_p, c_void_p, c_void_p, c_int, c_int, c_int,
                                                c_void_p, c_void_p, c_void_p]),
    "escx_dac_encode_param_grad_slices": (c_int, [c_void_p, c_int, c_int, c_int]),
    "escx_spec_loss_create": (c_int, [POINTER(EscxSpecLossConfig), c_int, POINTER(c_void_p)]),
    "escx_spec_loss_destroy": (None, [c_void_p]),
    "escx_spec_loss_workspace_floats": (c_int64, [c_void_p, c_int, c_int, c_int, c_int]),
    "escx_spec_loss_eval": (c_int, [c_void_p, c_void_p, c_void_p, c_int, c_int, c_void_p, c_void_p, c_void_p, c_void_p]),
    "escx_wave_l1": (c_int, [c_void_p, c_void_p, c_int64, c_float, c_void_p, c_void_p, c_void_p, c_void_p]),
    "escx_sisdr": (c_int, [c_void_p, c_void_p, c_int, c_int64, c_int, c_int, c_int, c_float, c_void_p, c_void_p, c_void_p, c_void_p]),
    "escx_set_rccl_library": (c_int, [c_char_p]),
    "escx_allgather_codes": (c_int, [c_void_p, c_void_p, c_int64, c_void_p, c_int, c_void_p, c_void_p]),
}

PRECISIONS = {"fp32": 0, "f16x2": 2, "bf16x3": 3}
ESCX_ERR_INVALID_ARG, ESCX_ERR_UNSUPPORTED, ESCX_ERR_HIP, ESCX_ERR_STATE, ESCX_ERR_ASSERT = -1, -2, -3, -4, -5

_lib = None
HW_QUEUES_ENV = "GPU_MAX_HW_QUEUES"
HW_QUEUES_WANTED = "8"


def ensure_hw_queues() -> str:
    cur = os.environ.get(HW_QUEUES_ENV)
    if cur:
        return cur
    late = False
    try:
        import sys
        tc = sys.modules.get("torch")
        late = bool(tc is not None and tc.cuda.is_initialized())
    except Exception:
        late = False
    if late:
        import warnings
        warnings.warn(f"{HW_QUEUES_ENV} was not set before HIP initialised: the two-stream overlap of esc.ESC.encode/decode may serialise "
                      f"next to RCCL (export {HW_QUEUES_ENV}={HW_QUEUES_WANTED}, or import esc before the first CUDA call)", RuntimeWarning, stacklevel=3)
        return "default"
    os.environ[HW_QUEUES_ENV] = HW_QUEUES_WANTED
    return HW_QUEUES_WANTED


def lib_path() -> str:
    return _LIB_PATH


def load():
    global _lib
    if _lib is not None:
        return _lib
    ensure_hw_queues()
    if not os.path.exists(_LIB_PATH):
        raise ImportError(
            f"{_LIB_PATH} not found: the HIP library is the only implementation of esc.ESC.encode/decode. "
            "Build it with `python efficient-speech-codec_amd/build.py` (hipcc, gfx950).")
    lib = ctypes.CDLL(_LIB_PATH)
    for name, (res, args) in SIGNATURES.items():
        fn = getattr(lib, name)
        fn.restype = res
        fn.argtypes = args
    _lib = lib
    return lib


def check(rc: int):
    if rc == 0:
        return
    msg = (load().escx_last_error() or b"").decode("utf-8", "replace")
    if rc == ESCX_ERR_ASSERT:
        raise AssertionError(msg)
    if rc == ESCX_ERR_INVALID_ARG:
        raise ValueError(msg)
    if rc == ESCX_ERR_UNSUPPORTED:
        raise NotImplementedError(msg)
    raise RuntimeError(f"escx error {rc}: {msg}")
```

### include/escx.h

```cpp
#ifndef ESCX_H
#define ESCX_H

#include <stdint.h>

#ifdef __cplusplus
extern "C" {
#endif

#define ESCX_MAX_SCALES 8

typedef enum {
    ESCX_OK = 0,
    ESCX_ERR_INVALID_ARG = -1,
    ESCX_ERR_UNSUPPORTED = -2,
    ESCX_ERR_HIP = -3,
    ESCX_ERR_STATE = -4,
    ESCX_ERR_ASSERT = -5
} escx_status;

typedef struct {
    int32_t in_dim;
    int32_t in_freq;
    int32_t n_scales;
    int32_t h_dims[ESCX_MAX_SCALES];
    int32_t max_streams;
    int32_t win_length;
    int32_t hop_length;
    int32_t patch_f, patch_t;
    int32_t swin_heads[ESCX_MAX_SCALES];
    int32_t swin_depth;
    int32_t window_size;
    float   mlp_ratio;
    int32_t overlap;
    int32_t group_size;
    int32_t codebook_size;
    int32_t codebook_dims[ESCX_MAX_SCALES];
    int32_t l2norm;
} escx_config;

typedef struct escx_handle_s* escx_handle;

typedef struct {
    escx_config base;
    int32_t num_rvqs;
    int32_t codebook_dim;
} escx_rvq_config;

const char* escx_last_error(void);
const char* escx_version(void);
int escx_create(const escx_config* cfg, int device, escx_handle* out);
int escx_create_rvq(const escx_rvq_config* cfg, int device, escx_handle* out);
int escx_quantizer_kind(escx_handle h);
void escx_destroy(escx_handle h);

int escx_set_param(escx_handle h, const char* key, const float* host_data, const int64_t* shape, int ndim);
int escx_finalize_params(escx_handle h);
int escx_num_required_keys(escx_handle h);
const char* escx_required_key(escx_handle h, int i);

int escx_reserve(escx_handle h, int batch, int n_samples);
int64_t escx_workspace_bytes(escx_handle h);

#define ESCX_PRECISION_FP32   0
#define ESCX_PRECISION_F16X2  2
#define ESCX_PRECISION_BF16X3 3
int escx_set_precision(escx_handle h, int mode);
int escx_get_precision(escx_handle h);

int escx_encode(escx_handle h, const float* wave_dev, int batch, int n_samples, int num_streams,
                int64_t* codes_dev, int* feat_h, int* feat_w, void* stream);
int escx_decode(escx_handle h, const int64_t* codes_dev, int batch, int num_streams, int feat_h, int feat_w,
                float* wave_out_dev, float* recon_feat_dev, void* stream);
int escx_forward(escx_handle h, const float* wave_dev, int batch, int n_samples, int num_streams,
                 int64_t* codes_dev, float* wave_out_dev, float* raw_feat_dev, float* recon_feat_dev,
                 float* cm_loss_dev, void* stream);
int escx_forward_feat(escx_handle h, const float* feat_dev, int batch, int n_frames, int num_streams,
                      int64_t* codes_dev, float* wave_out_dev, float* recon_feat_dev, float* cm_loss_dev, void* stream);
int escx_encode_streams(escx_handle h, const float* wave_dev, int batch, int n_samples, const int32_t* streams,
                        int64_t* codes_dev, int* feat_h, int* feat_w, void* stream);
int escx_decode_streams(escx_handle h, const int64_t* codes_dev, int batch, int smax, const int32_t* streams, int feat_h, int feat_w,
                        float* wave_out_dev, float* recon_feat_dev, void* stream);
int escx_forward_streams(escx_handle h, const float* wave_dev, const float* feat_dev, int batch, int n_samples_or_frames, const int32_t* streams,
                         int64_t* codes_dev, float* wave_out_dev, float* raw_feat_dev, float* recon_feat_dev, float* cm_loss_dev, void* stream);
int escx_encode_lengths(escx_handle h, const float* wave_dev, int batch, int row_len, const int32_t* lengths, int num_streams,
                        int64_t* codes_dev, int* feat_h, int* feat_w, void* stream);
int escx_decode_lengths(escx_handle h, const int64_t* codes_dev, int batch, int num_streams, const int32_t* widths, int feat_h, int feat_w,
                        float* wave_out_dev, float* recon_feat_dev, void* stream);
int escx_forward_lengths(escx_handle h, const float* wave_dev, int batch, int row_len, const int32_t* lengths, int num_streams,
                         int64_t* codes_dev, float* wave_out_dev, float* raw_feat_dev, float* recon_feat_dev, float* cm_loss_dev, void* stream);
int escx_num_frames(escx_handle h, int n_samples);
int escx_output_samples(escx_handle h, int feat_w);

int escx_spec_transform(escx_handle h, const float* wave_dev, int batch, int n_samples, float* spec_dev, void* stream);
int escx_audio_reconstruct(escx_handle h, const float* spec_dev, int batch, int n_frames, float* wave_dev, void* stream);
int escx_patch_embed(escx_handle h, const float* spec_dev, int batch, int n_frames, float* tokens_dev, void* stream);
int escx_transformer_layer(escx_handle h, int layer_id, const float* x_dev, int batch, int H, int W,
                           float* y_dev, int* H_out, void* stream);
int escx_pvq_encode(escx_handle h, int stream_id, const float* enc_dev, const float* dec_dev, int batch, int W,
                    int64_t* codes_dev, int64_t code_batch_stride, void* stream);
int escx_pvq_decode(escx_handle h, int stream_id, const int64_t* codes_dev, int64_t code_batch_stride,
                    const float* dec_dev, int batch, int W, float* out_dev, void* stream);
int escx_rvq_encode(escx_handle h, const float* tokens_dev, int batch, int W, int num_streams, int64_t* codes_dev, float* zq_out_dev, void* stream);
int escx_rvq_decode(escx_handle h, const int64_t* codes_dev, int batch, int num_streams, int W, float* tokens_out_dev, void* stream);
int escx_patch_deembed(escx_handle h, const float* tokens_dev, int batch, int W, float* spec_dev, void* stream);

int escx_profile_enable(escx_handle h, int enable);
const char* escx_profile_report(escx_handle h);

int escx_debug_mlp_trace(unsigned long long* dev_buf);
int escx_test_math(const float* x_dev, float* y_dev, int64_t n, int which, void* stream);
int escx_test_copy_rows(const float* src_dev, float* dst_dev, int64_t rows, int row_floats, void* stream);
int escx_test_fastdiv(int n, int d);

int escx_codes_pack10(const int64_t* codes_dev, uint8_t* out_dev, int64_t n, void* stream);
int escx_codes_unpack10(const uint8_t* in_dev, int64_t* codes_dev, int64_t n, void* stream);
int escx_codes_pack10_streams(const int64_t* codes_dev, int batch, int smax, int64_t gt, const int32_t* streams, uint8_t* out_dev, void* stream);
int escx_codes_unpack10_streams(const uint8_t* in_dev, int batch, int smax, int64_t gt, const int32_t* streams, int64_t* codes_dev, void* stream);
int escx_codes_narrow(const int64_t* codes_dev, int16_t* out_dev, int64_t n, void* stream);
int escx_codes_widen(const int16_t* in_dev, int64_t* codes_dev, int64_t n, void* stream);

int escx_flat_param_count(escx_handle h);
const char* escx_flat_param_key(escx_handle h, int i);
int64_t escx_flat_param_offset(escx_handle h, int i);
int64_t escx_flat_param_numel(escx_handle h, int i);
int64_t escx_flat_param_total(escx_handle h);
int escx_load_flat_params(escx_handle h, const float* flat_params_dev, int full, void* stream);
int escx_train_forward(escx_handle h, const float* flat_params_dev, const float* wave_dev, int batch, int n_samples, int num_streams,
                       int freeze_codebook, int64_t* codes_dev, float* wave_out_dev, float* raw_feat_dev, float* recon_feat_dev,
                       float* cm_loss_dev, float* cb_loss_dev, void* stream);
int escx_train_forward_feat(escx_handle h, const float* flat_params_dev, const float* feat_dev, int batch, int n_frames, int num_streams, int freeze_codebook,
                            int64_t* codes_dev, float* wave_out_dev, float* recon_feat_dev, float* cm_loss_dev, float* cb_loss_dev, void* stream);
int escx_train_backward(escx_handle h, const float* d_wave_dev, const float* d_recon_feat_dev, const float* d_cm_loss_dev,
                        const float* d_cb_loss_dev, float* grad_flat_dev, void* stream);
int escx_train_backward_ex(escx_handle h, const float* d_wave_dev, const float* d_recon_feat_dev, const float* d_raw_feat_dev,
                           const float* d_cm_loss_dev, const float* d_cb_loss_dev, float* grad_flat_dev, float* d_input_dev, void* stream);
int escx_rvq_train_forward(escx_handle h, const float* flat_params_dev, const float* wave_dev, const float* feat_dev, int batch, int n_samples_or_frames,
                           int num_streams, int freeze_codebook, int64_t* codes_dev, float* wave_out_dev, float* raw_feat_dev, float* recon_feat_dev,
                           float* cm_loss_dev, float* cb_loss_dev, void* stream);
int escx_rvq_train_backward(escx_handle h, const float* d_wave_dev, const float* d_recon_feat_dev, const float* d_raw_feat_dev,
                            const float* d_cm_loss_dev, const float* d_cb_loss_dev, float* grad_flat_dev, float* d_input_dev, void* stream);
int64_t escx_train_tape_bytes(escx_handle h);
int64_t escx_train_tape_generation(escx_handle h);
int escx_stft_loss(const float* raw_feat_dev, const float* recon_feat_dev, int batch, int64_t per_clip, float* loss_dev,
                   float* d_recon_feat_dev, void* stream);
int escx_stft_loss_ex(const float* raw_feat_dev, const float* recon_feat_dev, int batch, int64_t per_clip, float* loss_dev,
                      float* d_recon_feat_dev, float* d_raw_feat_dev, void* stream);
int escx_mel_loss(const float* raw_wave_dev, const float* recon_wave_dev, int batch, int n_samples, int sample_rate, float* loss_dev,
                  float* d_recon_wave_dev, void* stream);
int escx_mel_loss_ex(const float* raw_wave_dev, const float* recon_wave_dev, int batch, int n_samples, int sample_rate, float* loss_dev,
                     float* d_recon_wave_dev, float* d_raw_wave_dev, void* stream);
int escx_scale_rows(const float* x_dev, const float* g_dev, float* out_dev, int rows, int64_t per_row, void* stream);
int escx_grad_norm_clip(const float* grad_flat_dev, int64_t n, float max_norm, float* norm_out_dev, void* stream);
int escx_adamw_step(float* param_flat_dev, const float* grad_flat_dev, float* exp_avg_dev, float* exp_avg_sq_dev, int64_t n, int step,
                    double lr, double beta1, double beta2, double eps, double weight_decay, const float* clip_dev, void* stream);

typedef struct {
    int32_t sample_rate;
    int32_t n_rates;
    int32_t n_periods; int32_t periods[8];
    int32_t n_ffts; int32_t fft_sizes[8];
    int32_t n_bands; float bands[8][2];
    int32_t rates[8];
} escx_disc_config;
typedef struct escx_disc_s* escx_disc;
int escx_disc_create(const escx_disc_config* cfg, int device, escx_disc* out);
void escx_disc_destroy(escx_disc d);
int escx_disc_param_count(escx_disc d);
const char* escx_disc_param_key(escx_disc d, int i);
int64_t escx_disc_param_offset(escx_disc d, int i);
int64_t escx_disc_param_numel(escx_disc d, int i);
int64_t escx_disc_param_total(escx_disc d);
int escx_disc_num_fmaps(escx_disc d, int n_samples);
int escx_disc_fmap_shape(escx_disc d, int n_samples, int i, int* sub, int* C, int* Cp, int* D0, int* D1, int* P1, int* off1);
int escx_disc_forward(escx_disc d, const float* flat_params_dev, int64_t params_version, const float* wave_dev, int batch, int n_samples,
                      float* const* fmaps_dev, void* stream);
int escx_disc_backward(escx_disc d, const float* flat_params_dev, int64_t params_version, const float* wave_dev, int batch, int n_samples,
                       float* const* fmaps_dev, const float* const* d_fmaps_dev, float* grad_flat_dev, float* d_wave_dev, void* stream);
int escx_disc_set_precision(escx_disc d, int mode);
int escx_disc_get_precision(escx_disc d);
int escx_gan_term(const float* x_dev, const float* ref_dev, float* grad_dev, int batch, int C, int Cp, int D0, int D1, int P1, int mode, float target,
                  float* loss_dev, int accumulate, void* stream);
int escx_gan_term_grad(const float* x_dev, const float* ref_dev, const float* g_dev, float* grad_dev, int batch, int C, int Cp, int D0, int D1, int P1, int mode,
                       float target, void* stream);
int escx_disc_profile_enable(int enable);
const char* escx_disc_profile_report(void);

int escx_set_rccl_library(const char* path);
int escx_allgather_codes(escx_handle h, const int64_t* codes_local_dev, int64_t n_local_codes, int64_t* codes_all_dev,
                         int world_size, void* nccl_comm, void* stream);

#define ESCX_DAC_MAX_RATES 8
typedef struct {
    int32_t encoder_dim; int32_t n_encoder_rates; int32_t encoder_rates[ESCX_DAC_MAX_RATES];
    int32_t latent_dim;
    int32_t decoder_dim; int32_t n_decoder_rates; int32_t decoder_rates[ESCX_DAC_MAX_RATES];
    int32_t n_codebooks; int32_t codebook_size; int32_t codebook_dim;
    int32_t sample_rate;
} escx_dac_config;
typedef struct escx_dac_s* escx_dac;
int escx_dac_create(const escx_dac_config* cfg, int device, escx_dac* out);
void escx_dac_destroy(escx_dac d);
int escx_dac_param_count(escx_dac d);
const char* escx_dac_param_key(escx_dac d, int i);
int64_t escx_dac_param_offset(escx_dac d, int i);
int64_t escx_dac_param_numel(escx_dac d, int i);
int64_t escx_dac_param_total(escx_dac d);
int escx_dac_num_frames(escx_dac d, int n_samples);
int escx_dac_output_samples(escx_dac d, int n_frames);
int escx_dac_encode(escx_dac d, const float* flat_params_dev, int64_t params_version, const float* audio_dev, int batch, int n_samples, int n_quantizers,
                    float* z_dev, int64_t* codes_dev, float* latents_dev, float* losses_dev, void* stream);
int escx_dac_encode_ex(escx_dac d, const float* flat_params_dev, int64_t params_version, const float* audio_dev, int batch, int n_samples, int n_quantizers,
                       const int32_t* clip_n, const int32_t* snap_n, int n_snaps, float* z_dev, int64_t* codes_dev, float* latents_dev, float* losses_dev,
                       float* zsnap_dev, void* stream);
int escx_dac_from_codes(escx_dac d, const float* flat_params_dev, int64_t params_version, const int64_t* codes_dev, int batch, int n_codes, int n_frames,
                        float* z_dev, float* zp_dev, void* stream);
int escx_dac_from_codes_ex(escx_dac d, const float* flat_params_dev, int64_t params_version, const int64_t* codes_dev, int batch, int n_codes, int n_frames,
                           const int32_t* clip_n, float* z_dev, float* zp_dev, void* stream);
int escx_dac_decode(escx_dac d, const float* flat_params_dev, int64_t params_version, const float* z_dev, int batch, int n_frames, float* audio_dev, void* stream);
int escx_dac_encode_lengths(escx_dac d, const float* flat_params_dev, int64_t params_version, const float* audio_dev, int batch, int row_samples,
                            const int32_t* lengths, int pad_multiple, int n_quantizers, const int32_t* clip_n, float* z_dev, int64_t* codes_dev,
                            float* latents_dev, float* losses_dev, void* stream);
int escx_dac_from_codes_lengths(escx_dac d, const float* flat_params_dev, int64_t params_version, const int64_t* codes_dev, int batch, int n_codes, int n_frames,
                                const int32_t* frame_lengths, const int32_t* clip_n, float* z_dev, float* zp_dev, void* stream);
int escx_dac_decode_lengths(escx_dac d, const float* flat_params_dev, int64_t params_version, const float* z_dev, int batch, int n_frames,
                            const int32_t* frame_lengths, const int32_t* sample_caps, float* audio_dev, void* stream);
#define ESCX_DAC_SNAKE_RES7 0
#define ESCX_DAC_SNAKE_RES1 1
#define ESCX_DAC_SNAKE_DOWN 2
#define ESCX_DAC_SNAKE_UP 3
#define ESCX_DAC_SNAKE_LAST 4
#define ESCX_DAC_SNAKE_ALL 31
#define ESCX_DAC_SNAKE_MAPS_DEFAULT ESCX_DAC_SNAKE_ALL
int escx_dac_set_snake_maps(escx_dac d, int mask);
int escx_dac_get_snake_maps(escx_dac d);
int escx_dac_set_precision(escx_dac d, int mode);
int escx_dac_get_precision(escx_dac d);
int escx_dac_set_grad_precision(escx_dac d, int mode);
int escx_dac_get_grad_precision(escx_dac d);
int escx_dac_set_padding(escx_dac d, int on);
int escx_dac_get_padding(escx_dac d);
int escx_dac_delay(escx_dac d);
int escx_dac_output_length(escx_dac d, int n_samples);
int escx_dac_encode_chunks(escx_dac d, const float* flat_params_dev, int64_t params_version, const float* signal_dev, int rows, int64_t n_signal, int n_chunks,
                           int n_samples, int hop, int64_t lead, int n_quantizers, float* z_dev, int64_t* codes_dev, float* latents_dev, float* losses_dev,
                           void* stream);
int64_t escx_dac_decode_tape_floats(escx_dac d, int batch, int n_frames);
int escx_dac_decode_tape(escx_dac d, const float* flat_params_dev, int64_t params_version, const float* z_dev, int batch, int n_frames, float* audio_dev,
                         float* tape_dev, int64_t tape_floats, void* stream);
int escx_dac_decode_backward(escx_dac d, const float* flat_params_dev, int64_t params_version, const float* tape_dev, int64_t tape_floats,
                             const float* d_audio_dev, int batch, int n_frames, float* d_z_dev, void* stream);
int escx_dac_decode_backward_params(escx_dac d, const float* flat_params_dev, int64_t params_version, const float* tape_dev, int64_t tape_floats,
                                    const float* z_dev, const float* d_audio_dev, int batch, int n_frames, float* d_z_dev, float* grad_flat_dev, void* stream);
int64_t escx_dac_param_grad_workspace_floats(escx_dac d);
int escx_dac_param_grad_slices(escx_dac d, int batch, int n_frames, int layer);
int escx_dac_set_param_grad_precision(escx_dac d, int mode);
int escx_dac_get_param_grad_precision(escx_dac d);
int64_t escx_dac_encode_tape_floats(escx_dac d, int batch, int n_samples, int n_quantizers);
int escx_dac_encode_tape(escx_dac d, const float* flat_params_dev, int64_t params_version, const float* audio_dev, int batch, int n_samples, int n_quantizers,
                         const int32_t* clip_n, float* z_dev, int64_t* codes_dev, float* latents_dev, float* losses_dev, float* tape_dev, int64_t tape_floats,
                         void* stream);
int escx_dac_encode_backward(escx_dac d, const float* flat_params_dev, int64_t params_version, const float* tape_dev, int64_t tape_floats, const float* d_z_dev,
                             const float* d_latents_dev, const float* d_commitment_dev, int batch, int n_samples, float* d_audio_dev, void* stream);
int escx_dac_encode_backward_params(escx_dac d, const float* flat_params_dev, int64_t params_version, const float* tape_dev, int64_t tape_floats,
                                    const float* audio_dev, const float* d_z_dev, const float* d_latents_dev, const float* d_commitment_dev,
                                    const float* d_codebook_dev, int batch, int n_samples, int parts, float* d_audio_dev, float* grad_flat_dev, void* stream);
int escx_dac_encode_param_grad_slices(escx_dac d, int batch, int n_samples, int layer);
int escx_dac_test_math(const float* x_dev, const float* alpha_dev, float* out_dev, int64_t n, int mode, void* stream);
int escx_dac_test_grad_math(const float* x_dev, const float* alpha_dev, float* out_dev, int64_t n, int mode, void* stream);

#define ESCX_SPEC_LOSS_MAX_SCALES 16
typedef struct {
    int32_t n_scales;
    int32_t window[ESCX_SPEC_LOSS_MAX_SCALES];
    int32_t n_mels[ESCX_SPEC_LOSS_MAX_SCALES];
    const float* filterbank[ESCX_SPEC_LOSS_MAX_SCALES];
    float clamp_eps;
    float pow;
    float mag_weight;
    float log_weight;
} escx_spec_loss_config;
typedef struct escx_spec_loss_s* escx_spec_loss;
int escx_spec_loss_create(const escx_spec_loss_config* cfg, int device, escx_spec_loss* out);
void escx_spec_loss_destroy(escx_spec_loss h);
int64_t escx_spec_loss_workspace_floats(escx_spec_loss h, int batch, int n_samples, int want_d_est, int want_d_ref);
int escx_spec_loss_eval(escx_spec_loss h, const float* est_dev, const float* ref_dev, int batch, int n_samples, float* loss_dev, float* d_est_dev,
                        float* d_ref_dev, void* stream);
int escx_wave_l1(const float* est_dev, const float* ref_dev, int64_t n, float scale, float* loss_dev, float* d_est_dev, float* d_ref_dev, void* stream);
int escx_sisdr(const float* references_dev, const float* estimates_dev, int batch, int64_t n_samples, int scaling, int zero_mean, int has_clip_min,
               float clip_min, float* loss_dev, float* d_references_dev, float* d_estimates_dev, void* stream);

#ifdef __cplusplus
}
#endif
#endif
```

Measured before the change: 12840.

## Make de-embed x2 kernel walk multiple tiles with prefetch of next tile

```diff
diff --git a/efficient-speech-codec_amd/build.py b/efficient-speech-codec_amd/build.py
--- a/efficient-speech-codec_amd/build.py
+++ b/efficient-speech-codec_amd/build.py
@@ -10,7 +10,7 @@
 OBJ_DIR = os.path.join(HERE, "build" + ("_" + TAG if TAG else ""))
 LIB = os.path.join(OUT_DIR, "libescx" + ("_" + TAG if TAG else "") + ".so")
 SOURCES = ["escx_api.cpp", "escx_params.cpp", "escx_profile.cpp", "collective.cpp", "train.hip", "disc.hip", "dac.hip", "dac_loss.hip", "gemm_swin.hip", "gemm_misc.hip", "kernels_misc.hip", "len_kernels.hip", "fused_swin.hip"]
-HEADERS = ["launch_prof.h", "split_terms.h", "fused_pvq.h", "fused_prvq.h", "train_prvq.h", "fused_mlp_x3.h", "train_kernels.h", "train_mlp_fused.h", "disc_kernels.h", "disc_msd_kernels.h", "dac_kernels.h", "dac_x3.h", "dac_grad_kernels.h", "dac_param_grad_kernels.h", "dac_loss_kernels.h", "gemm_bf16.h", "conv32_halo.h", "gemm_engine.h", "kernels.h", "len_kernels.h", "launchers.h", "escx_internal.h", "fused_mlp.h", "fused_attn.h", "fused_rowgemm.h", "fused_deembed.h", os.path.join("..", "..", "include", "escx.h")]
+HEADERS = ["launch_prof.h", "split_terms.h", "fused_pvq.h", "fused_prvq.h", "train_prvq.h", "fused_mlp_x3.h", "train_kernels.h", "train_mlp_fused.h", "disc_kernels.h", "disc_msd_kernels.h", "dac_kernels.h", "dac_x3.h", "dac_grad_kernels.h", "dac_param_grad_kernels.h", "dac_loss_kernels.h", "gemm_bf16.h", "conv32_halo.h", "gemm_engine.h", "kernels.h", "len_kernels.h", "launchers.h", "escx_internal.h", "fused_mlp.h", "fused_attn.h", "fused_rowgemm.h", "fused_deembed.h", "deembed_border.h", os.path.join("..", "..", "include", "escx.h")]
 HIPCC = os.environ.get("HIPCC", "/opt/rocm/bin/hipcc")
 FLAGS = ["--offload-arch=gfx950", "-O3", "-std=c++17", "-fPIC", "-Wno-unused-result"] + os.environ.get("ESCX_EXTRA_CXXFLAGS", "").split()
 
diff --git a/efficient-speech-codec_amd/csrc/deembed_border.h b/efficient-speech-codec_amd/csrc/deembed_border.h
--- /dev/null
+++ b/efficient-speech-codec_amd/csrc/deembed_border.h
@@ -0,0 +1,55 @@
+#pragma once
+#include <hip/hip_runtime.h>
+
+namespace escx {
+
+template <int NO>
+__device__ __forceinline__ void deembed_border_pixel(const float* __restrict__ x, const float* __restrict__ wvar, const float* __restrict__ bvar,
+                                                     float* __restrict__ out, int lane, int b, int h, int w, int H, int W, int Wb, int C, int Cp,
+                                                     int pf, int pt, int in_dim, int Fp) {
+    constexpr int U = 7;
+    const int K = 49 * C;
+    const int q64 = 64 / C, r64 = 64 - q64 * C;
+    const float* xb = x + (size_t)b * H * W * Cp;
+    const int dh_lo = max(0, 3 - h), dh_hi = min(6, H + 2 - h);
+    const int k_lo = (dh_lo * 7 * C) & ~63, k_hi = min(K, (dh_hi + 1) * 7 * C);
+    float acc[NO];
+#pragma unroll
+    for (int o = 0; o < NO; ++o) acc[o] = 0.f;
+    int k = k_lo + lane, tap = k / C, ci = k - tap * C;
+    for (int k0 = k_lo; k0 < k_hi; k0 += 64 * U) {
+        float xv[U], wt[U][NO];
+        bool in[U];
+#pragma unroll
+        for (int u = 0; u < U; ++u) {
+            const int dh = tap / 7, dw = tap - 7 * dh;
+            const int hh = h + dh - 3, ww = w + dw - 3;
+            in[u] = k < K && hh >= 0 && hh < H && ww >= 0 && ww < Wb;
+            const int hc = min(max(hh, 0), H - 1), wc = min(max(ww, 0), Wb - 1), kc = min(k, K - 1);
+            xv[u] = xb[((size_t)hc * W + wc) * Cp + ci];
+#pragma unroll
+            for (int o = 0; o < NO; ++o) wt[u][o] = wvar[(size_t)o * K + kc];
+            k += 64; tap += q64; ci += r64;
+            if (ci >= C) { ci -= C; ++tap; }
+        }
+#pragma unroll
+        for (int u = 0; u < U; ++u) {
+#pragma unroll
+            for (int o = 0; o < NO; ++o) acc[o] = in[u] ? fmaf(wt[u][o], xv[u], acc[o]) : acc[o];
+        }
+    }
+#pragma unroll
+    for (int o = 0; o < NO; ++o) {
+#pragma unroll
+        for (int sft = 32; sft >= 1; sft >>= 1) acc[o] += __shfl_xor(acc[o], sft);
+    }
+    if (lane == 0) {
+        const int Q = pf * pt;
+        for (int o = 0; o < NO; ++o) {
+            const int co = o / Q, q = o - co * Q, s1 = q / pt, s2 = q - s1 * pt;
+            out[((size_t)(b * (pt * W) + pt * w + s2) * in_dim + co) * Fp + pf * h + s1] = acc[o] + bvar[o];
+        }
+    }
+}
+
+}
diff --git a/efficient-speech-codec_amd/csrc/escx_api.cpp b/efficient-speech-codec_amd/csrc/escx_api.cpp
--- a/efficient-speech-codec_amd/csrc/escx_api.cpp
+++ b/efficient-speech-codec_amd/csrc/escx_api.cpp
@@ -1289,10 +1289,18 @@
     int rc = check_infer_ready(h); if (rc) return rc;
     Shapes s; if ((rc = stage_ws_for_w(h, B, W, &s))) return rc;
     hipStream_t st = (hipStream_t)stream;
+    if ((rc = ensure_pvq_tables(h, st))) return rc;
     pad_rows(tokens, h->stageA, (long long)B * s.H0 * W, h->C0, h->C0p, st);
     if ((rc = run_deembed(h, h->stageA, B, W, h->rspec, st))) return rc;
     spec_unpad(h, h->rspec, spec, (long long)B * h->cfg.patch_t * W, st);
     return launch_ok("patch_deembed");
+}
+
+extern "C" int escx_patch_deembed_walk(escx_handle h, int B, int W) {
+    if (!h || B < 1 || W < 1) return 1;
+    const auto& c = h->cfg;
+    const bool x2 = h->dch_x2 && h->C0p == 48 && h->deembed_halo && !h->deembed_two_stage && c.in_dim * h->Q <= 16;
+    return x2 ? deembed7_x2_tiles_per_workgroup(B, c.in_freq / c.patch_f, W) : 1;
 }
 
 extern "C" int escx_debug_mlp_trace(unsigned long long* dev_buf) { mlp_set_trace(dev_buf); return 0; }
diff --git a/efficient-speech-codec_amd/csrc/fused_deembed.h b/efficient-speech-codec_amd/csrc/fused_deembed.h
--- a/efficient-speech-codec_amd/csrc/fused_deembed.h
+++ b/efficient-speech-codec_amd/csrc/fused_deembed.h
@@ -113,6 +113,8 @@
 }
 
 constexpr int de2_steps(int CP) { return (49 * CP + 31) / 32; }
+constexpr int DE2_TH = 8, DE2_TW = 32, DE2_CH = 8;
+constexpr int de2_lds_bytes(int CP) { return 2 * (DE2_TH + 6) * (DE2_TW + 6) * CP * 2 + 2 * DE2_CH * 2 * 1024 + 32; }
 inline size_t deembed7_x2_bytes(int CP) { return (size_t)de2_steps(CP) * 2 * 1024 + 32; }
 
 __global__ __launch_bounds__(256) void deembed7_x2_pack_kernel(const f32x4* __restrict__ wf, bf16x8* __restrict__ out, int CP, int nsteps) {
@@ -133,23 +135,24 @@
     if (idx == 0) { float* o = reinterpret_cast<float*>(tail + 1); o[0] = 1.0f / sc; o[1] = sc; o[2] = 0.f; o[3] = 0.f; }
 }
 
+inline int deembed7_x2_walk(int n_tiles) { return n_tiles > 256 ? (n_tiles + 255) / 256 : 1; }
+
 template <int CP>
-__global__ __launch_bounds__(512) void deembed7_x2_kernel(DeembedArgs a, const bf16x8* __restrict__ wf2) {
+__global__ __launch_bounds__(512) void deembed7_x2_kernel(DeembedArgs a, const bf16x8* __restrict__ wf2, int n_tiles, int walk) {
     static_assert(CP == 48, "one wrap of the channel index per 32-deep step");
     ESCX_SET_PRIO_SMALL();
-    constexpr int TH = 8, TW = 32, HH = TH + 6, HW = TW + 6, PS = CP + 8;
-    constexpr int NSTEP = de2_steps(CP), CH = 8, NCH = (NSTEP + CH - 1) / CH, NW = 8, Q8 = CP / 8;
+    constexpr int TH = DE2_TH, TW = DE2_TW, HH = TH + 6, HW = TW + 6, PS = CP;
+    constexpr int NSTEP = de2_steps(CP), CH = DE2_CH, NCH = (NSTEP + CH - 1) / CH, NW = 8, Q8 = CP / 8;
+    constexpr bool EARLY0 = ((NCH - 1) & 1) == 1;
     extern __shared__ __attribute__((aligned(16))) unsigned char de2_lds[];
     _Float16* xh0 = reinterpret_cast<_Float16*>(de2_lds);
     _Float16* xh1 = xh0 + HH * HW * PS;
     bf16x8* wr = reinterpret_cast<bf16x8*>(xh1 + HH * HW * PS);
+    float* de2_red = reinterpret_cast<float*>(wr + 2 * CH * 2 * 64);
     const int tid = threadIdx.x, lane = tid & 63, l15 = lane & 15, lg = lane >> 4;
     const int wave = __builtin_amdgcn_readfirstlane(tid >> 6);
     const int ntw = (a.W + TW - 1) / TW, nth = (a.H + TH - 1) / TH;
-    int bid = blockIdx.x;
-    const int tw = bid % ntw; bid /= ntw;
-    const int th = bid % nth; const int b = bid / nth;
-    const int h0 = th * TH, w0 = tw * TW;
+    const int t0 = blockIdx.x * walk, t1 = min(t0 + walk, n_tiles);
 
     auto issue_chunk = [&](int ch, int buf) {
         const int pieces = min(CH, NSTEP - ch * CH) * 2;
@@ -160,87 +163,113 @@
     issue_chunk(0, 0);
     const f32x4 scv = *reinterpret_cast<const f32x4*>(wf2 + (size_t)NSTEP * 2 * 64 + 1);
 
-    const float* xb = a.x + (size_t)b * a.H * a.W * CP;
     constexpr int NV = (HH * HW * Q8 + 511) / 512;
-    float xr[NV][8];
-    float amax = 0.f;
-#pragma unroll
-    for (int i = 0; i < NV; ++i) {
-        const int v = tid + 512 * i;
-        const int pix = v / Q8, q = v - pix * Q8;
-        const int ph = pix / HW, pw = pix - ph * HW;
-        const int gh = h0 - 3 + ph, gw = w0 - 3 + pw;
-        if (v < HH * HW * Q8 && gh >= 0 && gh < a.H && gw >= 0 && gw < a.W) {
-            const float* p = xb + ((size_t)gh * a.W + gw) * CP + 8 * q;
-            const f32x4 u0 = ld4(p), u1 = ld4(p + 4);
-#pragma unroll
-            for (int e = 0; e < 4; ++e) { xr[i][e] = u0[e]; xr[i][4 + e] = u1[e]; amax = fmaxf(amax, fmaxf(fabsf(u0[e]), fabsf(u1[e]))); }
-        } else {
-#pragma unroll
-            for (int e = 0; e < 8; ++e) xr[i][e] = 0.f;
-        }
-    }
-    __shared__ float de2_red[NW];
-    for (int o = 32; o >= 1; o >>= 1) amax = fmaxf(amax, __shfl_xor(amax, o));
-    if (lane == 0) de2_red[wave] = amax;
-    __syncthreads();
-#pragma unroll
-    for (int i = 0; i < NW; ++i) amax = fmaxf(amax, de2_red[i]);
-    const float act_sc = act_pow2_scale(amax), act_inv = 1.0f / act_sc;
-#pragma unroll
-    for (int i = 0; i < NV; ++i) {
-        const int v = tid + 512 * i;
-        if (v < HH * HW * Q8) {
-            const int pix = v / Q8, q = v - pix * Q8;
-            bf16x8 t[2];
-            split_terms<2>(xr[i], t, act_sc);
-            *reinterpret_cast<bf16x8*>(xh0 + pix * PS + 8 * q) = t[0];
-            *reinterpret_cast<bf16x8*>(xh1 + pix * PS + 8 * q) = t[1];
-        }
-    }
-
-    const bool seg1 = w0 + 16 < a.W;
-    f32x4 acc0 = zero4(), acc1 = zero4();
-    int c = 8 * lg, dw = 0, dh = 0;
-    for (int ch = 0; ch < NCH; ++ch) {
-        asm volatile("s_waitcnt vmcnt(0)" ::: "memory");
-        __syncthreads();
-        if (ch + 1 < NCH) issue_chunk(ch + 1, (ch + 1) & 1);
-        const bf16x8* wb = &wr[((ch & 1) * CH * 2) * 64 + lane];
-#pragma unroll
-        for (int s = 0; s < CH; ++s) {
-            if (ch * CH + s >= NSTEP) break;
-            const int dhc = dh > 6 ? 6 : dh;
-            const int xoff = ((wave + dhc) * HW + dw + l15) * PS + c;
-            const bf16x8 wt0 = wb[(s * 2) * 64], wt1 = wb[(s * 2 + 1) * 64];
-            const bf16x8 x00 = *reinterpret_cast<const bf16x8*>(xh0 + xoff), x01 = *reinterpret_cast<const bf16x8*>(xh1 + xoff);
-            acc0 = mma_x<2>(wt0, x01, acc0); acc0 = mma_x<2>(wt1, x00, acc0); acc0 = mma_x<2>(wt0, x00, acc0);
-            if (seg1) {
-                const bf16x8 x10 = *reinterpret_cast<const bf16x8*>(xh0 + xoff + 16 * PS), x11 = *reinterpret_cast<const bf16x8*>(xh1 + xoff + 16 * PS);
-                acc1 = mma_x<2>(wt0, x11, acc1); acc1 = mma_x<2>(wt1, x10, acc1); acc1 = mma_x<2>(wt0, x10, acc1);
-            }
-            c += 32;
-            if (c >= CP) { c -= CP; if (++dw == 7) { dw = 0; ++dh; } }
-        }
-    }
-
-    const int h = h0 + wave;
-    if (h >= a.H) return;
+    static_assert(NV <= NCH, "one vector per chunk of the previous tile");
+    f32x4 xr[NV][2];
+    auto vec_pixel = [&](int tile, int i, int& gh, int& gw) {
+        const int twi = tile % ntw, r = tile / ntw, thi = r % nth;
+        const int v = min(tid + 512 * i, HH * HW * Q8 - 1);
+        const int pix = v / Q8, ph = pix / HW, pw = pix - ph * HW;
+        gh = thi * TH - 3 + ph; gw = twi * TW - 3 + pw;
+        return v - pix * Q8;
+    };
+    auto vec_inside = [&](int tile, int i) { int gh, gw; vec_pixel(tile, i, gh, gw); return gh >= 0 && gh < a.H && gw >= 0 && gw < a.W; };
+    auto load_vec = [&](int tile, int i) {
+        int gh, gw;
+        const int q = vec_pixel(tile, i, gh, gw), bi = tile / (ntw * nth);
+        const float* p = a.x + (((size_t)bi * a.H + min(max(gh, 0), a.H - 1)) * a.W + min(max(gw, 0), a.W - 1)) * CP + 8 * q;
+        xr[i][0] = ld4(p); xr[i][1] = ld4(p + 4);
+    };
+#pragma unroll
+    for (int i = 0; i < NV; ++i) load_vec(t0, i);
+
     const int Q = a.pf * a.pt;
     const f32x4 bv = ld4(a.bias + 4 * lg);
-    const f32x4 accs[2] = {acc0 * (scv[0] * act_inv), acc1 * (scv[0] * act_inv)};
-#pragma unroll
-    for (int t = 0; t < 2; ++t) {
-        const int w = w0 + 16 * t + l15;
-        if (w >= a.W) continue;
-#pragma unroll
-        for (int r = 0; r < 4; ++r) {
-            const int nn = 4 * lg + r;
-            if (nn >= a.n_out) continue;
-            const int co = nn / Q, q = nn - co * Q, s1 = q / a.pt, s2 = q - s1 * a.pt;
-            a.out[((size_t)(b * (a.pt * a.W) + a.pt * w + s2) * a.in_dim + co) * a.Fp + a.pf * h + s1] = accs[t][r] + bv[r];
-        }
-    }
-}
-
-}
+    auto walk_tile = [&](auto more_c, int tile) {
+        constexpr bool more = decltype(more_c)::value;
+        const int tw = tile % ntw, tr = tile / ntw, th = tr % nth, b = tr / nth;
+        const int h0 = th * TH, w0 = tw * TW;
+
+        float xv[NV][8];
+        float amax = 0.f;
+#pragma unroll
+        for (int i = 0; i < NV; ++i) {
+            const bool in = vec_inside(tile, i);
+#pragma unroll
+            for (int e = 0; e < 8; ++e) { xv[i][e] = in ? xr[i][e >> 2][e & 3] : 0.f; amax = fmaxf(amax, fabsf(xv[i][e])); }
+        }
+        for (int o = 32; o >= 1; o >>= 1) amax = fmaxf(amax, __shfl_xor(amax, o));
+        if (lane == 0) de2_red[wave] = amax;
+        asm volatile("s_waitcnt lgkmcnt(0)" ::: "memory");
+        __builtin_amdgcn_s_barrier();
+        asm volatile("" ::: "memory");
+        if (!EARLY0 && tile > t0) issue_chunk(0, 0);
+#pragma unroll
+        for (int i = 0; i < NW; ++i) amax = fmaxf(amax, de2_red[i]);
+        const float act_sc = act_pow2_scale(amax), act_inv = 1.0f / act_sc;
+#pragma unroll
+        for (int i = 0; i < NV; ++i) {
+            const int v = tid + 512 * i;
+            if (v < HH * HW * Q8) {
+                const int pix = v / Q8, q = v - pix * Q8;
+                bf16x8 t[2];
+                split_terms<2>(xv[i], t, act_sc);
+                *reinterpret_cast<bf16x8*>(xh0 + pix * PS + 8 * q) = t[0];
+                *reinterpret_cast<bf16x8*>(xh1 + pix * PS + 8 * q) = t[1];
+            }
+        }
+
+        const bool seg1 = w0 + 16 < a.W;
+        f32x4 acc0 = zero4(), acc1 = zero4();
+        constexpr int ROWK = 7 * CP, ROWSKIP = (HW - 7) * CP;
+        static_assert(ROWK % 32 == 0 || ROWK % 32 == 16, "a tap row ends on a lane-group pair");
+        const _Float16* xp0 = xh0 + (wave * HW + l15) * PS + 8 * lg;
+        const _Float16* xp1 = xh1 + (wave * HW + l15) * PS + 8 * lg;
+        const bool upper = lg >= 2;
+#pragma unroll
+        for (int ch = 0; ch < NCH; ++ch) {
+            if (ch >= 1 && ch <= NV && more) asm volatile("s_waitcnt vmcnt(2) lgkmcnt(0)" ::: "memory");
+            else asm volatile("s_waitcnt vmcnt(0) lgkmcnt(0)" ::: "memory");
+            __builtin_amdgcn_s_barrier();
+            asm volatile("" ::: "memory");
+            if (ch + 1 < NCH) issue_chunk(ch + 1, (ch + 1) & 1);
+            else if (EARLY0 && more) issue_chunk(0, 0);
+            asm volatile("" ::: "memory");
+            if (ch < NV && more) load_vec(tile + 1, ch);
+            asm volatile("" ::: "memory");
+            const bf16x8* wb = &wr[((ch & 1) * CH * 2) * 64 + lane];
+#pragma unroll
+            for (int s = 0; s < CH; ++s) {
+                if (ch * CH + s >= NSTEP) break;
+                constexpr auto off = [](int k) { const int dh = k / ROWK; return dh > 6 ? k - ROWK + 6 * ROWSKIP : k + dh * ROWSKIP; };
+                const int k0 = 32 * (ch * CH + s);
+                const int xoff = off(k0) == off(k0 + 24) - 24 ? off(k0) : (upper ? off(k0 + 24) - 24 : off(k0));
+                const bf16x8 wt0 = wb[(s * 2) * 64], wt1 = wb[(s * 2 + 1) * 64];
+                const bf16x8 x00 = *reinterpret_cast<const bf16x8*>(xp0 + xoff), x01 = *reinterpret_cast<const bf16x8*>(xp1 + xoff);
+                acc0 = mma_x<2>(wt0, x01, acc0); acc0 = mma_x<2>(wt1, x00, acc0); acc0 = mma_x<2>(wt0, x00, acc0);
+                if (seg1) {
+                    const bf16x8 x10 = *reinterpret_cast<const bf16x8*>(xp0 + xoff + 16 * PS), x11 = *reinterpret_cast<const bf16x8*>(xp1 + xoff + 16 * PS);
+                    acc1 = mma_x<2>(wt0, x11, acc1); acc1 = mma_x<2>(wt1, x10, acc1); acc1 = mma_x<2>(wt0, x10, acc1);
+                }
+            }
+        }
+
+        const int h = h0 + wave;
+        const f32x4 accs[2] = {acc0 * (scv[0] * act_inv), acc1 * (scv[0] * act_inv)};
+#pragma unroll
+        for (int t = 0; t < 2; ++t) {
+            const int w = w0 + 16 * t + l15;
+#pragma unroll
+            for (int r = 0; r < 4; ++r) {
+                const int nn = 4 * lg + r;
+                const int co = nn / Q, q = nn - co * Q, s1 = q / a.pt, s2 = q - s1 * a.pt;
+                if (h < a.H && w < a.W && nn < a.n_out)
+                    a.out[((size_t)(b * (a.pt * a.W) + a.pt * w + s2) * a.in_dim + co) * a.Fp + a.pf * h + s1] = accs[t][r] + bv[r];
+            }
+        }
+    };
+    for (int tile = t0; tile + 1 < t1; ++tile) walk_tile(std::true_type{}, tile);
+    walk_tile(std::false_type{}, t1 - 1);
+}
+
+}
diff --git a/efficient-speech-codec_amd/csrc/fused_swin.hip b/efficient-speech-codec_amd/csrc/fused_swin.hip
--- a/efficient-speech-codec_amd/csrc/fused_swin.hip
+++ b/efficient-speech-codec_amd/csrc/fused_swin.hip
@@ -296,6 +296,10 @@
     return 0;
 }
 
+int deembed7_x2_tiles_per_workgroup(int B, int H, int W) {
+    return deembed7_x2_walk(B * ((H + DE2_TH - 1) / DE2_TH) * ((W + DE2_TW - 1) / DE2_TW));
+}
+
 int deembed7_fused(const float* tok, int B, int H, int W, int Cp, const float* wfrag, const float* bias, float* out, int pf, int pt,
                    int in_dim, int Fp, hipStream_t s, const void* x2_image) {
     DeembedArgs a{tok, reinterpret_cast<const f32x4*>(wfrag), bias, out, B, H, W, pf, pt, in_dim, Fp, in_dim * pf * pt};
@@ -303,12 +307,13 @@
     const int grid = B * ((H + 7) / 8) * ((W + 31) / 32);
     if (x2_image && Cp == 48) {
         auto kern = deembed7_x2_kernel<48>;
-        constexpr int lds = 2 * 14 * 38 * (48 + 8) * 2 + 2 * 8 * 2 * 1024;
+        constexpr int lds = de2_lds_bytes(48);
         static std::atomic<unsigned> done{0};
         int dev = 0; (void)hipGetDevice(&dev);
         const unsigned bit = 1u << (dev & 31);
         if (!(done.load(std::memory_order_relaxed) & bit)) { (void)hipFuncSetAttribute((const void*)kern, hipFuncAttributeMaxDynamicSharedMemorySize, lds); done.fetch_or(bit, std::memory_order_relaxed); }
-        ESCX_LAUNCH(kern, dim3(grid), dim3(512), lds, s, a, reinterpret_cast<const bf16x8*>(x2_image));
+        const int n_tiles = B * ((H + DE2_TH - 1) / DE2_TH) * ((W + DE2_TW - 1) / DE2_TW), walk = deembed7_x2_walk(n_tiles);
+        ESCX_LAUNCH(kern, dim3((n_tiles + walk - 1) / walk), dim3(512), lds, s, a, reinterpret_cast<const bf16x8*>(x2_image), n_tiles, walk);
         return 0;
     }
     switch (Cp) {
diff --git a/efficient-speech-codec_amd/csrc/kernels.h b/efficient-speech-codec_amd/csrc/kernels.h
--- a/efficient-speech-codec_amd/csrc/kernels.h
+++ b/efficient-speech-codec_amd/csrc/kernels.h
@@ -1,6 +1,7 @@
 #pragma once
 #include <hip/hip_runtime.h>
 #include "gemm_engine.h"
+#include "deembed_border.h"
 
 namespace escx {
 
@@ -383,7 +384,7 @@
                                                              const float* __restrict__ bv, float* __restrict__ out, int B, int H, int W,
                                                              int C, int Cp, int pf, int pt, int in_dim, int Fp) {
     const int per_clip = 2 * W + 2 * (H > 2 ? H - 2 : 0);
-    const int wave = (blockIdx.x * 256 + threadIdx.x) >> 6, lane = threadIdx.x & 63;
+    const int wave = __builtin_amdgcn_readfirstlane((blockIdx.x * 256 + threadIdx.x) >> 6), lane = threadIdx.x & 63;
     if (wave >= B * per_clip) return;
     const int b = wave / per_clip; int i = wave - b * per_clip;
     int h, w;
@@ -393,31 +394,8 @@
     if (H == 1 && i >= W && i < 2 * W) return;
     if (W == 1 && i >= 2 * W && (i & 1)) return;
     const int eh = (h == 0 ? 1 : 0) | (h == H - 1 ? 2 : 0), ew = (w == 0 ? 1 : 0) | (w == W - 1 ? 2 : 0);
-    const int K = 49 * C;
-    const float* wvar = wv + (size_t)(4 * eh + ew) * NO * K;
-    float acc[NO];
-#pragma unroll
-    for (int o = 0; o < NO; ++o) acc[o] = 0.f;
-    for (int k = lane; k < K; k += 64) {
-        const int tap = k / C, ci = k - tap * C;
-        const int hh = h + tap / 7 - 3, ww = w + tap % 7 - 3;
-        if (hh < 0 || hh >= H || ww < 0 || ww >= W) continue;
-        const float xv = x[((size_t)(b * H + hh) * W + ww) * Cp + ci];
-#pragma unroll
-        for (int o = 0; o < NO; ++o) acc[o] = fmaf(wvar[(size_t)o * K + k], xv, acc[o]);
-    }
-#pragma unroll
-    for (int o = 0; o < NO; ++o) {
-#pragma unroll
-        for (int sft = 32; sft >= 1; sft >>= 1) acc[o] += __shfl_xor(acc[o], sft);
-    }
-    if (lane == 0) {
-        const int Q = pf * pt;
-        for (int o = 0; o < NO; ++o) {
-            const int co = o / Q, q = o - co * Q, s1 = q / pt, s2 = q - s1 * pt;
-            out[((size_t)(b * (pt * W) + pt * w + s2) * in_dim + co) * Fp + pf * h + s1] = acc[o] + bv[(4 * eh + ew) * NO + o];
-        }
-    }
+    const int var = 4 * eh + ew;
+    deembed_border_pixel<NO>(x, wv + (size_t)var * NO * 49 * C, bv + var * NO, out, lane, b, h, w, H, W, W, C, Cp, pf, pt, in_dim, Fp);
 }
 
 __global__ void pad_rows_kernel(const float* __restrict__ src, float* __restrict__ dst, long long rows, int C, int Cp) {
diff --git a/efficient-speech-codec_amd/csrc/launchers.h b/efficient-speech-codec_amd/csrc/launchers.h
--- a/efficient-speech-codec_amd/csrc/launchers.h
+++ b/efficient-speech-codec_amd/csrc/launchers.h
@@ -48,6 +48,7 @@
 int test_fastdiv(int n, int d);
 int deembed7_fused(const float* tok, int B, int H, int W, int Cp, const float* wfrag, const float* bias, float* out, int pf, int pt,
                    int in_dim, int Fp, hipStream_t s, const void* x2_image = nullptr);
+int deembed7_x2_tiles_per_workgroup(int B, int H, int W);
 size_t deembed7_x2_image_bytes(int Cp);
 int deembed7_x2_pack(const float* wfrag, void* image, int Cp, hipStream_t s);
 int attn_fused(const float* src, float* dst, int Cp, int C, int mode, int n_groups, const float* gamma, const float* beta,
diff --git a/efficient-speech-codec_amd/csrc/len_kernels.h b/efficient-speech-codec_amd/csrc/len_kernels.h
--- a/efficient-speech-codec_amd/csrc/len_kernels.h
+++ b/efficient-speech-codec_amd/csrc/len_kernels.h
@@ -1,6 +1,7 @@
 #pragma once
 #include <hip/hip_runtime.h>
 #include "gemm_engine.h"
+#include "deembed_border.h"
 
 namespace escx {
 
@@ -107,7 +108,7 @@
                                                                  float* __restrict__ out, const int* __restrict__ wlen, int B, int H, int W, int C, int Cp,
                                                                  int pf, int pt, int in_dim, int Fp) {
     const int per_clip = 2 * W + 2 * (H > 2 ? H - 2 : 0);
-    const int wave = (blockIdx.x * 256 + threadIdx.x) >> 6, lane = threadIdx.x & 63;
+    const int wave = __builtin_amdgcn_readfirstlane((blockIdx.x * 256 + threadIdx.x) >> 6), lane = threadIdx.x & 63;
     if (wave >= B * per_clip) return;
     const int b = wave / per_clip; int i = wave - b * per_clip;
     const int Wb = wlen[b];
@@ -119,31 +120,8 @@
     if (H == 1 && i >= W && i < 2 * W) return;
     if (Wb == 1 && i >= 2 * W && (i & 1)) return;
     const int eh = (h == 0 ? 1 : 0) | (h == H - 1 ? 2 : 0), ew = (w == 0 ? 1 : 0) | (w == Wb - 1 ? 2 : 0);
-    const int K = 49 * C;
-    const float* wvar = wv + (size_t)(4 * eh + ew) * NO * K;
-    float acc[NO];
-#pragma unroll
-    for (int o = 0; o < NO; ++o) acc[o] = 0.f;
-    for (int k = lane; k < K; k += 64) {
-        const int tap = k / C, ci = k - tap * C;
-        const int hh = h + tap / 7 - 3, ww = w + tap % 7 - 3;
-        if (hh < 0 || hh >= H || ww < 0 || ww >= Wb) continue;
-        const float xv = x[((size_t)(b * H + hh) * W + ww) * Cp + ci];
-#pragma unroll
-        for (int o = 0; o < NO; ++o) acc[o] = fmaf(wvar[(size_t)o * K + k], xv, acc[o]);
-    }
-#pragma unroll
-    for (int o = 0; o < NO; ++o) {
-#pragma unroll
-        for (int sft = 32; sft >= 1; sft >>= 1) acc[o] += __shfl_xor(acc[o], sft);
-    }
-    if (lane == 0) {
-        const int Q = pf * pt;
-        for (int o = 0; o < NO; ++o) {
-            const int co = o / Q, q = o - co * Q, s1 = q / pt, s2 = q - s1 * pt;
-            out[((size_t)(b * (pt * W) + pt * w + s2) * in_dim + co) * Fp + pf * h + s1] = acc[o] + bv[(4 * eh + ew) * NO + o];
-        }
-    }
+    const int var = 4 * eh + ew;
+    deembed_border_pixel<NO>(x, wv + (size_t)var * NO * 49 * C, bv + var * NO, out, lane, b, h, w, H, W, Wb, C, Cp, pf, pt, in_dim, Fp);
 }
 
 __global__ void istft_ola_len_kernel(const float* __restrict__ frames, const float* __restrict__ win2, float* __restrict__ wave, const int* __restrict__ wlen,
diff --git a/efficient-speech-codec_amd/esc/_native.py b/efficient-speech-codec_amd/esc/_native.py
--- a/efficient-speech-codec_amd/esc/_native.py
+++ b/efficient-speech-codec_amd/esc/_native.py
@@ -73,6 +73,7 @@
     "escx_rvq_encode": (c_int, [c_void_p, c_void_p, c_int, c_int, c_int, c_void_p, c_void_p, c_void_p]),
     "escx_rvq_decode": (c_int, [c_void_p, c_void_p, c_int, c_int, c_int, c_void_p, c_void_p]),
     "escx_patch_deembed": (c_int, [c_void_p, c_void_p, c_int, c_int, c_void_p, c_void_p]),
+    "escx_patch_deembed_walk": (c_int, [c_void_p, c_int, c_int]),
     "escx_profile_enable": (c_int, [c_void_p, c_int]),
     "escx_profile_report": (c_char_p, [c_void_p]),
     "escx_debug_mlp_trace": (c_int, [c_void_p]),
diff --git a/include/escx.h b/include/escx.h
--- a/include/escx.h
+++ b/include/escx.h
@@ -103,6 +103,7 @@
 int escx_rvq_encode(escx_handle h, const float* tokens_dev, int batch, int W, int num_streams, int64_t* codes_dev, float* zq_out_dev, void* stream);
 int escx_rvq_decode(escx_handle h, const int64_t* codes_dev, int batch, int num_streams, int W, float* tokens_out_dev, void* stream);
 int escx_patch_deembed(escx_handle h, const float* tokens_dev, int batch, int W, float* spec_dev, void* stream);
+int escx_patch_deembed_walk(escx_handle h, int batch, int W);
 
 int escx_profile_enable(escx_handle h, int enable);
 const char* escx_profile_report(escx_handle h);
```

New measurement: 12770. Within noise of the previous version (-0.6%).
